# hellovuong/ORB_SLAM3_FAST

Measured on AMD Instinct MI355X. Metric: ORB extract+match frames/sec @1280×720 stereo (both-eye ORBextractor + ComputeStereoMatches), higher is better.
Workload: dtype u8; 1 GPU; C3: synthetic 1280x720 rectified stereo pairs, 1500 features, 8 levels, scale 1.2, FAST 20/7, ComputeStereoMatches (bf=0.12*532.03, b=0.12); handles=4, distinct_streams_per_gpu=32, frames_in_ring=3, stereo_matches_pair0=987, parallelism=independent stereo pairs sharded across GPUs, no data-path collective

## Files before the change

### include/orbx.h

```cpp
#ifndef ORBX_H_
#define ORBX_H_

#include <stddef.h>
#include <stdint.h>

#ifdef __cplusplus
extern "C" {
#endif

#define ORBX_MAX_LEVELS 12

#define ORBX_OK 0
#define ORBX_E_EMPTY (-1)
#define ORBX_E_BADARG (-2)
#define ORBX_E_CAPACITY (-3)
#define ORBX_E_HIP (-4)
#define ORBX_E_NODEVICE (-5)
#define ORBX_E_UNSUPPORTED (-6)
#define ORBX_E_TIMEOUT (-7)

typedef struct orbx_keypoint {
  float x, y, size, angle, response;
  int32_t octave, class_id;
} orbx_keypoint;
// ... 663 lines not shown
int orbx_kfdb_create_sized(int device, int n_vocabulary_words, int scoring, int max_keyframes, int max_words_per_keyframe,
                           orbx_kfdb** out);
void orbx_kfdb_destroy(orbx_kfdb* db);
int orbx_kfdb_size(const orbx_kfdb* db);
int orbx_kfdb_profile(orbx_kfdb* db, int on, float* last_ms);
int orbx_kfdb_add(orbx_kfdb* db, int kf_id, int map_id, const uint32_t* word_ids, const double* word_values, int n_words);
int orbx_kfdb_add_from_batch(orbx_kfdb* db, orbx_extractor* ex, int image, int kf_id, int map_id);
int orbx_kfdb_erase(orbx_kfdb* db, int kf_id);
int orbx_kfdb_clear(orbx_kfdb* db);
int orbx_kfdb_clear_map(orbx_kfdb* db, int map_id);
int orbx_kfdb_set_covisibles(orbx_kfdb* db, int n, const int32_t* kf_ids, const int32_t* best10);
int orbx_kfdb_detect_relocalization_candidates(orbx_kfdb* db, const uint32_t* word_ids, const double* word_values, int n_words,
                                               int map_id, int32_t* candidates, int cap, int32_t* n, const orbx_kfdb_details* details);
int orbx_kfdb_detect_relocalization_candidates_batch(orbx_kfdb* db, orbx_extractor* ex, int first_image, int n_frames,
                                                     const int32_t* map_ids, int32_t* candidates, int cap, int32_t* n,
                                                     const orbx_kfdb_details* details);
int orbx_kfdb_detect_n_best_candidates(orbx_kfdb* db, const uint32_t* word_ids, const double* word_values, int n_words, int map_id,
                                       const int32_t* connected_ids, int n_connected, const int32_t* bad_map_ids, int n_bad_maps,
                                       int n_candidates, int32_t* loop, int32_t* n_loop, int32_t* merge, int32_t* n_merge,
                                       const orbx_kfdb_details* details);



#define ORBX_STAGE_RESIZE 0
#define ORBX_STAGE_DETECT 1
#define ORBX_STAGE_OCTREE 2
#define ORBX_STAGE_BLUR 3
#define ORBX_STAGE_SLOTS 4
#define ORBX_STAGE_DESCRIBE 5
#define ORBX_STAGE_STEREO_MATCH 6
#define ORBX_STAGE_STEREO_FILTER 7
#define ORBX_NUM_STAGES 8
int orbx_profile_enable(orbx_extractor* ex, int on);
int orbx_profile_collect(orbx_extractor* ex, double* ms, int32_t* launches);
const char* orbx_stage_name(int stage);
int orbx_level_stats(orbx_extractor* ex, int image, int32_t* w, int32_t* h, int32_t* n_candidates,
                     int32_t* n_selected);


int orbx_clock_probe_start(int device, int spin_us, void** probe);
int orbx_clock_probe_finish(void* probe, double* ghz);

int orbx_copy_probe(int device, size_t bytes, int iters, double* gbps);

void orbx_debug_introsort(uint64_t* v, int n);
int orbx_debug_introsort_device(int device, uint64_t* v, int n);
#define ORBX_LINALG_RCP64 0
#define ORBX_LINALG_RSQRT64 1
#define ORBX_LINALG_JACOBI_CS 2
#define ORBX_LINALG_SVD3 3
#define ORBX_LINALG_NULL_VECTOR4 4
#define ORBX_LINALG_LDLT6 5
#define ORBX_LINALG_LDLT6_DAMPED 6
#define ORBX_LINALG_LDLT7 7
#define ORBX_LINALG_NULL_VECTOR_SYM9 8
#define ORBX_LINALG_NULL_VECTOR_SYM12 9
#define ORBX_LINALG_SUM16 10
#define ORBX_LINALG_OPS 11
#define ORBX_LINALG_MAX_ITEMS 65536
int orbx_debug_linalg(int device, int op, int n, const void* in, void* out);
#define ORBX_GEOM_CAM_PROJECT 0
#define ORBX_GEOM_CAM_UNPROJECT 1
#define ORBX_GEOM_CAM_UNPROJECT_ROUNDED_TAN 2
#define ORBX_GEOM_KB8_PROJECT_D 3
#define ORBX_GEOM_KB8_PROJECT_JAC 4
#define ORBX_GEOM_SE3_MAP 5
#define ORBX_GEOM_SE3_COMPOSE 6
#define ORBX_GEOM_QMUL 7
#define ORBX_GEOM_QROT 8
#define ORBX_GEOM_NORMALIZE_ROTATION 9
#define ORBX_GEOM_QUAT_FROM_R 10
#define ORBX_GEOM_OPLUS 11
#define ORBX_GEOM_SIM3_EXP 12
#define ORBX_GEOM_SIM3_OPLUS 13
#define ORBX_GEOM_SO_INVERSE 14
#define ORBX_GEOM_RODRIGUES2ROT 15
#define ORBX_GEOM_ROT2RODRIGUES 16
#define ORBX_GEOM_OPS 17
#define ORBX_GEOM_MAX_ITEMS 65536
int orbx_debug_geometry(int device, int op, int n, const void* in, void* out);

void orbx_debug_set_detect_list_cap(int cap);
void orbx_debug_set_octree_global(int on);
void orbx_debug_set_stereo_direct(int max_pairs);
int orbx_debug_upload_results(orbx_extractor* ex, int image, const orbx_keypoint* kps, const uint8_t* desc, int n, int mono_index);
void orbx_debug_set_clahe_cell_kernel(int on);
void orbx_debug_set_remap_lds(int on);
int orbx_debug_remap_footprints(const float* map_x, const float* map_y, ptrdiff_t map_stride, int out_w, int out_h, int src_w,
                                int src_h, int n_maps, int32_t* table, int cap, int32_t* tiles_x, int32_t* tiles_y);
int orbx_debug_front_tables(const orbx_params* p, int width, int height, uint32_t* cells, int cells_cap, uint32_t* tiles,
                            int tiles_cap, int32_t info[4]);
int orbx_debug_preproc_plan(const orbx_preproc* pp, int32_t info[8]);
void orbx_debug_set_resize_tail(int first_level, int max_levels, int band_rows);
int orbx_debug_resize_plan(const orbx_extractor* ex, int32_t* first_level, int32_t* n_levels, int32_t* n_bands, int cap);
int orbx_debug_score_map(orbx_extractor* ex, int enable);
int orbx_debug_score_level(orbx_extractor* ex, int image, int level, uint8_t* dst, ptrdiff_t dst_stride);
int orbx_debug_sincos(int device, const float* angles, int n, int fused, float* sin_out, float* cos_out);

#ifdef __cplusplus
}
#endif
#endif
```

### orb_slam3_fast_amd/__init__.py

```python
import ctypes as C
import os

import numpy as np

_HERE = os.path.dirname(os.path.abspath(__file__))
LIB_PATH = os.path.join(_HERE, os.environ.get("ORBX_LIB_NAME", "liborbx.so"))

KP_DTYPE = np.dtype([("x", "<f4"), ("y", "<f4"), ("size", "<f4"), ("angle", "<f4"), ("response", "<f4"),
                     ("octave", "<i4"), ("class_id", "<i4")])
assert KP_DTYPE.itemsize == 28

OK, E_EMPTY, E_BADARG, E_CAPACITY, E_HIP, E_NODEVICE, E_UNSUPPORTED, E_TIMEOUT = 0, -1, -2, -3, -4, -5, -6, -7
TH_HIGH, TH_LOW, HISTO_LENGTH = 100, 50, 30
NUM_STAGES = 8
MP_DTYPE = np.dtype([("proj_x", "<f4"), ("proj_y", "<f4"), ("proj_xr", "<f4"), ("view_cos", "<f4"), ("track_depth", "<f4"),
                     ("predicted_level", "<i4"), ("in_view", "u1"), ("bad", "u1"), ("has_observations", "u1"),
                     ("pad_", "u1"), ("desc", "u1", (32,))])
assert MP_DTYPE.itemsize == 60
PP_DTYPE = np.dtype([("u", "<f4"), ("v", "<f4"), ("ur", "<f4"), ("radius", "<f4"), ("angle", "<f4"), ("min_level", "<i4"),
                     ("max_level", "<i4"), ("valid", "u1"), ("has_observations", "u1"), ("pad_", "u1", (2,)),
                     ("desc", "u1", (32,))])
assert PP_DTYPE.itemsize == 64
FP_DTYPE = np.dtype([("u", "<f4"), ("v", "<f4"), ("ur", "<f4"), ("radius", "<f4"), ("predicted_level", "<i4"), ("valid", "u1"),
                     ("pad_", "u1", (3,)), ("desc", "u1", (32,))])
# ... 96 lines not shown
        L.orbx_preproc_destroy.restype = None
        L.orbx_preproc_output_size.argtypes = [vp, C.POINTER(i), C.POINTER(i)]
        L.orbx_preproc_run.argtypes = [vp, vp, C.c_ssize_t, i, vp, C.c_ssize_t]
        L.orbx_preproc_run_device.argtypes = [vp, vp, i, C.c_ssize_t, C.c_ssize_t, C.POINTER(vp), C.POINTER(i), C.POINTER(i),
                                              C.POINTER(C.c_ssize_t), C.POINTER(C.c_ssize_t)]
        L.orbx_extract_batch_raw_device.argtypes = [vp, vp, vp, i, C.c_ssize_t, C.c_ssize_t, vp]
        L.orbx_vocabulary_create.argtypes = [i, i, i, i, i, i, vp, vp, vp, vp, C.POINTER(vp)]
        L.orbx_vocabulary_load_text.argtypes = [i, C.c_char_p, C.POINTER(vp)]
        L.orbx_vocabulary_destroy.argtypes = [vp]
        L.orbx_vocabulary_destroy.restype = None
        L.orbx_vocabulary_info.argtypes = [vp, vp]
        L.orbx_bow_transform.argtypes = [vp, vp, i, i, vp, vp, C.POINTER(i), vp, vp, vp, C.POINTER(i)]
        L.orbx_bow_transform_batch.argtypes = [vp, vp, i]
        L.orbx_bow_results_device.argtypes = [vp] + [C.POINTER(vp)] * 6 + [C.POINTER(i)]
        L.orbx_bow_download.argtypes = [vp, i, vp, vp, C.POINTER(i), vp, vp, vp, C.POINTER(i), i]
        L.orbx_kfdb_create.argtypes = [vp, i, i, C.POINTER(vp)]
        L.orbx_kfdb_create_sized.argtypes = [i, i, i, i, i, C.POINTER(vp)]
        L.orbx_kfdb_destroy.argtypes = [vp]
        L.orbx_kfdb_destroy.restype = None
        L.orbx_kfdb_size.argtypes = [vp]
        L.orbx_kfdb_profile.argtypes = [vp, i, C.POINTER(f)]
        L.orbx_kfdb_add.argtypes = [vp, i, i, vp, vp, i]
        L.orbx_kfdb_add_from_batch.argtypes = [vp, vp, i, i, i]
        L.orbx_kfdb_erase.argtypes = [vp, i]
        L.orbx_kfdb_clear.argtypes = [vp]
        L.orbx_kfdb_clear_map.argtypes = [vp, i]
        L.orbx_kfdb_set_covisibles.argtypes = [vp, i, vp, vp]
        L.orbx_kfdb_detect_relocalization_candidates.argtypes = [vp, vp, vp, i, i, vp, i, C.POINTER(i), vp]
        L.orbx_kfdb_detect_relocalization_candidates_batch.argtypes = [vp, vp, i, i, vp, vp, i, vp, vp]
        L.orbx_kfdb_detect_n_best_candidates.argtypes = [vp, vp, vp, i, i, vp, i, vp, i, i, vp, C.POINTER(i), vp, C.POINTER(i), vp]
        L.orbx_search_by_bow.argtypes = [i, vp, vp, vp, i, vp, vp, vp, i, vp, vp, vp, i, vp, vp, i, i, f, i, vp]
        L.orbx_search_by_projection_fisheye_batch.argtypes = [vp, i, i, i, f, f, f, f, vp, vp, vp, i, f, i, f, f, vp, vp, vp, vp, vp, vp]
        L.orbx_search_by_projection_frame_fisheye_batch.argtypes = [vp, i, i, i, f, f, f, f, vp, vp, vp, i, i, vp, vp, vp, vp]
        L.orbx_search_by_bow_batch.argtypes = [vp, i, i, vp, vp, vp, i, vp, vp, vp, vp, vp, i, i, f, i, vp, vp]
        L.orbx_search_by_projection_fisheye.argtypes = [i, vp, vp, i, i, f, f, f, f, vp, i, vp, vp, i, f, i, f, f, vp, vp, vp, vp]
        L.orbx_search_by_projection_frame_fisheye.argtypes = [i, vp, vp, i, i, f, f, f, f, vp, vp, i, i, vp, vp]
        L.orbx_compute_image_bounds.argtypes = [i, i, i, vp, vp, i, vp]
        L.orbx_fisheye_results_device.argtypes = [vp, vp, vp, vp, vp, vp]
        L.orbx_fisheye_download.argtypes = [vp, i, vp, vp, vp, vp, i, i, vp]
        L.orbx_search_for_initialization.argtypes = [i, vp, vp, i, vp, vp, i, f, f, f, f, vp, vp, i, f, i]
        L.orbx_search_for_initialization_batch.argtypes = [vp, i, i, vp, vp, vp, i, f, f, f, f, vp, vp, i, f, i, vp]
        L.orbx_search_by_projection.argtypes = [i, vp, vp, vp, i, f, f, f, f, vp, i, vp, i, f, i, f, f, vp, vp]
        L.orbx_search_by_projection_frame.argtypes = [i, vp, vp, vp, i, f, f, f, f, vp, i, i, vp, vp]
        L.orbx_search_by_projection_frame_batch.argtypes = [vp, i, i, f, f, f, f, vp, vp, i, i, i, vp, vp, vp, vp]
        L.orbx_search_by_projection_batch.argtypes = [vp, i, i, f, f, f, f, vp, vp, i, f, i, f, f, i, vp, vp, vp, vp]
        L.orbx_search_by_projection_keyframe.argtypes = [i, vp, vp, i, f, f, f, f, vp, i, i, i, vp, vp]
        L.orbx_map_upload.argtypes = [vp, i, vp, vp, vp, vp, vp, vp]
        L.orbx_project_map_points_batch.argtypes = [vp, i, vp, f, f, f, f, f, vp, vp]
        L.orbx_last_frames_upload.argtypes = [vp, i, i, vp, vp, vp, vp, vp, vp]
        L.orbx_project_map_points_fisheye_batch.argtypes = [vp, i, vp, vp, f, f, f, f, f, vp, vp, vp]
        L.orbx_project_last_frames_batch.argtypes = [vp, i, vp, f, f, f, f, f, vp]
        L.orbx_search_for_triangulation.argtypes = [i, vp, vp, vp, i, vp, vp, vp, vp, i, vp, vp, vp, i, vp, vp, vp, vp, i, vp, vp, i,
                                                    vp, vp, i, i, i, vp]
        L.orbx_search_for_triangulation_rig.argtypes = [i, vp, vp, vp, i, vp, vp, vp, i, i, vp, vp, vp, i, vp, vp, vp, i, i, vp, vp, i, vp,
                                                        i, i, i, vp]
        L.orbx_search_by_bow_keyframes.argtypes = [i, vp, vp, vp, i, vp, vp, vp, i, vp, vp, vp, i, vp, vp, vp, i, f, i, vp]
        L.orbx_fuse_search.argtypes = [i, vp, vp, vp, i, f, f, f, f, vp, i, vp, i, i, vp, vp]
        L.orbx_features_in_area.argtypes = [i, vp, i, f, f, f, f, vp, i, vp, vp, i, vp, vp]
        L.orbx_comm_unique_id.argtypes = [vp]
        L.orbx_comm_create.argtypes = [vp, i, i, i, C.POINTER(vp)]
        L.orbx_comm_adopt.argtypes = [vp, i, C.POINTER(vp)]
        L.orbx_comm_destroy.argtypes = [vp]
        L.orbx_comm_destroy.restype = None
        L.orbx_comm_size.argtypes = [vp, C.POINTER(i), C.POINTER(i)]
        L.orbx_allgather_descriptors.argtypes = [vp, vp, i, vp, vp]
        L.orbx_comm_wait.argtypes = [vp, i, C.POINTER(C.c_ulonglong)]
        L.orbx_clock_probe_start.argtypes = [i, i, C.POINTER(vp)]
        L.orbx_clock_probe_finish.argtypes = [vp, C.POINTER(C.c_double)]
        L.orbx_copy_probe.argtypes = [i, C.c_size_t, i, C.POINTER(C.c_double)]
        L.orbx_profile_enable.argtypes = [vp, i]
        L.orbx_profile_collect.argtypes = [vp, vp, vp]
        L.orbx_stage_name.restype = C.c_char_p
        L.orbx_stage_name.argtypes = [i]
        L.orbx_level_stats.argtypes = [vp, i, vp, vp, vp, vp]
        L.orbx_debug_introsort.argtypes = [vp, i]
        L.orbx_debug_introsort.restype = None
        L.orbx_debug_introsort_device.argtypes = [i, vp, i]
        L.orbx_debug_linalg.argtypes = [i, i, i, vp, vp]
        L.orbx_debug_geometry.argtypes = [i, i, i, vp, vp]
        L.orbx_debug_set_detect_list_cap.argtypes = [i]
        L.orbx_debug_set_detect_list_cap.restype = None
        L.orbx_debug_set_octree_global.argtypes = [i]
        L.orbx_debug_set_octree_global.restype = None
        L.orbx_debug_set_stereo_direct.argtypes = [i]
        L.orbx_debug_set_stereo_direct.restype = None
        L.orbx_debug_set_clahe_cell_kernel.argtypes = [i]
        L.orbx_debug_set_clahe_cell_kernel.restype = None
        L.orbx_debug_upload_results.argtypes = [vp, i, vp, vp, i, i]
        L.orbx_debug_set_remap_lds.argtypes = [i]
        L.orbx_debug_set_remap_lds.restype = None
        L.orbx_debug_remap_footprints.argtypes = [vp, vp, C.c_ssize_t, i, i, i, i, i, vp, i, C.POINTER(i), C.POINTER(i)]
        L.orbx_debug_preproc_plan.argtypes = [vp, vp]
        if hasattr(L, "orbx_debug_front_tables"):
            L.orbx_debug_front_tables.argtypes = [vp, i, i, vp, i, vp, i, vp]
        L.orbx_debug_set_resize_tail.argtypes = [i, i, i]
        L.orbx_debug_set_resize_tail.restype = None
        L.orbx_debug_resize_plan.argtypes = [vp, vp, vp, vp, i]
        L.orbx_debug_sincos.argtypes = [i, vp, i, i, vp, vp]
        L.orbx_debug_score_map.argtypes = [vp, i]
        L.orbx_set_opencv_compat.argtypes = [vp, i]
        L.orbx_debug_score_level.argtypes = [vp, i, i, vp, C.c_ssize_t]
        _lib = L
    return _lib


def _check(rc):
    if rc < 0:
        raise OrbxError(rc, lib().orbx_last_error().decode())
    return rc


def _p(a):
    return a.ctypes.data_as(C.c_void_p)


def device_count():
    return lib().orbx_device_count()


class ORBextractor:

    def __init__(self, nfeatures, scaleFactor, nlevels, iniThFAST, minThFAST, max_width=1280, max_height=720,
                 max_batch=1, device=0):
        self.nfeatures, self.nlevels = int(nfeatures), int(nlevels)
        self.max_batch = max_batch
        p = _Params(nfeatures, scaleFactor, nlevels, iniThFAST, minThFAST)
        h = C.c_void_p()
        _check(lib().orbx_extractor_create(C.byref(p), max_width, max_height, max_batch, device, C.byref(h)))
        self._h = h
        self.device = device
        L = self.nlevels
        t = [np.zeros(L, np.float32) for _ in range(4)]
        self._nfeat = np.zeros(L, np.int32)
        self._umax = np.zeros(16, np.int32)
        _check(lib().orbx_get_tables(h, _p(t[0]), _p(t[1]), _p(t[2]), _p(t[3]), _p(self._nfeat), _p(self._umax)))
        self._scale, self._inv_scale, self._sigma2, self._inv_sigma2 = t
        cap = C.c_int()
        _check(lib().orbx_batch_results_device(h, None, None, None, None, C.byref(cap)))
        self.capacity = cap.value

    def close(self):
        if getattr(self, "_h", None):
            lib().orbx_extractor_destroy(self._h)
            self._h = None

    def __del__(self):
        try:
            self.close()
        except Exception:
            pass

    def GetLevels(self):
        return self.nlevels

    def GetScaleFactor(self):
        return float(self._scale[1]) if self.nlevels > 1 else 1.0

    def GetScaleFactors(self):
        return self._scale.copy()

    def GetInverseScaleFactors(self):
        return self._inv_scale.copy()

    def GetScaleSigmaSquares(self):
        return self._sigma2.copy()

# ... 1266 lines not shown
    def __init__(self, src_w, src_h, channels=1, rgb=True, maps=None, out_size=None, clahe=None, max_batch=2, device=0):
        prm = _PreprocParams()
        prm.src_w, prm.src_h, prm.channels, prm.rgb_order = src_w, src_h, channels, int(bool(rgb))
        keep = []
        if maps is not None:
            mx = np.ascontiguousarray(maps[0], np.float32)
            my = np.ascontiguousarray(maps[1], np.float32)
            if mx.ndim == 2:
                mx, my = mx[None], my[None]
            prm.n_maps, prm.out_h, prm.out_w = mx.shape
            prm.map_x, prm.map_y, prm.map_stride = mx.ctypes.data, my.ctypes.data, mx.shape[2]
            keep = [mx, my]
        elif out_size is not None:
            prm.out_w, prm.out_h = out_size
        if clahe is not None:
            prm.clahe_clip_limit, (prm.clahe_tiles_x, prm.clahe_tiles_y) = float(clahe[0]), clahe[1]
        h = C.c_void_p()
        _check(lib().orbx_preproc_create(C.byref(prm), max_batch, device, C.byref(h)))
        del keep
        self._h = h
        ow, oh = C.c_int(), C.c_int()
        _check(lib().orbx_preproc_output_size(self._h, C.byref(ow), C.byref(oh)))
        self.out_w, self.out_h, self.channels, self.src_w, self.src_h = ow.value, oh.value, channels, src_w, src_h

    def __del__(self):
        if getattr(self, "_h", None):
            lib().orbx_preproc_destroy(self._h)
            self._h = None

    def run(self, frame, map_index=0):
        frame = np.ascontiguousarray(frame, np.uint8)
        dst = np.zeros((self.out_h, self.out_w), np.uint8)
        _check(lib().orbx_preproc_run(self._h, _p(frame), frame.strides[0], map_index, _p(dst), dst.strides[0]))
        return dst

    def run_device(self, d_frames_ptr, n_frames, row_pitch, image_pitch):
        out, w, h = C.c_void_p(), C.c_int(), C.c_int()
        rp, ip = C.c_ssize_t(), C.c_ssize_t()
        _check(lib().orbx_preproc_run_device(self._h, C.c_void_p(d_frames_ptr), n_frames, row_pitch, image_pitch, C.byref(out),
                                             C.byref(w), C.byref(h), C.byref(rp), C.byref(ip)))
        return out.value, w.value, h.value, rp.value, ip.value

    def plan(self):
        info = np.zeros(8, np.int32)
        _check(lib().orbx_debug_preproc_plan(self._h, _p(info)))
        opt = [None if v < 0 else int(v) for v in info[2:6]]
        return {"lds_table": bool(info[0]), "resize_prepared": bool(info[1]), "remap": opt[0],
                "resize": None if opt[1] is None else ("plain" if opt[1] else "generic"),
                "clahe_vec4": None if opt[2] is None else bool(opt[2]), "gray_segs": opt[3], "frames": int(info[6])}


REMAP_LDS, REMAP_WINDOWS, REMAP_GENERIC = 2, 1, 0


def remap_footprints(map_x, map_y, src_w, src_h):
    mx = np.ascontiguousarray(map_x, np.float32)
    my = np.ascontiguousarray(map_y, np.float32)
    if mx.ndim == 2:
        mx, my = mx[None], my[None]
    if mx.shape != my.shape or mx.ndim != 3:
        raise ValueError("map_x and map_y must be float images of the same size")
    nm, dh, dw = mx.shape
    tx, ty = (dw + 127) // 128, (dh + 7) // 8
    tab = np.zeros((nm, tx, ty, 8), np.int32)
    gx, gy = C.c_int(), C.c_int()
    rc = lib().orbx_debug_remap_footprints(_p(mx), _p(my), dw, dw, dh, src_w, src_h, nm, _p(tab), tab.size, C.byref(gx), C.byref(gy))
    _check(rc)
    if (gx.value, gy.value) != (tx, ty):
        raise OrbxError("unexpected tile grid %d x %d" % (gx.value, gy.value))
    return tab if rc == 1 else None


def front_tables(nfeatures, scaleFactor, nlevels, iniThFAST, minThFAST, width, height):
    prm = _Params(int(nfeatures), float(scaleFactor), int(nlevels), int(iniThFAST), int(minThFAST))
    info = np.zeros(4, np.int32)
    _check(lib().orbx_debug_front_tables(C.byref(prm), width, height, None, 0, None, 0, _p(info)))
    cells = np.zeros((int(info[0]), 16), np.uint32)
    tiles = np.zeros(int(info[1]), np.uint32)
    _check(lib().orbx_debug_front_tables(C.byref(prm), width, height, _p(cells), cells.size, _p(tiles) if tiles.size else None,
                                         tiles.size, _p(info)))
    return cells, tiles, int(info[2]), int(info[3])


class ORBVocabulary:

    def __init__(self, k=None, L=None, parent=None, is_leaf=None, desc=None, weight=None, scoring=0, weighting=0, path=None,
                 device=0):
        h = C.c_void_p()
        if path is not None:
            _check(lib().orbx_vocabulary_load_text(device, path.encode(), C.byref(h)))
        else:
            parent = np.ascontiguousarray(parent, np.int32)
            leaf = np.ascontiguousarray(is_leaf, np.uint8)
            d = np.ascontiguousarray(desc, np.uint8)
            w = np.ascontiguousarray(weight, np.float64)
            _check(lib().orbx_vocabulary_create(device, k, L, scoring, weighting, len(parent), _p(parent), _p(leaf), _p(d), _p(w),
                                                C.byref(h)))
        self._h = h
        info = np.zeros(6, np.int32)
        _check(lib().orbx_vocabulary_info(self._h, _p(info)))
        self.k, self.L, self.n_nodes, self.n_words, self.scoring, self.weighting = (int(x) for x in info)

    def __del__(self):
        if getattr(self, "_h", None):
            lib().orbx_vocabulary_destroy(self._h)
            self._h = None

    def transform(self, desc, levelsup=4):
        d = np.ascontiguousarray(desc, np.uint8).reshape(-1, 32)
        n = len(d)
        words, values = np.zeros(n, np.uint32), np.zeros(n, np.float64)
        nodes, start, feats = np.zeros(n, np.uint32), np.zeros(n + 1, np.int32), np.zeros(n, np.uint32)
        nw, nn = C.c_int(), C.c_int()
        nf = _check(lib().orbx_bow_transform(self._h, _p(d), n, levelsup, _p(words), _p(values), C.byref(nw), _p(nodes), _p(start),
                                             _p(feats), C.byref(nn)))
        return (words[:nw.value].copy(), values[:nw.value].copy()), (nodes[:nn.value].copy(), start[:nn.value + 1].copy(), feats[:nf].copy())

    def transform_batch(self, extractor, levelsup=4):
        _check(lib().orbx_bow_transform_batch(extractor._h, self._h, levelsup))

    @staticmethod
    def download(extractor, image):
        cap = extractor.capacity
        words, values = np.zeros(cap, np.uint32), np.zeros(cap, np.float64)
        nodes, start, feats = np.zeros(cap, np.uint32), np.zeros(cap + 1, np.int32), np.zeros(cap, np.uint32)
        nw, nn = C.c_int(), C.c_int()
        nf = _check(lib().orbx_bow_download(extractor._h, image, _p(words), _p(values), C.byref(nw), _p(nodes), _p(start), _p(feats),
                                            C.byref(nn), cap))
        return (words[:nw.value].copy(), values[:nw.value].copy()), (nodes[:nn.value].copy(), start[:nn.value + 1].copy(), feats[:nf].copy())


class _KfdbDetails(C.Structure):
    _fields_ = [("cap", C.c_int32), ("n_scored", C.c_void_p), ("max_common_words", C.c_void_p), ("kf_id", C.c_void_p),
                ("common_words", C.c_void_p), ("score", C.c_void_p), ("acc_score", C.c_void_p), ("best_kf_id", C.c_void_p)]


KFDB_DETAIL_DTYPE = np.dtype([("kf_id", "<i4"), ("common_words", "<i4"), ("score", "<f4"), ("acc_score", "<f4"), ("best_kf_id", "<i4")])


class KeyFrameDatabase:

    def __init__(self, voc, max_keyframes, max_words):
        self._h = None
        h = C.c_void_p()
        _check(lib().orbx_kfdb_create(voc._h if voc is not None else None, max_keyframes, max_words, C.byref(h)))
        self._h = h
        self.max_keyframes, self.max_words = max_keyframes, max_words

    def close(self):
        if getattr(self, "_h", None):
            lib().orbx_kfdb_destroy(self._h)
            self._h = None

    __del__ = close

    def __len__(self):
        return _check(lib().orbx_kfdb_size(self._h))

    @staticmethod
    def _bow(bow):
        w, v = np.ascontiguousarray(bow[0], np.uint32), np.ascontiguousarray(bow[1], np.float64)
        if w.ndim != 1 or w.shape != v.shape:
            raise ValueError("a BoW vector is (word_ids[n], values[n])")
        return w, v

    def profile(self, on=-1):
# ... 423 lines not shown
```

### orb_slam3_fast_amd/csrc/orbx_api.hip

```cpp
#include "orbx_host.h"
#include "orbx_rgbd.h"

namespace orbx_host {
thread_local std::string g_err;
}

namespace {
struct StageTimer {
  orbx_extractor* ex;
  hipStream_t s;
  int stage;
  size_t i0 = 0;
  bool on;
  StageTimer(orbx_extractor* ex_, hipStream_t s_, int stage_)
      : ex(ex_), s(s_), stage(stage_), on(ex_->profiling && (ex_->profStage < 0 || ex_->profStage == stage_)) {
    if (!on) {
      if (s == ex->stream) ex->lastEvValid = false;
      return;
    }
    if (s == ex->stream && ex->lastEvValid) {
      i0 = ex->lastEv;
    } else {
      hipEvent_t e = ex->next_event();
      i0 = ex->evCursor - 1;
// ... 50 lines not shown
    um[v] = v0;
    ++v0;
  }
  std::memcpy(ex->umax, um, sizeof(um));
}

int build_geom(const orbx_extractor* ex, int w, int h, Geom& g, std::string& why) {
  std::memset(&g, 0, sizeof(g));
  const int L = ex->prm.nlevels;
  g.nlevels = L;
  g.iniTh = ex->prm.ini_th_fast;
  g.minTh = ex->prm.min_th_fast;
  g.cv440 = ex->cv440;
  long long off = 0, candOff = 0, cellOff = 0;
  int cells = 0, sel = 0, xc = 0, yc = 0;
  int maxCW = 0, maxCH = 0;
  for (int l = 0; l < L; l++) {
    LevelDev& v = g.lv[l];
    v.w = cv_round((float)w * ex->inv[l]);
    v.h = cv_round((float)h * ex->inv[l]);
    v.pitch = align_up(v.w, 64);
    v.off = off;
    off += (long long)v.pitch * v.h;
    off = (off + 255) / 256 * 256;
    const int maxBX = v.w - kBorder, maxBY = v.h - kBorder;
    const float width = (float)(maxBX - kBorder), height = (float)(maxBY - kBorder);
    if (width < 35.f || height < 35.f) {
      why = "level " + std::to_string(l) + " is smaller than one 35 px FAST cell (+32 px border)";
      return ORBX_E_UNSUPPORTED;
    }
    v.nCols = (int)(width / 35.f);
    v.nRows = (int)(height / 35.f);
    v.wCell = (int)std::ceil(width / v.nCols);
    v.hCell = (int)std::ceil(height / v.nRows);
    v.cellStart = cells;
    cells += v.nCols * v.nRows;
    v.quota = ex->nfeat[l];
    const int nIni = (int)std::round(width / height);
    if (nIni < 1 || nIni > kMaxIni) {
      why = "unsupported aspect ratio at level " + std::to_string(l);
      return ORBX_E_UNSUPPORTED;
    }
    v.candCap = (((int)width + v.nCols + 1) / 2 + 1) * (((int)height + v.nRows + 1) / 2 + 1);
    v.candOff = candOff;
    candOff += v.candCap;
    v.cellCap = ((v.wCell + 1) / 2) * ((v.hCell + 1) / 2);
    v.cellOff = cellOff;
    cellOff += (long long)v.nCols * v.nRows * v.cellCap;
    v.selOff = sel;
    v.selCap = v.quota + 4 * kMaxIni + 4;
    sel += v.selCap;
    v.xcoef = xc;
    v.ycoef = yc;
    xc += align_up(v.w, 256);
    yc += v.h;
    v.scale = ex->scale[l];
    v.patch = (float)(int)(31 * ex->scale[l]);
    maxCW = std::max(maxCW, v.wCell);
    maxCH = std::max(maxCH, v.hCell);
    if (v.w > 4096 || v.h > 4096) {
      why = "images larger than 4096 px are not supported by the 12-bit key packing";
      return ORBX_E_UNSUPPORTED;
    }
  }
  if (maxCW > 250 || maxCH > 120) {
    why = "FAST cell too large for the packed corner list";
    return ORBX_E_UNSUPPORTED;
  }
  g.totalCells = cells;
  g.tileP = 4 * ((maxCW + 3) / 4 + 2);
  g.tileH = maxCH + 6;
  g.scoreP = 4 * ((maxCW + 3) / 4 + 2);
  g.scoreH = maxCH + 2;
  g.listCap = align_up((long long)maxCW * maxCH, 8);
  g.selImg = sel;
  g.outCap = sel;
  g.pyrImg = off;
  g.candImg = candOff;
  g.cellImg = cellOff;
  if (resize_lds_bytes(g) > 160 * 1024 - 2048) {
    why = "scale factor too large for the LDS-staged resize footprint";
    return ORBX_E_UNSUPPORTED;
  }
  if (octree_lds_bytes(g) > 160 * 1024 - 2048) {
    why = "nfeatures too large for the LDS-resident quadtree";
    return ORBX_E_UNSUPPORTED;
  }
  return ORBX_OK;
}

void build_yrow(const Geom& g, const std::vector<int>& yofs, std::vector<uint32_t>& yrow) {
  yrow.assign(yofs.size(), 0);
  for (int l = 1; l < g.nlevels; l++) {
    const int Sh = g.lv[l - 1].h;
    for (int dy = 0; dy < g.lv[l].h; dy++) {
      const int sy = yofs[g.lv[l].ycoef + dy];
      const int a = std::min(std::max(sy, 0), Sh - 1), b = std::min(std::max(sy + 1, 0), Sh - 1);
      yrow[g.lv[l].ycoef + dy] = (uint32_t)a | ((uint32_t)b << 16);
    }
  }
}

void build_resize_records(const Geom& g, const std::vector<uint4>& xtab, const std::vector<uint32_t>& yrow, const std::vector<short>& yab,
                          std::vector<uint32_t>& tab) {
  int tileOff, rowOff;
  tab.assign((size_t)resize_records_layout(g, g.nlevels, tileOff, rowOff), 0u);
  for (int l = 1; l < g.nlevels; l++) {
    const LevelDev &D = g.lv[l], &S = g.lv[l - 1];
    resize_records_layout(g, l, tileOff, rowOff);
    const int nbx = (D.w + 255) / 256, nby = (D.h + 15) / 16;
    for (int tby = 0; tby < nby; tby++) {
      const int y0 = tby * 16, y1 = std::min(y0 + 16, D.h) - 1;
      const int rb = (int)(yrow[D.ycoef + y0] & 0xFFFFu), re = (int)(yrow[D.ycoef + y1] >> 16);
      const int nrows = re - rb + 1;
      for (int tbx = 0; tbx < nbx; tbx++) {
        const int x0 = tbx * 256, x1 = std::min(x0 + 256, D.w) - 1;
        const int cb = (int)xtab[D.xcoef + x0].y;
        const int ce = std::min((int)xtab[D.xcoef + x1].x + 1, S.w - 1);
        const int ndw = ((ce - cb) >> 2) + 1;
        const bool whole = l > 1 || cb + 4 * ndw <= S.w;
        const bool fast = whole && ndw > 64 && ndw <= 85 && nrows <= 24 && rb + 28 <= S.h;
        uint32_t* t = &tab[(size_t)tileOff + 8 * (size_t)(tby * nbx + tbx)];
        t[0] = (uint32_t)(D.xcoef + x0);
        t[1] = (uint32_t)x0 | ((uint32_t)(y1 - y0 + 1) << 16);
        t[2] = (uint32_t)rb | ((uint32_t)nrows << 16);
        t[3] = (uint32_t)cb | ((uint32_t)ndw << 16);
        t[4] = (fast ? kTileFast : 0u) | (whole ? kTileWhole : 0u);
        t[5] = (uint32_t)((long long)y0 * D.pitch);
        t[6] = (uint32_t)tby;
      }
      for (int w = 0; w < 4; w++)
        for (int k = 0; k < 4; k++) {
          const int dy = std::min(y0 + w + 4 * k, D.h - 1);
          const uint32_t sy = yrow[D.ycoef + dy];
          uint32_t* r = &tab[(size_t)rowOff + 16 * (size_t)(4 * tby + w) + 4 * k];
          r[0] = (uint32_t)(uint16_t)yab[2 * (D.ycoef + dy)] | ((uint32_t)(uint16_t)yab[2 * (D.ycoef + dy) + 1] << 16);
          r[1] = (uint32_t)(((int)(sy & 0xFFFFu) - rb) * 512);
          r[2] = (uint32_t)(((int)(sy >> 16) - rb) * 512);
        }
    }
  }
}

void build_cell_records(const Geom& g, std::vector<CellRec>& recs) {
  recs.assign((size_t)g.totalCells, CellRec{});
  const int TPd = g.tileP >> 2;
  for (int l = 0; l < g.nlevels; l++) {
    const LevelDev& L = g.lv[l];
    const int maxBX = L.w - kBorder, maxBY = L.h - kBorder;
    for (int ci = 0; ci < L.nRows; ci++)
      for (int cj = 0; cj < L.nCols; cj++) {
        const int cell = ci * L.nCols + cj;
        CellRec& r = recs[(size_t)L.cellStart + cell];
        const int iniY = kBorder + ci * L.hCell, iniX = kBorder + cj * L.wCell;
        const int maxY = std::min(iniY + L.hCell + 6, maxBY), maxX = std::min(iniX + L.wCell + 6, maxBX);
        const int rw = maxX - iniX, rh = maxY - iniY;
        const int dw = rw - 6, dh = rh - 6;
        r.flags = ((uint32_t)l << 8) | ((uint32_t)L.w << 16) | (l == 0 ? kCellL0 : 0u);
        if (iniY >= maxBY - 3 || iniX >= maxBX - 6 || dw <= 0 || dh <= 0) {
          r.flags |= kCellReject;
          continue;
        }
        if (iniX + g.tileP <= L.w) r.flags |= kCellWide;
        r.xy = (uint32_t)iniX | ((uint32_t)iniY << 16);
        r.roi = (uint32_t)rw | ((uint32_t)rh << 16);
        r.pitch = (uint32_t)L.pitch;
        r.baseOff = (uint32_t)(L.off + (long long)iniY * L.pitch + iniX);
// ... 152 lines not shown
    bands.insert(bands.end(), nd.begin(), nd.end());
    plans.push_back(tp);
    l += nT;
  }
}

constexpr int kLatLdsMax = 156 * 1024, kLatMaxImages = 2;
static int g_lat_max_images = kLatMaxImages;
static int g_lat_levels = 4, g_lat_rows = 2;
void build_latency_plans(const Geom& g, const std::vector<int>& yofs, std::vector<TailPlan>& plans, std::vector<TailBand>& bands) {
  plans.clear();
  bands.clear();
  static const bool envRead = [] {
    if (const char* e = getenv("ORBX_LAT_TAIL")) {
      int a = -1, b = 0;
      if (sscanf(e, "%d,%d", &a, &b) >= 1) {
        g_lat_levels = a;
        if (b > 0) g_lat_rows = b;
      }
    }
    if (const char* e = getenv("ORBX_LAT_MAX_IMAGES")) g_lat_max_images = atoi(e);
    return true;
  }();
  (void)envRead;
  if (g_lat_levels <= 0) return;
  const int L = g.nlevels;
  int l = 1;
  while (l < L) {
    TailPlan tp;
    std::vector<TailBand> nd;
    int nT = std::min(g_lat_levels, L - l);
    while (nT >= 1 && !build_tail_segment(g, yofs, l, nT, g_lat_rows, tp, nd, 1, 1, (size_t)kLatLdsMax)) nT--;
    if (nT < 1) {
      plans.clear();
      bands.clear();
      return;
    }
    tp.bandOff = (int)bands.size();
    bands.insert(bands.end(), nd.begin(), nd.end());
    plans.push_back(tp);
    l += nT;
  }
}

int configure(orbx_extractor* ex, int w, int h) {
  if (w == ex->curW && h == ex->curH) return ORBX_OK;
  if (w > ex->maxW || h > ex->maxH)
    return fail(ORBX_E_CAPACITY, "image larger than the handle's max_width x max_height");
  Geom g;
  std::string why;
  int rc = build_geom(ex, w, h, g, why);
  if (rc != ORBX_OK) return fail(rc, why);
  const Geom& m = ex->gmax;
  if (g.pyrImg > m.pyrImg || g.candImg > m.candImg || g.selImg > m.selImg || g.cellImg > m.cellImg ||
      g.totalCells > m.totalCells)
    return fail(ORBX_E_CAPACITY, "image within max_width x max_height but its pyramid / cell-grid rounding needs more "
                                 "buffer than the handle's maximum size: create the handle with this size");
  g.outCap = m.outCap;
  g.selImg = m.selImg;
  g.pyrImg = m.pyrImg;
  g.candImg = m.candImg;
  g.cellImg = m.cellImg;
  std::vector<uint4> xtab;
  std::vector<int> yofs;
  std::vector<short> yab;
  build_coefs(g, xtab, yofs, yab);
  HIPC(hipStreamSynchronize(ex->stream));
  HIPC(hipMemcpy(ex->d_xtab.p, xtab.data(), xtab.size() * sizeof(uint4), hipMemcpyHostToDevice));
  HIPC(hipMemcpy(ex->d_yofs.p, yofs.data(), yofs.size() * sizeof(int), hipMemcpyHostToDevice));
  {
    std::vector<uint32_t> yrow, rec;
    build_yrow(g, yofs, yrow);
    HIPC(hipMemcpy(ex->d_yrow.p, yrow.data(), yrow.size() * sizeof(uint32_t), hipMemcpyHostToDevice));
    build_resize_records(g, xtab, yrow, yab, rec);
    if (ex->d_rsRec.n < rec.size()) HIPC(ex->d_rsRec.alloc(rec.size()));
    if (!rec.empty()) HIPC(hipMemcpy(ex->d_rsRec.p, rec.data(), rec.size() * sizeof(uint32_t), hipMemcpyHostToDevice));
  }
  HIPC(hipMemcpy(ex->d_yab.p, yab.data(), yab.size() * sizeof(short), hipMemcpyHostToDevice));
  {
    std::vector<CellRec> recs;
    build_cell_records(g, recs);
    HIPC(hipMemcpy(ex->d_cellRec.p, recs.data(), recs.size() * sizeof(CellRec), hipMemcpyHostToDevice));
  }
  HIPC(prepare_kernels(g));
  std::vector<TailPlan> plans;
  std::vector<TailBand> bands;
  build_tail_plans(g, yofs, plans, bands);
  if (!plans.empty()) {
    if (ex->d_tailBands.n < bands.size()) HIPC(ex->d_tailBands.alloc(bands.size()));
    HIPC(hipMemcpy(ex->d_tailBands.p, bands.data(), bands.size() * sizeof(TailBand), hipMemcpyHostToDevice));
    unsigned lds = 0;
    for (const TailPlan& tp : plans) lds = std::max(lds, tp.ldsBytes);
    HIPC(prepare_resize_tail(lds));
  }
  ex->tails = plans;
  {
    std::vector<TailPlan> lp;
    std::vector<TailBand> lb;
    build_latency_plans(g, yofs, lp, lb);
    if (!lp.empty()) {
      if (ex->d_latBands.n < lb.size()) HIPC(ex->d_latBands.alloc(lb.size()));
      HIPC(hipMemcpy(ex->d_latBands.p, lb.data(), lb.size() * sizeof(TailBand), hipMemcpyHostToDevice));
      unsigned lds = 0;
      for (const TailPlan& tp : lp) lds = std::max(lds, tp.ldsBytes);
      HIPC(prepare_resize_tail(lds));
    }
    ex->latTails = lp;
  }
  ex->g = g;
  ex->curW = w;
  ex->curH = h;
  return ORBX_OK;
}

struct DetectToken {
  std::mutex mu;
  hipEvent_t ev = nullptr;
  bool valid = false;
  const orbx_extractor* last = nullptr;
};
static DetectToken* detect_token(int device) {
  static std::mutex mu;
  static DetectToken* toks[64] = {nullptr};
  if (device < 0 || device >= 64) return nullptr;
  std::lock_guard<std::mutex> lk(mu);
  if (!toks[device]) {
    DetectToken* t = new DetectToken();
    if (hipEventCreateWithFlags(&t->ev, hipEventDisableTiming) != hipSuccess) {
      delete t;
      return nullptr;
    }
    toks[device] = t;
  }
  return toks[device];
}

int record_pipeline(orbx_extractor* ex, int n, bool lapTrivial, bool capturing, bool pyrDone = false);
static void drop_graphs(orbx_extractor* ex) {
  for (auto& e : ex->graphExec) {
    if (e) (void)hipGraphExecDestroy(e);
    e = nullptr;
  }
}

static bool latency_plan_ok(const orbx_extractor* ex, const uint8_t* d_images, int n, int w, ptrdiff_t row_pitch,
                            ptrdiff_t image_pitch) {
  if (ex->latTails.empty() || n > g_lat_max_images) return false;
  if (((uintptr_t)d_images & 15) || (row_pitch & 15) || (image_pitch & 15)) return false;
  return (w & 15) == 0 || d_images == ex->d_stage.p;
}

static int prepare_extract(orbx_extractor* ex, const uint8_t* d_images, int n, int w, int h, ptrdiff_t row_pitch,
                           ptrdiff_t image_pitch, const int32_t* lap, bool& lapTrivial) {
  int rc = configure(ex, w, h);
  if (rc != ORBX_OK) return rc;
  ex->pyr.l0 = d_images;
  ex->pyr.l0Row = row_pitch;
  ex->pyr.l0Img = image_pitch;
  ex->pyr.pyr = ex->d_pyr.p;
  ex->lastN = n;
  ex->lastEvValid = false;
  ex->blurValid = false;
  ex->lastStereoPairs = 0;
  ex->hostPyrImages = 0;
  ex->useLat = latency_plan_ok(ex, d_images, n, w, row_pitch, image_pitch);
  hipStream_t s = ex->stream;
// ... 22 lines not shown
    return ORBX_OK;
  }
  size_t seg = 0;
  for (int l = 1; l < g.nlevels;) {
    StageTimer t(ex, s, ORBX_STAGE_RESIZE);
    if (seg < ex->tails.size() && ex->tails[seg].lA == l) {
      const TailPlan& tp = ex->tails[seg++];
      HIPC(launch_resize_tail(g, ex->pyr, tp, ex->d_tailBands.p + tp.bandOff, 0, n, ex->d_xtab.p, ex->d_yofs.p, ex->d_yab.p, s));
      l += tp.nT;
    } else {
      HIPC(launch_resize(g, ex->pyr, n, l, ex->d_xtab.p, ex->d_yrow.p, ex->d_yab.p, ex->d_rsRec.p, s));
      l++;
    }
  }
  return ORBX_OK;
}

int enqueue_extract(orbx_extractor* ex, const uint8_t* d_images, int n, int w, int h, ptrdiff_t row_pitch,
                    ptrdiff_t image_pitch, const int32_t* lap) {
  bool lapTrivial = true;
  int rc = prepare_extract(ex, d_images, n, w, h, row_pitch, image_pitch, lap, lapTrivial);
  if (rc != ORBX_OK) return rc;
  hipStream_t s = ex->stream;
  static const bool useGraph = getenv("ORBX_GRAPH") && atoi(getenv("ORBX_GRAPH")) != 0;
  if (useGraph && n == 1 && d_images == ex->d_stage.p && !ex->profiling && !ex->graphOff) {
    if (ex->graphW != w || ex->graphH != h) {
      drop_graphs(ex);
      ex->graphW = w;
      ex->graphH = h;
    }
    hipGraphExec_t& exec = ex->graphExec[lapTrivial ? 1 : 0];
    if (!exec) {
      hipGraph_t graph = nullptr;
      bool ok = hipStreamBeginCapture(s, hipStreamCaptureModeThreadLocal) == hipSuccess;
      if (ok) {
        const int rcCap = record_pipeline(ex, n, lapTrivial, true);
        const hipError_t ee = hipStreamEndCapture(s, &graph);
        ok = rcCap == ORBX_OK && ee == hipSuccess && graph != nullptr;
      }
      if (ok) ok = hipGraphInstantiate(&exec, graph, nullptr, nullptr, 0) == hipSuccess;
      if (graph) (void)hipGraphDestroy(graph);
      if (!ok) {
        (void)hipGetLastError();
        exec = nullptr;
        ex->graphOff = true;
      }
    }
    if (exec) {
      HIPC(hipGraphLaunch(exec, s));
      return ORBX_OK;
    }
  }
  return record_pipeline(ex, n, lapTrivial, false);
}

int record_pipeline(orbx_extractor* ex, int n, bool lapTrivial, bool capturing, bool pyrDone) {
  const Geom& g = ex->g;
  hipStream_t s = ex->stream;
  ex->blurValid = false;
  if (!pyrDone) {
    const int rc = enqueue_pyramid(ex, s, 0, n);
    if (rc != ORBX_OK) return rc;
  }
  if (ex->d_dbgScore.p) HIPC(hipMemsetAsync(ex->d_dbgScore.p, 0, ex->d_dbgScore.n, s));
  static const bool noToken = getenv("ORBX_NO_DETECT_TOKEN") && atoi(getenv("ORBX_NO_DETECT_TOKEN")) != 0;
  DetectToken* tok = (!capturing && !noToken && n > g_lat_max_images) ? detect_token(ex->device) : nullptr;
  if (tok) {
    std::lock_guard<std::mutex> lk(tok->mu);
    if (tok->valid && tok->last != ex) HIPC(hipStreamWaitEvent(s, tok->ev, 0));
    ex->lastEvValid = false;
    {
      StageTimer t(ex, s, ORBX_STAGE_DETECT);
      HIPC(launch_detect(g, ex->pyr, ex->d_cellRec.p, n, ex->d_cellCand.p, ex->d_cellCount.p, 0, g.nlevels, ex->d_dbgScore.p, s));
    }
    HIPC(hipEventRecord(tok->ev, s));
    tok->valid = true;
    tok->last = ex;
  } else {
    StageTimer t(ex, s, ORBX_STAGE_DETECT);
    HIPC(launch_detect(g, ex->pyr, ex->d_cellRec.p, n, ex->d_cellCand.p, ex->d_cellCount.p, 0, g.nlevels, ex->d_dbgScore.p, s));
  }
  {
    StageTimer t(ex, s, ORBX_STAGE_OCTREE);
    HIPC(launch_octree(g, n, ex->d_cellCand.p, ex->d_cellCount.p, ex->d_cellPrefix.p, ex->d_cand.p,
                       ex->d_candCount.p, ex->d_knode.p, ex->d_sel.p, ex->d_selCount.p, 0, g.nlevels, s));
  }
  if (!lapTrivial) {
    StageTimer t(ex, s, ORBX_STAGE_SLOTS);
    HIPC(launch_slots(g, n, ex->d_sel.p, ex->d_selCount.p, ex->d_lap.p, ex->d_slot.p, ex->d_nOut.p, ex->d_mono.p, s));
  }
  {
    StageTimer t(ex, s, ORBX_STAGE_DESCRIBE);
    HIPC(launch_describe(g, ex->pyr, n, ex->d_sel.p, ex->d_selCount.p, lapTrivial ? nullptr : ex->d_slot.p, ex->d_kps.p,
                         ex->d_desc.p, ex->d_nOut.p, ex->d_mono.p, s));
  }
  return ORBX_OK;
}

int set_device(int device) {
  int n = 0;
  if (hipGetDeviceCount(&n) != hipSuccess || n <= 0) return fail(ORBX_E_NODEVICE, "no HIP device available");
  if (device < 0 || device >= n) return fail(ORBX_E_BADARG, "device index out of range");
  HIPC(hipSetDevice(device));
  return ORBX_OK;
}

}

extern "C" {

const char* orbx_last_error(void) { return g_err.c_str(); }
int orbx_abi_version(void) { return 1; }
int orbx_device_count(void) {
  int n = 0;
  if (hipGetDeviceCount(&n) != hipSuccess) return 0;
  return n;
}

int orbx_extractor_create(const orbx_params* p, int max_width, int max_height, int max_batch, int device,
                          orbx_extractor** out) {
  if (!p || !out) return fail(ORBX_E_BADARG, "null argument");
  *out = nullptr;
  if (p->nlevels < 1 || p->nlevels > ORBX_MAX_LEVELS || p->nfeatures < 1 || !(p->scale_factor > 1.0f) ||
      p->ini_th_fast < p->min_th_fast || p->min_th_fast < 1 || p->ini_th_fast > 254 || max_batch < 1 ||
      max_width < 1 || max_height < 1)
    return fail(ORBX_E_BADARG, "invalid extractor parameters");
  int rc = set_device(device);
  if (rc != ORBX_OK) return rc;
  orbx_extractor* ex = new orbx_extractor();
  ex->prm = *p;
  ex->device = device;
  ex->maxW = max_width;
  ex->maxH = max_height;
  ex->maxB = max_batch;
  build_tables(ex);
  std::string why;
  rc = build_geom(ex, max_width, max_height, ex->gmax, why);
  if (rc != ORBX_OK) {
    delete ex;
    return fail(rc, why);
  }
  const Geom& m = ex->gmax;
  const size_t B = (size_t)max_batch;
  ex->stagePitch = align_up(max_width, 64);
  int nx = 0, ny = 0;
  for (int l = 0; l < m.nlevels; l++) {
    nx += align_up(m.lv[l].w, 256);
    ny += m.lv[l].h;
  }
  hipError_t e = hipSuccess;
  auto ok = [&](hipError_t r) {
    if (e == hipSuccess) e = r;
  };
  ok(hipStreamCreateWithFlags(&ex->stream, hipStreamNonBlocking));
  ok(hipEventCreateWithFlags(&ex->done, hipEventDisableTiming));
  ok(ex->d_pyr.alloc(B * m.pyrImg + 256));
  ok(ex->d_stage.alloc(B * (size_t)ex->stagePitch * max_height + 256));
  ok(ex->d_cand.alloc(B * m.candImg));
  ok(ex->d_cellCand.alloc(B * m.cellImg));
  ok(ex->d_cellCount.alloc(B * m.totalCells));
  ok(ex->d_cellPrefix.alloc(B * m.totalCells));
  ok(ex->d_knode.alloc(B * m.candImg));
  ok(ex->d_candCount.alloc(B * m.nlevels));
  ok(ex->d_sel.alloc(B * m.selImg));
  ok(ex->d_selCount.alloc(B * m.nlevels + ORBX_MAX_LEVELS));
  ok(ex->d_slot.alloc(B * m.selImg));
  ok(ex->d_kps.alloc(B * m.outCap));
  ok(ex->d_desc.alloc(B * m.outCap * 32));
// ... 612 lines not shown
    HIPC(hipHostMalloc(reinterpret_cast<void**>(&ex->hostPyr), need, hipHostMallocDefault));
    ex->hostPyrBytes = need;
  }
  uint8_t* H = ex->hostPyr;
  const bool want0 = n_levels > 0 && dst[0];
  bool wantRest = false;
  for (int l = 1; l < n_levels; l++) wantRest = wantRest || dst[l];
  if (want0) HIPC(hipMemcpyAsync(H, l0, l0Bytes, hipMemcpyDeviceToHost, ex->stream));
  if (wantRest)
    HIPC(hipMemcpyAsync(H + l0Bytes, ex->pyr.pyr + (long long)image * g.pyrImg + restOff, restBytes, hipMemcpyDeviceToHost, ex->stream));
  HIPC(hipStreamSynchronize(ex->stream));
  for (int l = 0; l < n_levels; l++) {
    if (!dst[l]) continue;
    const LevelDev& L = g.lv[l];
    const uint8_t* src = l == 0 ? H : H + l0Bytes + ((size_t)L.off - restOff);
    const size_t sp = l == 0 ? (size_t)p0 : (size_t)L.pitch;
    if ((size_t)dst_stride[l] == sp && sp == (size_t)L.w) {
      std::memcpy(dst[l], src, sp * L.h);
    } else {
      for (int y = 0; y < L.h; y++) std::memcpy(dst[l] + (size_t)y * dst_stride[l], src + (size_t)y * sp, (size_t)L.w);
    }
  }
  return ORBX_OK;
}

int orbx_debug_candidates(orbx_extractor* ex, int image, int level, int32_t* xys, int cap) {
  if (!ex || image < 0 || image >= ex->lastN || level < 0 || level >= ex->g.nlevels)
    return fail(ORBX_E_BADARG, "bad argument");
  HIPC(hipSetDevice(ex->device));
  HIPC(hipStreamSynchronize(ex->stream));
  const LevelDev& L = ex->g.lv[level];
  const int cells = L.nCols * L.nRows;
  std::vector<int> cnt(cells);
  HIPC(hipMemcpy(cnt.data(), ex->d_cellCount.p + (long long)image * ex->g.totalCells + L.cellStart, (size_t)cells * sizeof(int),
                 hipMemcpyDeviceToHost));
  std::vector<uint32_t> v((size_t)cells * L.cellCap);
  if (!v.empty())
    HIPC(hipMemcpy(v.data(), ex->d_cellCand.p + (long long)image * ex->g.cellImg + L.cellOff, v.size() * 4, hipMemcpyDeviceToHost));
  int n = 0;
  for (int c = 0; c < cells; c++)
    for (int i = 0; i < cnt[c] && n < L.candCap; i++, n++) {
      if (n >= cap) continue;
      const uint32_t k = v[(size_t)c * L.cellCap + i];
      xys[3 * n] = key_x(k);
      xys[3 * n + 1] = key_y(k);
      xys[3 * n + 2] = key_r(k);
    }
  return n;
}

int orbx_debug_front_tables(const orbx_params* p, int width, int height, uint32_t* cells, int cells_cap, uint32_t* tiles,
                            int tiles_cap, int32_t info[4]) {
  if (!p || !info || width < 1 || height < 1 || cells_cap < 0 || tiles_cap < 0 || (cells_cap && !cells) || (tiles_cap && !tiles) ||
      p->nlevels < 1 || p->nlevels > ORBX_MAX_LEVELS || p->nfeatures < 1 || !(p->scale_factor > 1.0f))
    return fail(ORBX_E_BADARG, "bad argument");
  std::unique_ptr<orbx_extractor> ex(new orbx_extractor());
  ex->prm = *p;
  build_tables(ex.get());
  Geom g;
  std::string why;
  const int rc = build_geom(ex.get(), width, height, g, why);
  if (rc != ORBX_OK) return fail(rc, why);
  std::vector<uint4> xtab;
  std::vector<int> yofs;
  std::vector<short> yab;
  std::vector<uint32_t> yrow, rec;
  std::vector<CellRec> cr;
  build_coefs(g, xtab, yofs, yab);
  build_yrow(g, yofs, yrow);
  build_resize_records(g, xtab, yrow, yab, rec);
  build_cell_records(g, cr);
  info[0] = (int32_t)cr.size(); info[1] = (int32_t)rec.size(); info[2] = g.tileP; info[3] = g.tileH;
  if (cells) {
    if (cr.size() * 16 > (size_t)cells_cap) return fail(ORBX_E_CAPACITY, "cell records larger than cells_cap");
    std::memcpy(cells, cr.data(), cr.size() * sizeof(CellRec));
  }
  if (tiles) {
    if (rec.size() > (size_t)tiles_cap) return fail(ORBX_E_CAPACITY, "tile records larger than tiles_cap");
    std::memcpy(tiles, rec.data(), rec.size() * sizeof(uint32_t));
  }
  return ORBX_OK;
}

int orbx_hamming256(const void* a, const void* b) {
  const uint32_t* x = (const uint32_t*)a;
  const uint32_t* y = (const uint32_t*)b;
  int d = 0;
  for (int i = 0; i < 8; i++) d += __builtin_popcount(x[i] ^ y[i]);
  return d;
}

static int enqueue_stereo_match(orbx_extractor* left, int first_left, orbx_extractor* right, int first_right,
                                int n_pairs, float bf, float b, bool withFilter, StereoArgs* argsOut,
                                const ResultPack* packWithBand, bool* packedOut) {
  if (packedOut) *packedOut = false;
  if (!left || !right) return fail(ORBX_E_BADARG, "null handle");
  if (n_pairs <= 0 || first_left < 0 || first_right < 0 || first_left + n_pairs > left->lastN ||
      first_right + n_pairs > right->lastN)
    return fail(ORBX_E_BADARG, "pair range outside the last extraction");
  if (left->device != right->device || left->curW != right->curW || left->curH != right->curH ||
      std::memcmp(&left->prm, &right->prm, sizeof(orbx_params)) != 0)
    return fail(ORBX_E_BADARG, "left and right extractors must share device, image size and parameters");
  if (!(b > 0.f)) return fail(ORBX_E_BADARG, "baseline must be positive");
  HIPC(hipSetDevice(left->device));
  const size_t capL = (size_t)left->gmax.outCap;
  if (left->stereoPairs < n_pairs) {
    HIPC(hipStreamSynchronize(left->stream));
    if (left->uRPairs < n_pairs) {
      HIPC(left->d_uR.alloc((size_t)n_pairs * capL));
      HIPC(left->d_depth.alloc((size_t)n_pairs * capL));
      left->uRPairs = n_pairs;
    }
    HIPC(left->d_sad.alloc((size_t)n_pairs * capL));
    const size_t capS = std::max(capL, (size_t)right->gmax.outCap);
    HIPC(left->d_rowStart.alloc((size_t)n_pairs * 2 * (left->maxH + 2)));
    HIPC(left->d_srec.alloc((size_t)n_pairs * 2 * capS));
    HIPC(left->d_sdesc.alloc((size_t)n_pairs * 2 * capS * 2));
    left->stereoPairs = n_pairs;
  }
  left->lastStereoPairs = n_pairs;
  if (right != left && hipStreamQuery(right->stream) != hipSuccess) {
    HIPC(hipEventRecord(right->done, right->stream));
    HIPC(hipStreamWaitEvent(left->stream, right->done, 0));
  }
  StereoArgs a;
  a.kL = left->d_kps.p;
  a.kR = right->d_kps.p;
  a.dL = left->d_desc.p;
  a.dR = right->d_desc.p;
  a.nL = left->d_nOut.p;
  a.nR = right->d_nOut.p;
  a.capL = (int)capL;
  a.capR = right->gmax.outCap;
  a.firstL = first_left;
  a.firstR = first_right;
  a.bf = bf;
  a.b = b;
  a.uRight = left->d_uR.p;
  a.depth = left->d_depth.p;
  a.sad = left->d_sad.p;
  a.rowStart = left->d_rowStart.p;
  a.srec = left->d_srec.p;
  a.sdesc = left->d_sdesc.p;
  a.cap = (int)std::max(capL, (size_t)right->gmax.outCap);
  a.imgH = left->curH;
  a.band = (int)std::ceil(2.0f * left->scale.back()) + 2;
  const bool direct = stereo_direct_ok(a, n_pairs);
  if (!direct) {
    StageTimer t(left, left->stream, ORBX_STAGE_STEREO_MATCH);
    HIPC(launch_stereo_sort(left->g, a, n_pairs, left->stream));
  }
  {
    StageTimer t(left, left->stream, ORBX_STAGE_STEREO_MATCH);
    const bool pack = direct && packWithBand && n_pairs == 1;
    HIPC(launch_stereo_match(left->g, left->pyr, right->pyr, a, n_pairs, left->stream, direct, pack ? packWithBand : nullptr));
    if (pack && packedOut) *packedOut = true;
  }
  if (withFilter) {
    StageTimer t(left, left->stream, ORBX_STAGE_STEREO_FILTER);
    HIPC(launch_stereo_filter(a, n_pairs, left->stream));
  }
  if (argsOut) *argsOut = a;
  return ORBX_OK;
}

int orbx_stereo_match_batch(orbx_extractor* left, int first_left, orbx_extractor* right, int first_right,
// ... 130 lines not shown
                                const float** d_depth, const float** d_points3d, const int32_t** d_counts) {
  if (!left || left->fisheyePairs == 0) return fail(ORBX_E_BADARG, "no fisheye association has been run on this handle");
  if (d_left_to_right) *d_left_to_right = left->d_fl2r.p;
  if (d_right_to_left) *d_right_to_left = left->d_fr2l.p;
  if (d_depth) *d_depth = left->d_fdepth.p;
  if (d_points3d) *d_points3d = left->d_fp3d.p;
  if (d_counts) *d_counts = left->d_fcnt.p;
  return ORBX_OK;
}

int orbx_fisheye_download(orbx_extractor* left, int pair, int32_t* left_to_right, int32_t* right_to_left, float* depth,
                          float* points3d, int cap_left, int cap_right, int32_t* n_desc_matches) {
  if (!left || pair < 0 || pair >= left->fisheyePairs) return fail(ORBX_E_BADARG, "bad pair index");
  HIPC(hipSetDevice(left->device));
  HIPC(hipStreamSynchronize(left->stream));
  const size_t capL = (size_t)left->gmax.outCap, capR = (size_t)left->fisheyeCapR;
  const size_t nl = std::min(capL, (size_t)std::max(cap_left, 0)), nr = std::min(capR, (size_t)std::max(cap_right, 0));
  if (left_to_right) HIPC(hipMemcpy(left_to_right, left->d_fl2r.p + pair * capL, nl * sizeof(int), hipMemcpyDeviceToHost));
  if (right_to_left) HIPC(hipMemcpy(right_to_left, left->d_fr2l.p + pair * capR, nr * sizeof(int), hipMemcpyDeviceToHost));
  if (depth) HIPC(hipMemcpy(depth, left->d_fdepth.p + pair * capL, nl * sizeof(float), hipMemcpyDeviceToHost));
  if (points3d) HIPC(hipMemcpy(points3d, left->d_fp3d.p + pair * capL * 3, nl * 3 * sizeof(float), hipMemcpyDeviceToHost));
  int cnt[2] = {0, 0};
  HIPC(hipMemcpy(cnt, left->d_fcnt.p + 2 * pair, sizeof(cnt), hipMemcpyDeviceToHost));
  if (n_desc_matches) *n_desc_matches = cnt[1];
  return cnt[0];
}

int orbx_profile_enable(orbx_extractor* ex, int on) {
  if (!ex) return fail(ORBX_E_BADARG, "null handle");
  ex->profiling = on != 0;
  ex->profStage = on >= 2 ? on - 2 : -1;
  ex->lastEvValid = false;
  return ORBX_OK;
}

int orbx_profile_collect(orbx_extractor* ex, double* ms, int32_t* launches) {
  if (!ex || !ms || !launches) return fail(ORBX_E_BADARG, "null argument");
  HIPC(hipSetDevice(ex->device));
  HIPC(hipStreamSynchronize(ex->stream));
  for (int i = 0; i < ORBX_NUM_STAGES; i++) {
    ms[i] = 0;
    launches[i] = 0;
  }
  for (const auto& r : ex->evLog) {
    float t = 0;
    HIPC(hipEventElapsedTime(&t, ex->evPool[r.e0], ex->evPool[r.e1]));
    ms[r.stage] += t;
    launches[r.stage]++;
  }
  ex->evLog.clear();
  ex->evCursor = 0;
  ex->lastEvValid = false;
  return ORBX_OK;
}

const char* orbx_stage_name(int stage) {
  static const char* names[ORBX_NUM_STAGES] = {"k_resize", "k_detect", "k_octree", "k_blur",
                                                "k_slots",  "k_describe", "k_stereo_match", "k_stereo_filter"};
  return stage >= 0 && stage < ORBX_NUM_STAGES ? names[stage] : "?";
}

int orbx_level_stats(orbx_extractor* ex, int image, int32_t* w, int32_t* h, int32_t* n_candidates,
                     int32_t* n_selected) {
  if (!ex || ex->curW == 0 || image < 0 || image >= ex->lastN) return fail(ORBX_E_BADARG, "bad argument");
  HIPC(hipSetDevice(ex->device));
  HIPC(hipStreamSynchronize(ex->stream));
  const int L = ex->g.nlevels;
  for (int l = 0; l < L; l++) {
    if (w) w[l] = ex->g.lv[l].w;
    if (h) h[l] = ex->g.lv[l].h;
  }
  if (n_candidates)
    HIPC(hipMemcpy(n_candidates, ex->d_candCount.p + image * L, L * sizeof(int), hipMemcpyDeviceToHost));
  if (n_selected)
    HIPC(hipMemcpy(n_selected, ex->d_selCount.p + image * L, L * sizeof(int), hipMemcpyDeviceToHost));
  return ORBX_OK;
}

void orbx_debug_introsort(uint64_t* v, int n) { debug_introsort_host(v, n); }
void orbx_debug_set_detect_list_cap(int cap) { debug_set_detect_list_cap(cap); }
void orbx_debug_set_clahe_cell_kernel(int on) { debug_set_clahe_cell_kernel(on); }
void orbx_debug_set_remap_lds(int on) { debug_set_remap_lds(on); }
void orbx_debug_set_octree_global(int on) { debug_set_octree_global(on); }
void orbx_debug_set_stereo_direct(int max_pairs) { debug_set_stereo_direct(max_pairs); }
void orbx_debug_set_resize_tail(int first_level, int max_levels, int band_rows) {
  orbx_host::g_tail_first = first_level;
  orbx_host::g_tail_levels = max_levels > 0 ? max_levels : orbx_host::kTailLevels;
  orbx_host::g_tail_rows = band_rows > 0 ? band_rows : orbx_host::kTailRows;
}
int orbx_debug_resize_plan(const orbx_extractor* ex, int32_t* first_level, int32_t* n_levels, int32_t* n_bands, int cap) {
  if (!ex) return fail(ORBX_E_BADARG, "null handle");
  int n = 0;
  for (const TailPlan& tp : ex->tails) {
    if (n < cap) {
      if (first_level) first_level[n] = tp.lA;
      if (n_levels) n_levels[n] = tp.nT;
      if (n_bands) n_bands[n] = tp.nBands;
    }
    n++;
  }
  return n;
}
int orbx_debug_introsort_device(int device, uint64_t* v, int n) {
  if (!v || n < 0 || n > 4000) return fail(ORBX_E_BADARG, "bad argument");
  if (n == 0) return ORBX_OK;
  int rc = set_device(device);
  if (rc != ORBX_OK) return rc;
  ScratchBuf<uint64_t> d;
  HIPC(d.alloc(n));
  hipError_t e = hipMemcpy(d.p, v, (size_t)n * 8, hipMemcpyHostToDevice);
  if (e == hipSuccess) e = launch_debug_sort(d.p, n, nullptr);
  if (e == hipSuccess) e = hipDeviceSynchronize();
  if (e == hipSuccess) e = hipMemcpy(v, d.p, (size_t)n * 8, hipMemcpyDeviceToHost);
  if (e != hipSuccess) return fail(ORBX_E_HIP, hipGetErrorString(e));
  return ORBX_OK;
}

int orbx_debug_score_map(orbx_extractor* ex, int enable) {
  if (!ex) return fail(ORBX_E_BADARG, "null handle");
  HIPC(hipSetDevice(ex->device));
  HIPC(hipStreamSynchronize(ex->stream));
  drop_graphs(ex);
  if (enable && !ex->d_dbgScore.p) HIPC(ex->d_dbgScore.alloc((size_t)ex->maxB * ex->gmax.pyrImg + 256));
  if (!enable) ex->d_dbgScore.free();
  return ORBX_OK;
}

int orbx_debug_score_level(orbx_extractor* ex, int image, int level, uint8_t* dst, ptrdiff_t dst_stride) {
  if (!ex || !dst || !ex->d_dbgScore.p || ex->curW == 0 || image < 0 || image >= ex->lastN || level < 0 ||
      level >= ex->g.nlevels)
    return fail(ORBX_E_BADARG, "score map not enabled or no such level");
  HIPC(hipSetDevice(ex->device));
  HIPC(hipStreamSynchronize(ex->stream));
  const LevelDev& L = ex->g.lv[level];
  HIPC(hipMemcpy2D(dst, dst_stride, ex->d_dbgScore.p + (long long)image * ex->g.pyrImg + L.off, L.pitch, L.w, L.h,
                   hipMemcpyDeviceToHost));
  return ORBX_OK;
}

int orbx_debug_sincos(int device, const float* angles, int n, int fused, float* sin_out, float* cos_out) {
  if (!angles || !sin_out || !cos_out || n < 0) return fail(ORBX_E_BADARG, "bad argument");
  if (n == 0) return ORBX_OK;
  int rc = set_device(device);
  if (rc != ORBX_OK) return rc;
  ScratchBuf<float> d;
  HIPC(d.alloc((size_t)3 * n));
  hipError_t e = hipMemcpy(d.p, angles, (size_t)n * 4, hipMemcpyHostToDevice);
  if (e == hipSuccess) e = launch_debug_sincos(d.p, n, fused, d.p + n, d.p + 2 * (size_t)n, nullptr);
  if (e == hipSuccess) e = hipDeviceSynchronize();
  if (e == hipSuccess) e = hipMemcpy(sin_out, d.p + n, (size_t)n * 4, hipMemcpyDeviceToHost);
  if (e == hipSuccess) e = hipMemcpy(cos_out, d.p + 2 * (size_t)n, (size_t)n * 4, hipMemcpyDeviceToHost);
  if (e != hipSuccess) return fail(ORBX_E_HIP, hipGetErrorString(e));
  return ORBX_OK;
}

}
```

### orb_slam3_fast_amd/csrc/orbx_host.h

```cpp
#ifndef ORBX_HOST_H
#define ORBX_HOST_H
#if defined(__x86_64__) || defined(__i386__)
#include <immintrin.h>
static inline void cpu_pause() { _mm_pause(); }
#else
static inline void cpu_pause() {}
#endif
#include <memory>
#include <new>
#include <chrono>
#include <climits>
#include <cmath>
#include <cstdio>
#include <cstdlib>
#include <cstring>
#include <string>
#include <mutex>
#include <type_traits>
#include <vector>

#include "orbx_internal.h"

using namespace orbx;

// ... 247 lines not shown
    if (!flag[i]) continue;
    if (kps && (kps[i].octave < 0 || kps[i].octave >= nlevels)) return "keypoint octave outside [0, nlevels)";
    const float* w = worldPos + 3 * (size_t)i;
    if (!finite_all(w, 3)) return "world position not finite";
    idx.push_back(i);
    pos.insert(pos.end(), w, w + 3);
  }
  return nullptr;
}

struct BowSide {
  const uint32_t* ids; const int32_t* start; const uint32_t* feat; int nNodes;
  const orbx_keypoint* kps; const uint8_t* desc; const uint8_t* flags; int n;
  int list() const { return nNodes ? start[nNodes] : 0; }
};
inline int check_nodes(const BowSide& s, const char* what) {
  for (int j = 0; j < s.nNodes; j++)
    if (s.start[j] < 0 || s.start[j] > s.start[j + 1] || (j && s.ids[j] <= s.ids[j - 1]))
      return fail(ORBX_E_BADARG, std::string(what) + ": node ids must ascend and offsets must be monotone");
  return ORBX_OK;
}
inline int check_features(const BowSide& s, const char* what) {
  for (int i = 0; i < s.list(); i++)
    if (s.feat[i] >= (uint32_t)s.n) return fail(ORBX_E_BADARG, std::string(what) + " out of range");
  return ORBX_OK;
}

struct SideAreas { size_t ids, start, feat, desc, flags, kps; };
inline SideAreas add_side(Pack& pk, const BowSide& s) {
  SideAreas o;
  o.ids = pk.add(s.ids, (size_t)s.nNodes * 4);
  o.start = pk.add(s.start, ((size_t)s.nNodes + 1) * 4);
  o.feat = pk.add(s.feat, (size_t)s.list() * 4);
  o.desc = pk.add(s.desc, (size_t)s.n * 32);
  o.flags = pk.add(s.flags, s.n);
  o.kps = pk.add(s.kps, (size_t)s.n * sizeof(orbx_keypoint));
  return o;
}
inline TriArgs tri_args(const Pack& pk, const BowSide& s1, const SideAreas& o1, const BowSide& s2, const SideAreas& o2) {
  TriArgs a{};
  a.nodes1 = pk.ptr<uint32_t>(o1.ids); a.start1 = pk.ptr<int>(o1.start); a.feat1 = pk.ptr<uint32_t>(o1.feat);
  a.nNodes1 = s1.nNodes; a.nList1 = s1.list();
  a.nodes2 = pk.ptr<uint32_t>(o2.ids); a.start2 = pk.ptr<int>(o2.start); a.feat2 = pk.ptr<uint32_t>(o2.feat); a.nNodes2 = s2.nNodes;
  a.k1 = pk.ptr<orbx_keypoint>(o1.kps); a.k2 = pk.ptr<orbx_keypoint>(o2.kps);
  a.d1 = pk.ptr<uint32_t>(o1.desc); a.d2 = pk.ptr<uint32_t>(o2.desc); a.mp1 = pk.ptr<uint8_t>(o1.flags); a.mp2 = pk.ptr<uint8_t>(o2.flags);
  a.n1 = s1.n; a.n2 = s2.n;
  return a;
}

}
using namespace orbx_host;


static inline size_t hr_flag() { return 32; }
static inline size_t hr_kps(size_t) { return 64; }
static inline size_t hr_desc(size_t cap) { return hr_kps(cap) + 2 * cap * sizeof(orbx_keypoint); }
static inline size_t hr_ur(size_t cap) { return hr_desc(cap) + 2 * cap * 32; }
static inline size_t hr_depth(size_t cap) { return hr_ur(cap) + cap * sizeof(float); }
static inline size_t host_results_bytes(size_t cap) { return hr_depth(cap) + cap * sizeof(float) + 64; }

struct orbx_extractor {
  orbx_params prm{};
  int device = 0;
  hipStream_t stream = nullptr;
  hipEvent_t done = nullptr;
  int maxW = 0, maxH = 0, maxB = 0;
  std::vector<float> scale, inv, sig2, invsig2;
  std::vector<int> nfeat;
  int umax[16];
  Geom g{};
  Geom gmax{};
  int curW = 0, curH = 0;
  Pyr pyr{};
  int lastN = 0;
  DevBuf<uint8_t> d_pyr, d_blur, d_stage, d_desc;
  DevBuf<uint8_t> d_dbgScore;
  DevBuf<uint32_t> d_cand, d_cellCand, d_sel;
  DevBuf<uint16_t> d_knode;
  DevBuf<int> d_rowStart, d_cellCount, d_cellPrefix, d_candCount, d_selCount, d_slot, d_nOut, d_mono, d_lap, d_yofs, d_sad;
  DevBuf<short> d_yab;
  DevBuf<uint4> d_xtab;
  DevBuf<uint32_t> d_rsRec;
  DevBuf<orbx::CellRec> d_cellRec;
  DevBuf<int> d_packCtr;
  uint32_t packSeq = 0;
  bool packCtrDirty = false;
  DevBuf<uint32_t> d_yrow;
  DevBuf<uint4> d_srec, d_sdesc;
  std::vector<orbx::TailPlan> tails;
  DevBuf<orbx::TailBand> d_tailBands;
  std::vector<orbx::TailPlan> latTails;
  DevBuf<orbx::TailBand> d_latBands;
  DevBuf<orbx_keypoint> d_kps;
  DevBuf<float> d_uR, d_depth;
  int stagePitch = 0;
  int stereoPairs = 0;
  int lastStereoPairs = 0;
  int uRPairs = 0;
  DevBuf<float> d_mapPos, d_mapNormal, d_mapMinD, d_mapMaxD;
  DevBuf<uint8_t> d_mapDesc, d_mapFlags, d_mapSkip;
  DevBuf<orbx_frame_pose> d_poses;
  DevBuf<orbx_map_point_view> d_views;
  DevBuf<float> d_lfPos, d_lfAngle;
  DevBuf<int> d_lfOct, d_lfN;
  DevBuf<uint8_t> d_lfDesc, d_lfFlags;
  DevBuf<orbx_frame_pose_q> d_posesQ;
  DevBuf<orbx_projected_point> d_pviews;
  DevBuf<float> d_scaleF;
  DevBuf<orbx_frame_pose_kb8> d_posesK;
  DevBuf<orbx_map_point_view> d_fviewsL, d_fviewsR;
  int fviewsFrames = 0, fviewsStride = 0;
  int lfFrames = 0, lfStride = 0, pviewsFrames = 0;
  std::vector<int> lfN;
  int mapN = 0, viewsFrames = 0, viewsStride = 0;
  uint8_t* hostResults = nullptr;
  int hostResImages = 0;
  bool hostResStereo = false;
  uint8_t* hostPyr = nullptr;
  size_t hostPyrBytes = 0;
  bool useLat = false;
  hipStream_t streamPyr = nullptr;
  hipEvent_t evPyr = nullptr;
  bool keepHostPyr = false;
  uint8_t* hostPyrAll = nullptr;
  size_t hostPyrAllBytes = 0;
  int hostPyrImages = 0;
  int hostPyrL0Pitch = 0;
  int32_t* h_lap = nullptr;
  int lapN = 0;
  hipGraphExec_t graphExec[2] = {nullptr, nullptr};
  int graphW = 0, graphH = 0;
  bool graphOff = false;
  DevBuf<int> d_bowWord, d_bowNode, d_bowStart, d_bowCounts;
  DevBuf<double> d_bowWeight, d_bowValues;
  DevBuf<uint32_t> d_bowWords, d_bowNodes, d_bowFeats;
  int bowImages = 0;
  DevBuf<int> d_fl2r, d_fr2l, d_fcnt, d_fcand;
  DevBuf<float> d_fdepth, d_fp3d;
  int fisheyePairs = 0, fisheyeCapR = 0;
  bool profiling = false;
  int profStage = -1;
  std::vector<hipEvent_t> evPool;
  size_t evCursor = 0;
  struct EvRec { int stage; size_t e0, e1; };
  std::vector<EvRec> evLog;
  size_t lastEv = 0;
  bool lastEvValid = false;
  int cv440 = 0;
  bool blurValid = false;
  hipEvent_t next_event() {
    if (evCursor == evPool.size()) {
      hipEvent_t e;
      if (hipEventCreate(&e) != hipSuccess) return nullptr;
      evPool.push_back(e);
    }
    return evPool[evCursor++];
  }
};

struct orbx_vocabulary {
  int device = 0, k = 0, L = 0, scoring = 0, weighting = 0, nNodes = 0, nWords = 0;
  DevBuf<int> childStart, children, wordId;
  DevBuf<uint32_t> desc;
  DevBuf<double> weight;
  BowVoc view() const {
    BowVoc v{};
// ... 25 lines not shown
```

### orb_slam3_fast_amd/csrc/orbx_internal.h

```cpp
#pragma once
#include <hip/hip_runtime.h>
#include <stdint.h>
#include <vector>

#include "../../include/orbx.h"

namespace orbx {

constexpr int kEdge = 19;
constexpr int kHalfPatch = 15;
constexpr int kBorder = 16;
constexpr int kMaxIni = 8;

struct LevelDev {
  int w, h, pitch;
  int nCols, nRows, wCell, hCell;
  int cellStart;
  int quota;
  int candCap;
  int cellCap;
  int selOff, selCap;
  int xcoef, ycoef;
  long long off;
  long long candOff;
// ... 16 lines not shown
  LevelDev lv[ORBX_MAX_LEVELS];
};

constexpr uint32_t kCellReject = 1u;
constexpr uint32_t kCellWide = 2u;
constexpr uint32_t kCellL0 = 4u;
struct alignas(64) CellRec {
  uint32_t xy;
  uint32_t roi;
  uint32_t flags;
  uint32_t pitch;
  uint32_t baseOff;
  uint32_t outOff;
  uint32_t cellCap;
  uint32_t rounds;
  uint32_t nRounds;
  uint32_t nScore16;
  uint32_t actLastLo, actLastHi;
  uint32_t killLastA, killLastB;
  float invQpr;
  uint32_t pad_;
};
static_assert(sizeof(CellRec) == 64, "one scalar load");
struct DetectArgs {
  int totalCells, iniTh, minTh;
  int tileP, tileH, scoreH;
  float invTileP;
  int listCap, cellBegin;
  long long pyrImg, cellImg;
};

struct Pyr {
  const uint8_t* l0;
  long long l0Row, l0Img;
  uint8_t* pyr;
  uint8_t* blur;
};

__host__ __device__ inline const uint8_t* level_ptr(const Geom& g, const Pyr& p, int img, int l, int& pitch) {
  if (l == 0) {
    pitch = (int)p.l0Row;
    return p.l0 + (long long)img * p.l0Img;
  }
  pitch = g.lv[l].pitch;
  return p.pyr + (long long)img * g.pyrImg + g.lv[l].off;
}

__host__ __device__ inline uint32_t pack_key(int x, int y, int r) {
  return (uint32_t)x | ((uint32_t)y << 12) | ((uint32_t)r << 24);
}
__host__ __device__ inline int key_x(uint32_t k) { return k & 0xFFF; }
__host__ __device__ inline int key_y(uint32_t k) { return (k >> 12) & 0xFFF; }
__host__ __device__ inline int key_r(uint32_t k) { return k >> 24; }

struct TailBand {
  int first, last, ownEnd, pad_;
};
struct TailPlan {
  int lA, nT, nBands, bandOff;
  int tileBytes[2];
  int pitch[ORBX_MAX_LEVELS + 1];
  int rtOff[ORBX_MAX_LEVELS];
  int rtTotal;
  unsigned ldsBytes;
};
hipError_t launch_resize_tail(const Geom& g, const Pyr& p, const TailPlan& tp, const TailBand* bands, int img0, int nimg,
                              const uint4* xtab, const int* yofs, const short* yab, hipStream_t s);
hipError_t prepare_resize_tail(unsigned ldsBytes);
hipError_t raise_dynamic_lds(const void* fn, size_t bytes);

size_t resize_plain_lds(int sw, int sh, int dw, int dh);
hipError_t prepare_resize_plain(int sw, int sh, int dw, int dh);
hipError_t launch_resize_plain(const uint8_t* src, int sw, int sh, long long sp, long long sip, uint8_t* dst, int dw, int dh,
                               long long dp, long long dip, const uint4* xtab, const uint32_t* yrow, const short* yab, int nimg,
                               hipStream_t s);
hipError_t launch_resize(const Geom& g, const Pyr& p, int nimg, int level, const uint4* xtab, const uint32_t* yofs ,
                         const short* yab, const uint32_t* records, hipStream_t s);
int resize_records_layout(const Geom& g, int level, int& tileOff, int& rowOff);
constexpr uint32_t kTileFast = 1u, kTileWhole = 2u;
hipError_t launch_detect(const Geom& g, const Pyr& p, const CellRec* cellRec, int nimg, uint32_t* cellCand, int* cellCount,
                         int level0, int level1, uint8_t* dbgScore, hipStream_t s);
hipError_t launch_octree(const Geom& g, int nimg, const uint32_t* cellCand, const int* cellCount, int* cellPrefix,
                         uint32_t* cand, int* candCount, uint16_t* knode, uint32_t* sel, int* selCount, int level0,
                         int level1, hipStream_t s);
hipError_t launch_blur(const Geom& g, const Pyr& p, int nimg, int level0, int level1, hipStream_t s);
hipError_t launch_slots(const Geom& g, int nimg, const uint32_t* sel, const int* selCount, const int* lap,
                        int* slot, int* nOut, int* mono, hipStream_t s);
hipError_t launch_describe(const Geom& g, const Pyr& p, int nimg, const uint32_t* sel, const int* selCount,
                           const int* slot, orbx_keypoint* kps, uint8_t* desc, int* nOut, int* mono, hipStream_t s);
size_t octree_lds_bytes(const Geom& g);
size_t resize_lds_bytes(const Geom& g);

struct StereoArgs {
  const orbx_keypoint *kL, *kR;
  const uint8_t *dL, *dR;
  const int *nL, *nR;
  int capL, capR;
  int firstL, firstR;
  float bf, b;
  float* uRight;
  float* depth;
  int* sad;
  int* rowStart;
  uint4* srec;
  uint4* sdesc;
  int cap;
  int imgH;
  int band;
};
hipError_t launch_stereo_sort(const Geom& g, const StereoArgs& a, int npairs, hipStream_t s);
bool stereo_direct_ok(const StereoArgs& a, int npairs);
void debug_set_stereo_direct(int max_pairs);
struct ResultPack;
hipError_t launch_stereo_match(const Geom& g, const Pyr& pl, const Pyr& pr, const StereoArgs& a, int npairs,
                               hipStream_t s, bool direct = false, const ResultPack* pack = nullptr);
hipError_t launch_stereo_filter(const StereoArgs& a, int npairs, hipStream_t s);
hipError_t launch_bf_knn2(const uint8_t* dQ, int nQ, const uint8_t* dT, int nT, int* idx2, int* dist2,
                          uint8_t* ok, hipStream_t s);

struct FisheyeArgs {
  const orbx_keypoint* kL;
  const orbx_keypoint* kR;
  int nL, nR, monoL, monoR;
  const int* idx2;
  const uint8_t* ratioOk;
  orbx_kb8_rig rig;
  const float* sigma2;
  int nLevels;
  int* leftToRight;
  int* rightToLeft;
  float* depth;
  float* p3D;
  int* counters;
};
hipError_t launch_fisheye_triangulate(const FisheyeArgs& a, hipStream_t s);

struct FisheyeBatchArgs {
  const orbx_keypoint* kL;
  const orbx_keypoint* kR;
  const uint8_t* dL;
  const uint8_t* dR;
  const int* nL;
  const int* nR;
  const int* monoL;
  const int* monoR;
  int capL, capR, firstL, firstR;
  orbx_kb8_rig rig;
  float sigma2[ORBX_MAX_LEVELS];
  int nLevels;
  int* leftToRight;
  int* rightToLeft;
  float* depth;
  float* p3D;
  int* counters;
  uint2* cand;
  int* candCount;
};
hipError_t launch_fisheye_batch(const FisheyeBatchArgs& a, int npairs, hipStream_t s);

struct UndistortArgs {
  const float* in;
  float* out;
  int n, stride;
  float K[4];
  float k[12];
  int hasDist;
};
hipError_t launch_undistort(const UndistortArgs& a, hipStream_t s);

struct RgbdArgs {
  const orbx_keypoint* kps;
  const int* nOut;
  int cap, first;
// ... 213 lines not shown
struct MapProjArgs {
  const float *pos, *normal, *minDist, *maxDist;
  const uint8_t *desc, *flags, *skip;
  const orbx_frame_pose* poses;
  orbx_map_point_view* views;
  int n, nlevels;
  float minX, minY, maxX, maxY, viewCosLimit, logScaleFactor;
};
hipError_t launch_project_map(const MapProjArgs& a, int nFrames, hipStream_t s);
struct MapProjKb8Args {
  const float *pos, *normal, *minDist, *maxDist;
  const uint8_t *desc, *flags, *skip;
  const orbx_frame_pose_kb8 *posesL, *posesR;
  orbx_map_point_view *viewsL, *viewsR;
  int n, nlevels;
  float minX, minY, maxX, maxY, viewCosLimit, logScaleFactor;
};
hipError_t launch_project_map_kb8(const MapProjKb8Args& a, int nFrames, hipStream_t s);
struct LastProjArgs {
  const float* pos;
  const int* octave;
  const float* angle;
  const uint8_t *desc, *flags;
  const int* npts;
  const orbx_frame_pose_q* poses;
  const float* scale;
  orbx_projected_point* views;
  int stride, nlevels;
  float minX, minY, maxX, maxY, th;
};
hipError_t launch_project_last(const LastProjArgs& a, int nFrames, hipStream_t s);
hipError_t launch_proj_batch(const ProjArgs* d_frames, int nFrames, int maxPts, int maxN2, int mode, int checkOri, int rounds,
                             hipStream_t s);

struct FuseArgs {
  InitArgs grid;
  const uint32_t* desc;
  const float* uRight;
  const float* invSigma2;
  const orbx_fuse_point* pts;
  int npts;
  int maxDist;
  int* bestIdx;
  int* bestDist;
  int* result;
};
hipError_t launch_fuse_search(const FuseArgs& a, hipStream_t s);


struct ProjFeArgs {
  const int *offL, *idxL, *distL;
  const int *offR, *idxR, *distR;
  int nLeft, n, nmp, mode, checkOri;
  float nnratio;
  const orbx_map_point_view* mps;
  const orbx_projected_point* pts;
  const orbx_keypoint* kps;
  const int *l2r, *r2l;
  uint8_t* occupied;
  int* match;
  int* result;
  int4* writes[2];
  int* writers[3];
  int* nwriters[3];
  int* flags;
};
hipError_t launch_proj_resolve_fisheye(const ProjFeArgs& a, hipStream_t s);
hipError_t launch_proj_rounds_fisheye(const ProjFeArgs& a, int first_round, int rounds, hipStream_t s);
hipError_t launch_proj_finish_fisheye(const ProjFeArgs& a, int last_round, hipStream_t s);
struct FeConcatArgs {
  const orbx_keypoint* kps; const uint8_t* desc; const int* nOut;
  int firstL, firstR, cap;
  orbx_keypoint* kcat; uint8_t* dcat;
};
hipError_t launch_fe_concat(const FeConcatArgs& a, int nFrames, hipStream_t s);
hipError_t launch_proj_fisheye_batch(const ProjArgs* d_sides, const ProjFeArgs* d_frames, int nFrames, int maxPts, int maxN, int mode,
                                     int checkOri, int rounds, hipStream_t s);
hipError_t prepare_kernels(const Geom& g);
hipError_t prepare_detect(const Geom& g);
void debug_introsort_host(uint64_t* v, int n);
void debug_set_detect_list_cap(int cap);
void debug_set_clahe_cell_kernel(int on);
void debug_set_octree_global(int on);
hipError_t launch_debug_sort(uint64_t* d_v, int n, hipStream_t s);
hipError_t launch_debug_sincos(const float* ang, int n, int fused, float* s, float* c, hipStream_t st);

}
```

### orb_slam3_fast_amd/csrc/orbx_kernels.hip

```cpp
#include <type_traits>
#include <map>
#include <mutex>

#include "orbx_device.h"
#include "orbx_introsort.h"
#include "orbx_sincos.h"
#include "orbx_blur_mfma.h"

namespace orbx {

__constant__ int c_umax[16] = {15, 15, 15, 15, 14, 14, 14, 13, 13, 12, 11, 10, 9, 8, 6, 3};

#define RS_DW 256
#define RS_DR 16
#define RS_HROWS 6
struct ResizeLv {
  struct { int w, h, pitch, xcoef, ycoef; } D;
  struct { int w, h; } S;
  int sp, l;
  int nbx;
  const uint8_t* src; long long srcImg;
  uint8_t* dst; long long dstImg;
  const uint32_t* tiles;
  const uint32_t* rows;
// ... 469 lines not shown
      if (lane == sel) v = vf;
      const bool in = lane > f && lane < l;
      const bool stL = in && !less(v, pivot), stR = in && !less(pivot, v);
      const uint64_t mL = __ballot(stL), mR = __ballot(stR);
      const int nL = __popcll(mL), nR = __popcll(mR), nmin = min(nL, nR);
      const int rankL = __popcll(mL & lanemask_lt()), rankR = __popcll(mR & ~(lanemask_lt() | (1ull << lane)));
      const int LiK = __builtin_amdgcn_ds_permute(4 * (stL ? rankL : 63), lane);
      const int RiK = __builtin_amdgcn_ds_permute(4 * (stR ? rankR : 63), lane);
      const int K = __popcll(__ballot(lane < nmin && LiK < RiK));
      const int INF = 1 << 30;
      const int lk = K < nL ? __builtin_amdgcn_readlane(LiK, K) : INF;
      const int rk = K > 0 ? __builtin_amdgcn_readlane(RiK, K - 1) : INF;
      const int cut = min(lk, rk);
      const int pL = __builtin_amdgcn_ds_bpermute(4 * rankL, RiK), pR = __builtin_amdgcn_ds_bpermute(4 * rankR, LiK);
      const int src = (stL && rankL < K) ? pL : ((stR && rankR < K) ? pR : lane);
      const uint32_t nlo = (uint32_t)__builtin_amdgcn_ds_bpermute(4 * src, (int)(uint32_t)v);
      const uint32_t nhi = (uint32_t)__builtin_amdgcn_ds_bpermute(4 * src, (int)(uint32_t)(v >> 32));
      v = ((uint64_t)nhi << 32) | nlo;
      if (l - cut > 16) {
        const uint32_t e = (uint32_t)cut | ((uint32_t)l << 8) | ((uint32_t)d << 16);
        if (sp == 0) stk[0] = e; else if (sp == 1) stk[1] = e; else stk[2] = e;
        ++sp;
      }
      l = cut;
    }
    if (sp == 0) break;
    --sp;
    const uint32_t e = sp == 0 ? stk[0] : (sp == 1 ? stk[1] : stk[2]);
    f = (int)(e & 0xFF);
    l = (int)((e >> 8) & 0xFF);
    d = (int)(e >> 16);
  }
  if (lane < n) a[first + lane] = v;
}

__device__ int partition_reg2(uint64_t* a, int first, int last, uint64_t* box, int lane) {
  const KeyLess less;
  const int n = last - first;
  uint64_t v0 = a[first + lane], v1 = a[first + min(64 + lane, n - 1)];
  const bool in0 = lane >= 1, in1 = 64 + lane < n;
  auto get = [&](int i) { return i < 64 ? readlane_u64(v0, i) : readlane_u64(v1, i - 64); };
  const int mid = n / 2;
  const uint64_t va = get(1), vb = get(mid), vc = get(n - 1);
  int sel;
  if (less(va, vb)) sel = less(vb, vc) ? mid : (less(va, vc) ? n - 1 : 1);
  else if (less(va, vc)) sel = 1;
  else sel = less(vb, vc) ? n - 1 : mid;
  const uint64_t vf = get(0), pivot = get(sel);
  if (lane == 0) v0 = pivot;
  if (sel < 64) {
    if (lane == sel) v0 = vf;
  } else if (lane == sel - 64) {
    v1 = vf;
  }
  const bool stL0 = in0 && !less(v0, pivot), stL1 = in1 && !less(v1, pivot);
  const bool stR0 = in0 && !less(pivot, v0), stR1 = in1 && !less(pivot, v1);
  const uint64_t mL0 = __ballot(stL0), mL1 = __ballot(stL1), mR0 = __ballot(stR0), mR1 = __ballot(stR1);
  const uint64_t lt = lanemask_lt(), gt = ~(lt | (1ull << lane));
  const int belowL0 = __popcll(mL0 & lt), belowL1 = __popcll(mL0) + __popcll(mL1 & lt);
  const int aboveR0 = __popcll(mR0 & gt) + __popcll(mR1), aboveR1 = __popcll(mR1 & gt);
  const bool swL0 = stL0 && aboveR0 > belowL0, swL1 = stL1 && aboveR1 > belowL1;
  const bool swR0 = stR0 && belowL0 > aboveR0, swR1 = stR1 && belowL1 > aboveR1;
  const uint64_t sL0 = __ballot(swL0), sL1 = __ballot(swL1), sR0 = __ballot(swR0), sR1 = __ballot(swR1);
  const uint64_t nsL0 = mL0 & ~sL0, nsL1 = mL1 & ~sL1;
  const int INF = 1 << 30;
  const int lk = nsL0 ? (int)__builtin_ctzll(nsL0) : (nsL1 ? 64 + (int)__builtin_ctzll(nsL1) : INF);
  const int rk = sR0 ? (int)__builtin_ctzll(sR0) : (sR1 ? 64 + (int)__builtin_ctzll(sR1) : INF);
  const int half = n / 2;
  if (swL0) box[belowL0] = v0;
  if (swL1) box[belowL1] = v1;
  if (swR0) box[half + aboveR0] = v0;
  if (swR1) box[half + aboveR1] = v1;
  wsync();
  if (swL0) v0 = box[half + belowL0];
  if (swL1) v1 = box[half + belowL1];
  if (swR0) v0 = box[aboveR0];
  if (swR1) v1 = box[aboveR1];
  a[first + lane] = v0;
  if (in1) a[first + 64 + lane] = v1;
  wsync();
  return first + min(lk, rk);
}

__device__ __forceinline__ void introsort_block(uint64_t* a, int n, uint64_t* tmp, uint16_t* Li, uint16_t* Ri, uint32_t* segs) {
  const int tid = threadIdx.x, lane = tid & 63, wv = tid >> 6, nw = blockDim.x >> 6, nt = blockDim.x;
  const KeyLess less;
#ifdef OCT_PROF
  long long smk[24]; int nsmk = 0;
#define SMK() do { if (nsmk < 24) smk[nsmk++] = wall_clock64(); } while (0)
#else
#define SMK() do {} while (0)
#endif
  SMK();
  if (n > 16) {
    uint32_t* cnt = segs + 512;
    int lg = 0;
    for (int t = n; t > 1; t >>= 1) lg++;
    if (tid == 0) {
      segs[0] = (uint32_t)n << 13 | (uint32_t)(2 * lg) << 26;
      cnt[0] = 1;
      cnt[1] = 0;
    }
    __syncthreads();
    int cur = 0;
    for (;;) {
      const int ns = (int)cnt[cur];
      if (ns == 0) break;
      for (int k = wv; k < ns; k += nw) {
        const uint32_t sg = segs[cur * 256 + k];
        const int first = (int)(sg & 0x1FFF), last = (int)((sg >> 13) & 0x1FFF), depth = (int)(sg >> 26);
        if (last - first <= 64) {
          introsort_seg_reg(a, first, last, depth, lane);
        } else if (depth == 0) {
          if (lane == 0) is_heapsort<uint64_t, KeyLess>(a, first, last, less);
        } else {
          const int cut = last - first <= 128 ? partition_reg2(a, first, last, tmp + first, lane)
                                              : partition_wave(a, first, last, Li + first, Ri + first, lane);
          if (lane == 0) {
            const uint32_t d = (uint32_t)(depth - 1) << 26;
            if (cut - first > 16) segs[(cur ^ 1) * 256 + atomicAdd(&cnt[cur ^ 1], 1u)] = (uint32_t)first | (uint32_t)cut << 13 | d;
            if (last - cut > 16) segs[(cur ^ 1) * 256 + atomicAdd(&cnt[cur ^ 1], 1u)] = (uint32_t)cut | (uint32_t)last << 13 | d;
          }
        }
      }
      SMK();
      __syncthreads();
      if (tid == 0) cnt[cur] = 0;
      cur ^= 1;
      __syncthreads();
      SMK();
    }
  }
  SMK();
  {
    const int per = (4 * n <= nt) ? 4 : ((2 * n <= nt) ? 2 : 1);
    const int chunk = (33 + per - 1) / per;
    for (int i0 = 0; i0 < n * per; i0 += nt) {
      const int t = i0 + tid, i = min(t / per, n - 1), sub = t % per;
      const uint64_t vi = a[i];
      int c = 0;
      const int jb = i - 16 + sub * chunk, je = min(jb + chunk, i + 17);
      for (int j = jb; j < je; j++) {
        const uint64_t vj = a[min(max(j, 0), n - 1)];
        const bool inw = j >= 0 && j < n;
        c += (inw && (less(vj, vi) || (!less(vi, vj) && j < i))) ? 1 : 0;
      }
      if (per >= 2) c += __shfl_xor(c, 1);
      if (per >= 4) c += __shfl_xor(c, 2);
      if (t < n * per && sub == 0) tmp[max(0, i - 16) + c] = vi;
    }
  }
  SMK();
  __syncthreads();
  for (int i = tid; i < n; i += nt) a[i] = tmp[i];
  __syncthreads();
  SMK();
#if defined(OCT_PROF) && !defined(OCT_NO_SORT_PRINT)
  if (tid == 0 && blockIdx.x == 0 && gridDim.x > 1) {
    printf("sort n=%d:", n);
    for (int i = 1; i < nsmk; i++) printf(" %d", (int)(smk[i] - smk[i - 1]));
    printf("  (x10 ns: init | {work, barriers} per round | - | final rank | copy back)\n");
  }
#endif
#undef SMK
}

__global__ __launch_bounds__(512) void k_debug_sort(uint64_t* v, int n) {
  extern __shared__ __attribute__((aligned(16))) uint8_t smem[];
  uint64_t* a = reinterpret_cast<uint64_t*>(smem);
  uint64_t* tmp = a + n;
  uint32_t* segs = reinterpret_cast<uint32_t*>(tmp + n);
  uint16_t* Li = reinterpret_cast<uint16_t*>(segs + 516);
  uint16_t* Ri = Li + n + 4;
  const int tid = threadIdx.x;
  for (int i = tid; i < n; i += blockDim.x) a[i] = v[i];
  __syncthreads();
  if (blockDim.x == 64) introsort_wave(a, n, tmp, Li, Ri, reinterpret_cast<int*>(segs), tid);
  else introsort_block(a, n, tmp, Li, Ri, segs);
  __syncthreads();
  for (int i = tid; i < n; i += blockDim.x) v[i] = a[i];
}
hipError_t launch_debug_sort(uint64_t* d_v, int n, hipStream_t s) {
  const size_t lds = (size_t)n * 16 + 516 * 4 + (size_t)(2 * n + 16) * 2 + 64;
  hipError_t e = hipFuncSetAttribute(reinterpret_cast<const void*>(k_debug_sort),
                                     hipFuncAttributeMaxDynamicSharedMemorySize, (int)lds);
  if (e != hipSuccess) return e;
  static int flip = 0;
  hipLaunchKernelGGL(k_debug_sort, dim3(1), dim3((flip++ & 1) ? 64 : 512), lds, s, d_v, n);
  return hipGetLastError();
}

struct OctLds {
  int nx0[2], nx1[2], ny0[2], ny1[2], ncnt[2];
  int cnt4, cntr, cpos, scan, e[2], mark, bestk, tsum, cellpre;
  int total;
};
__host__ __device__ inline OctLds oct_layout(int maxn, int maxcells, int rep) {
  OctLds o;
  int off = 0;
  auto take = [&](int bytes) {
    int r = off;
    off += (bytes + 7) & ~7;
    return r;
  };
  for (int b = 0; b < 2; b++) {
    o.nx0[b] = take(maxn * 2);
    o.nx1[b] = take(maxn * 2);
    o.ny0[b] = take(maxn * 2);
    o.ny1[b] = take(maxn * 2);
    o.ncnt[b] = take(maxn * 4);
  }
  o.cnt4 = take(maxn * 16 > 4096 ? maxn * 16 : 4096);
  o.cntr = take(maxn * 16 * rep > 16400 ? maxn * 16 * rep : 16400);
  o.scan = take(maxn * 8);
  o.cpos = take(maxn * 8);
  o.e[0] = take(maxn * 8);
  o.e[1] = take(maxn * 8);
  o.mark = take(maxn * 2);
  o.bestk = take(maxn * 4);
  o.tsum = take(256 * 8 + 64);
  o.cellpre = take((maxcells + 1) * 4);
  o.total = off;
  return o;
}
__host__ __device__ inline int oct_maxn(const Geom& g) {
  int q = 0;
  for (int l = 0; l < g.nlevels; l++) q = g.lv[l].quota > q ? g.lv[l].quota : q;
  return q + 4 * kMaxIni + 8;
}
__host__ __device__ inline int oct_maxcells(const Geom& g) {
  int c = 0;
  for (int l = 0; l < g.nlevels; l++) c = g.lv[l].nCols * g.lv[l].nRows > c ? g.lv[l].nCols * g.lv[l].nRows : c;
  return c;
}
__host__ __device__ inline int oct_rep(const Geom& g) {
  const int maxn = oct_maxn(g), maxcells = oct_maxcells(g);
  if (oct_layout(maxn, maxcells, 2).total <= 78 * 1024) return 2;
  return 1;
}
size_t octree_lds_bytes(const Geom& g) { return (size_t)oct_layout(oct_maxn(g), oct_maxcells(g), oct_rep(g)).total; }

constexpr int OCT_NT = 512;
__device__ __forceinline__ uint64_t wave0_scan_u64(uint64_t* v, int n) {
  const int lane = threadIdx.x;
  const uint64_t s = lane < n ? v[lane] : 0;
  const uint64_t incl = wave_scan_dpp_u64(s);
  if (lane < n) v[lane] = incl - s;
  return readlane_u64(incl, 63);
}
__device__ __forceinline__ uint64_t block_scan_u64(uint64_t* v, int n, uint64_t* tsum) {
  const int tid = threadIdx.x, lane = tid & 63, wv = tid >> 6;
  const int per = (n + OCT_NT - 1) / OCT_NT;
  const int b = min(tid * per, n), e = min(b + per, n);
  uint64_t s = 0;
  for (int i = b; i < e; i++) s += v[i];
  const uint64_t incl = wave_scan_dpp_u64(s);
  if (lane == 63) tsum[wv] = incl;
  __syncthreads();
  uint64_t wbase = 0, total = 0;
#pragma unroll
  for (int w = 0; w < OCT_NT / 64; w++) {
    const uint64_t t = tsum[w];
    if (w < wv) wbase += t;
    total += t;
  }
  uint64_t run = wbase + incl - s;
  for (int i = b; i < e; i++) {
    const uint64_t t = v[i];
    v[i] = run;
    run += t;
  }
  __syncthreads();
  return total;
}

__device__ __forceinline__ int quadrant(int x, int y, int x0, int x1, int y0, int y1) {
  const int hx = (x1 - x0 + 1) >> 1, hy = (y1 - y0 + 1) >> 1;
  return (x < x0 + hx ? 0 : 1) | (y < y0 + hy ? 0 : 2);
}

constexpr int OCT_KMAX = 32;
constexpr int OCT_GROUP = 4;
template <bool REG>
struct OctCands {
  uint32_t rk[REG ? OCT_KMAX : 1];
  uint32_t rn2[REG ? OCT_KMAX / 2 : 1];
  uint32_t* keys;
  uint16_t* kn;
  int n;
  static constexpr uint32_t kNoCand = 0xFFFFu;
  template <class F>
  __device__ __forceinline__ void sweep(F f) {
    if constexpr (REG) {
#pragma unroll
      for (int j0 = 0; j0 < OCT_KMAX; j0 += OCT_GROUP) {
        if (j0 * OCT_NT >= n) continue;
#pragma unroll
        for (int j = j0; j < j0 + OCT_GROUP; j++)
        {
          uint32_t key = rk[j], nd = (rn2[j >> 1] >> (16 * (j & 1))) & 0xFFFFu;
          asm volatile("" : "+v"(key), "+v"(nd));
          if (nd != kNoCand) {
            f(0, key, nd);
            rn2[j >> 1] = (j & 1) ? (rn2[j >> 1] & 0xFFFFu) | (nd << 16) : (rn2[j >> 1] & 0xFFFF0000u) | nd;
          }
        }
        __builtin_amdgcn_sched_barrier(0);
      }
    } else {
      for (int k = threadIdx.x; k < n; k += OCT_NT) {
        uint32_t nd = kn[k];
        const uint32_t nd0 = nd;
        f(k, keys[k], nd);
        if (nd != nd0) kn[k] = (uint16_t)nd;
      }
    }
  }
  template <class F>
  __device__ __forceinline__ void fill(F f) {
    if constexpr (REG) {
#pragma unroll
      for (int j = 0; j < OCT_KMAX; j++) {
        const int k = (int)threadIdx.x + j * OCT_NT;
        rk[j] = 0;
        if (k < n) rk[j] = f(k);
      }
#pragma unroll
      for (int j = 0; j < OCT_KMAX; j++) {
        const int k = (int)threadIdx.x + j * OCT_NT;
        const uint32_t nd = k < n ? 0u : kNoCand;
        rn2[j >> 1] = (j & 1) ? rn2[j >> 1] | (nd << 16) : nd;
      }
    } else {
      for (int k = threadIdx.x; k < n; k += OCT_NT) {
        keys[k] = f(k);
        kn[k] = 0;
      }
    }
  }
};

struct OctCtx {
  int16_t *nx0, *nx1, *ny0, *ny1;
  uint32_t* ncnt;
  int nodeStride;
  uint32_t* cnt4;
  int nrep;
  uint32_t* cntr;
  uint16_t* cpos;
  uint64_t* scan;
  uint64_t* ebuf;
  uint16_t* mark;
  uint32_t* nmid;
  uint64_t* tsum;
  int* cellpre;
  int* s_i;
  int maxn;
  uint16_t* owner;
  int ownerBytes;
  uint8_t* tab;
  int tabBytes;
};

template <class CD>
__device__ __forceinline__ void octree_gather(CD& cd, const OctCtx& c, const LevelDev& L, int n, int cells,
                                              const uint32_t* __restrict__ sparse) {
  if (2 * n <= c.ownerBytes) {
    for (int cell = threadIdx.x; cell < cells; cell += OCT_NT) {
      const int b = c.cellpre[cell], e = min(c.cellpre[cell + 1], n);
      for (int i = b; i < e; i++) c.owner[i] = (uint16_t)cell;
    }
    __syncthreads();
    cd.fill([&](int k) {
      const int cell = c.owner[k];
      return sparse[(long long)cell * L.cellCap + (k - c.cellpre[cell])];
    });
    __syncthreads();
  } else {
    cd.fill([&](int k) {
      int lo = 0, hi = cells;
      while (hi - lo > 1) {
        const int mid = (lo + hi) >> 1;
        if (c.cellpre[mid] <= k) lo = mid; else hi = mid;
      }
      return sparse[(long long)lo * L.cellCap + (k - c.cellpre[lo])];
    });
  }
}

template <bool REG>
__device__ __forceinline__ void octree_body(const Geom& g, const LevelDev& L, const OctCtx& c, int n, int cells,
                                            const uint32_t* __restrict__ sparse, uint32_t* __restrict__ keys,
                                            uint16_t* __restrict__ kn, uint32_t* __restrict__ out,
                                            int* __restrict__ outCount, int profLevel) {
  const int tid = threadIdx.x;
#ifdef OCT_PROF
  long long tmk[96]; int nmk = 0;
#define MK() do { if (nmk < 96) tmk[nmk++] = wall_clock64(); } while (0)
#else
#define MK() do {} while (0)
#endif
  MK();
  OctCands<REG> cd;
  cd.keys = keys;
  cd.kn = kn;
  cd.n = n;
  octree_gather(cd, c, L, n, cells, sparse);
  MK();
  const int N = L.quota;
  struct Buf {
    char* base;
    int stride;
    __device__ __forceinline__ int16_t* operator[](int b) const { return reinterpret_cast<int16_t*>(base + b * stride); }
  };
  struct BufU {
    char* base;
    int stride;
    __device__ __forceinline__ uint32_t* operator[](int b) const { return reinterpret_cast<uint32_t*>(base + b * stride); }
  };
  const Buf nx0{(char*)c.nx0, c.nodeStride}, nx1{(char*)c.nx1, c.nodeStride}, ny0{(char*)c.ny0, c.nodeStride},
      ny1{(char*)c.ny1, c.nodeStride};
  const BufU ncnt{(char*)c.ncnt, c.nodeStride};
  uint32_t* cnt4 = c.cnt4;
  uint32_t* cntr = c.cntr;
  const int nrep = c.nrep, rep = tid & (nrep - 1);
  auto zero_counters = [&](int nslots) {
    for (int i = tid; i < nslots * nrep; i += OCT_NT) cntr[i] = 0;
  };
  auto reduce_counters = [&](int nslots) {
    for (int i = tid; i < nslots; i += OCT_NT) {
      uint32_t v = 0;
      for (int r = 0; r < nrep; r++) v += cntr[i * nrep + r];
      cnt4[i] = v;
    }
  };
  uint16_t* cpos = c.cpos;
  uint64_t* scan = c.scan;
  uint16_t* mark = c.mark;
  uint32_t* nmid = c.nmid;
  uint64_t* tsum = c.tsum;
  auto pack_mid = [&](int b, int i) {
    const int x0 = nx0[b][i], x1 = nx1[b][i], y0 = ny0[b][i], y1 = ny1[b][i];
    return (uint32_t)(x0 + ((x1 - x0 + 1) >> 1)) | ((uint32_t)(y0 + ((y1 - y0 + 1) >> 1)) << 12) |
           (ncnt[b][i] > 1 ? 0x80000000u : 0u);
  };
  auto classify = [&](uint32_t key, uint32_t mid) {
    return (key_x(key) >= (int)(mid & 0xFFF) ? 1 : 0) | (key_y(key) >= (int)((mid >> 12) & 0xFFF) ? 2 : 0);
  };
  int* s_i = c.s_i;

  const int W = L.w - 2 * kBorder, H = L.h - 2 * kBorder;
  const int nIni = (int)roundf((float)W / (float)H);
  const float hX = (float)W / (float)nIni;

  zero_counters(kMaxIni);
  __syncthreads();
  cd.sweep([&](int, uint32_t key, uint32_t& nd) {
    const int r = (int)((float)key_x(key) / hX);
    nd = (uint32_t)r;
    atomicAdd(&cntr[r * nrep + rep], 1u);
  });
  __syncthreads();
  reduce_counters(kMaxIni);
  __syncthreads();
  if (tid == 0) {
    int na = 0;
    for (int i = 0; i < nIni; i++) {
      if (cnt4[i] == 0) {
        cpos[i] = 0xFFFF;
        continue;
      }
      nx0[0][na] = (int16_t)(int)(hX * (float)i);
      nx1[0][na] = (int16_t)(int)(hX * (float)(i + 1));
      ny0[0][na] = 0;
      ny1[0][na] = (int16_t)H;
      ncnt[0][na] = cnt4[i];
      cpos[i] = (uint16_t)na;
      na++;
    }
    s_i[0] = na;
    for (int i = 0; i < na; i++) nmid[i] = pack_mid(0, i);
  }
  __syncthreads();
  cd.sweep([&](int, uint32_t, uint32_t& nd) { nd = cpos[nd]; });
  int nA = s_i[0];
  int cur = 0;
  __syncthreads();

  MK();
  bool finish = false;
  int nE = 0, ecur = 0;
  while (!finish) {
    const int prevSize = nA;
    zero_counters(nA * 4);
    __syncthreads();
    MK();
    cd.sweep([&](int, uint32_t key, uint32_t& nd) {
      const uint32_t mid = nmid[nd];
      if (mid >> 31) {
        const int q = classify(key, mid);
        atomicAdd(&cntr[(nd * 4 + q) * nrep + rep], 1u);
        nd |= (uint32_t)q << 14;
      }
    });
    __syncthreads();
    reduce_counters(nA * 4);
    __syncthreads();
    MK();
    for (int i = tid; i < nA; i += OCT_NT) {
      uint64_t cc = 0, nm = 1, ce = 0;
      if (ncnt[cur][i] > 1) {
        nm = 0;
        for (int q = 0; q < 4; q++) {
          cc += cnt4[i * 4 + q] > 0;
          ce += cnt4[i * 4 + q] > 1;
        }
      }
      scan[i] = cc | (nm << 21) | (ce << 42);
    }
    __syncthreads();
    const uint64_t tot = block_scan_u64(scan, nA, tsum);
    MK();
    const int tc = (int)(tot & 0x1FFFFF), tnm = (int)((tot >> 21) & 0x1FFFFF), tce = (int)(tot >> 42);
    const int nxt = cur ^ 1;
    for (int i = tid; i < nA; i += OCT_NT) {
      const uint64_t pre = scan[i];
      const int pc = (int)(pre & 0x1FFFFF), pnm = (int)((pre >> 21) & 0x1FFFFF), pce = (int)(pre >> 42);
      if (ncnt[cur][i] > 1) {
        const int x0 = nx0[cur][i], x1 = nx1[cur][i], y0 = ny0[cur][i], y1 = ny1[cur][i];
        const int hx = (x1 - x0 + 1) >> 1, hy = (y1 - y0 + 1) >> 1;
        int cc = 0;
        for (int q = 0; q < 4; q++) cc += cnt4[i * 4 + q] > 0;
        const int base = tc - (pc + cc);
        int after = 0, eb = pce;
        for (int q = 0; q < 4; q++) {
          const uint32_t cq = cnt4[i * 4 + q];
          if (cq > 1) {
            int rank_after = 0;
            for (int q2 = q + 1; q2 < 4; q2++) rank_after += cnt4[i * 4 + q2] > 0;
            const int cx0 = (q & 1) ? x0 + hx : x0;
            (c.ebuf + ecur * c.maxn)[eb++] = ((uint64_t)cq << 28) | ((uint64_t)(uint32_t)cx0 << 16) | (uint64_t)(base + rank_after);
          }
        }
        for (int q = 3; q >= 0; q--) {
          const uint32_t cq = cnt4[i * 4 + q];
          if (cq == 0) continue;
          const int pos = base + after++;
          nx0[nxt][pos] = (int16_t)((q & 1) ? x0 + hx : x0);
          nx1[nxt][pos] = (int16_t)((q & 1) ? x1 : x0 + hx);
          ny0[nxt][pos] = (int16_t)((q & 2) ? y0 + hy : y0);
          ny1[nxt][pos] = (int16_t)((q & 2) ? y1 : y0 + hy);
          ncnt[nxt][pos] = cq;
          cpos[i * 4 + q] = (uint16_t)pos;
        }
      } else {
        const int pos = tc + pnm;
        nx0[nxt][pos] = nx0[cur][i];
        nx1[nxt][pos] = nx1[cur][i];
        ny0[nxt][pos] = ny0[cur][i];
        ny1[nxt][pos] = ny1[cur][i];
        ncnt[nxt][pos] = ncnt[cur][i];
        cpos[i * 4] = (uint16_t)pos;
      }
    }
    __syncthreads();
    MK();
    cd.sweep([&](int, uint32_t, uint32_t& v) { v = cpos[(v & 0x3FFF) * 4 + (v >> 14)]; });
    for (int i = tid; i < tc + tnm; i += OCT_NT) nmid[i] = pack_mid(nxt, i);
    __syncthreads();
    MK();
    cur = nxt;
    nA = tc + tnm;
    nE = tce;
    if (nA >= N || nA == prevSize) {
      finish = true;
    } else if (nA + 3 * nE > N) {
      break;
    }
  }

  MK();
  while (!finish) {
    const int prevSize = nA;
    uint64_t* E = c.ebuf + ecur * c.maxn;
    uint64_t* E2 = c.ebuf + (ecur ^ 1) * c.maxn;
    introsort_block(E, nE, E2, reinterpret_cast<uint16_t*>(scan), reinterpret_cast<uint16_t*>(scan) + c.maxn + 4,
                    reinterpret_cast<uint32_t*>(tsum));
    MK();
    if (tid == 0) {
      s_i[1] = nE;
      s_i[2] = 0;
    }
    zero_counters(nA * 4);
    for (int i = tid; i < nA; i += OCT_NT) {
      mark[i] = 0;
      nmid[i] &= 0x7FFFFFFFu;
    }
    __syncthreads();
    for (int m = tid; m < nE; m += OCT_NT) {
      const int nd = (int)(E[nE - 1 - m] & 0xFFFF);
      mark[nd] = (uint16_t)(m + 1);
      nmid[nd] |= 0x80000000u;
    }
    __syncthreads();
    cd.sweep([&](int, uint32_t key, uint32_t& nd) {
      const uint32_t mid = nmid[nd];
      if (mid >> 31) {
        const int q = classify(key, mid);
        atomicAdd(&cntr[(nd * 4 + q) * nrep + rep], 1u);
        nd |= (uint32_t)q << 14;
      }
    });
    __syncthreads();
    reduce_counters(nA * 4);
    __syncthreads();
    for (int m = tid; m < nE; m += OCT_NT) {
      const int nd = (int)(E[nE - 1 - m] & 0xFFFF);
      uint64_t cc = 0, ce = 0;
      for (int q = 0; q < 4; q++) {
        cc += cnt4[nd * 4 + q] > 0;
        ce += cnt4[nd * 4 + q] > 1;
      }
      scan[m] = cc | (ce << 21);
    }
    __syncthreads();
    block_scan_u64(scan, nE, tsum);
    for (int m = tid; m < nE; m += OCT_NT) {
      const int nd = (int)(E[nE - 1 - m] & 0xFFFF);
      int cc = 0;
      for (int q = 0; q < 4; q++) cc += cnt4[nd * 4 + q] > 0;
      const int cincl = (int)(scan[m] & 0x1FFFFF) + cc;
      if (nA + cincl - (m + 1) >= N) {
        atomicMin(&s_i[1], m + 1);
        s_i[2] = 1;
      }
    }
    __syncthreads();
    const int nP = s_i[1];
    const bool broke = s_i[2] != 0;
    int tc, tce;
    if (nP < nE) {
      tc = (int)(scan[nP] & 0x1FFFFF);
      tce = (int)(scan[nP] >> 21);
    } else {
      const int nd = (int)(E[0] & 0xFFFF);
      int cc = 0, ce = 0;
      for (int q = 0; q < 4; q++) {
        cc += cnt4[nd * 4 + q] > 0;
        ce += cnt4[nd * 4 + q] > 1;
      }
      tc = nE ? (int)(scan[nE - 1] & 0x1FFFFF) + cc : 0;
      tce = nE ? (int)(scan[nE - 1] >> 21) + ce : 0;
    }
    const int nxt = cur ^ 1;
    for (int m = tid; m < nP; m += OCT_NT) {
      const int nd = (int)(E[nE - 1 - m] & 0xFFFF);
      const int x0 = nx0[cur][nd], x1 = nx1[cur][nd], y0 = ny0[cur][nd], y1 = ny1[cur][nd];
      const int hx = (x1 - x0 + 1) >> 1, hy = (y1 - y0 + 1) >> 1;
      int cc = 0;
      for (int q = 0; q < 4; q++) cc += cnt4[nd * 4 + q] > 0;
      const int pc = (int)(scan[m] & 0x1FFFFF);
      int eb = (int)(scan[m] >> 21);
      const int base = tc - (pc + cc);
      for (int q = 0; q < 4; q++) {
        const uint32_t cq = cnt4[nd * 4 + q];
        if (cq > 1) {
          int rank_after = 0;
          for (int q2 = q + 1; q2 < 4; q2++) rank_after += cnt4[nd * 4 + q2] > 0;
          const int cx0 = (q & 1) ? x0 + hx : x0;
          E2[eb++] = ((uint64_t)cq << 28) | ((uint64_t)(uint32_t)cx0 << 16) | (uint64_t)(base + rank_after);
        }
      }
      int after = 0;
      for (int q = 3; q >= 0; q--) {
        const uint32_t cq = cnt4[nd * 4 + q];
        if (cq == 0) continue;
        const int pos = base + after++;
        nx0[nxt][pos] = (int16_t)((q & 1) ? x0 + hx : x0);
        nx1[nxt][pos] = (int16_t)((q & 1) ? x1 : x0 + hx);
        ny0[nxt][pos] = (int16_t)((q & 2) ? y0 + hy : y0);
        ny1[nxt][pos] = (int16_t)((q & 2) ? y1 : y0 + hy);
        ncnt[nxt][pos] = cq;
        cpos[nd * 4 + q] = (uint16_t)pos;
      }
    }
    __syncthreads();
    for (int i = tid; i < nA; i += OCT_NT) scan[i] = (mark[i] == 0 || mark[i] > nP) ? 1 : 0;
    __syncthreads();
    const int nKeep = (int)block_scan_u64(scan, nA, tsum);
    for (int i = tid; i < nA; i += OCT_NT) {
      if (mark[i] == 0 || mark[i] > nP) {
        const int pos = tc + (int)scan[i];
        nx0[nxt][pos] = nx0[cur][i];
        nx1[nxt][pos] = nx1[cur][i];
        ny0[nxt][pos] = ny0[cur][i];
        ny1[nxt][pos] = ny1[cur][i];
        ncnt[nxt][pos] = ncnt[cur][i];
        cpos[i * 4] = cpos[i * 4 + 1] = cpos[i * 4 + 2] = cpos[i * 4 + 3] = (uint16_t)pos;
      }
    }
    __syncthreads();
    cd.sweep([&](int, uint32_t, uint32_t& v) { v = cpos[(v & 0x3FFF) * 4 + (v >> 14)]; });
    for (int i = tid; i < tc + nKeep; i += OCT_NT) nmid[i] = pack_mid(nxt, i);
    __syncthreads();
    cur = nxt;
    nA = tc + nKeep;
    nE = tce;
    ecur ^= 1;
    MK();
    if (broke || nA == prevSize) finish = true;
  }

  MK();
  uint64_t* best = scan;
  uint64_t* bestr = reinterpret_cast<uint64_t*>(cntr);
  const int nrepB = nrep >= 2 ? nrep * 2 : 1, repB = tid & (nrepB - 1);
  if (nrepB > 1)
    for (int i = tid; i < nA * nrepB; i += OCT_NT) bestr[i] = 0;
  else
    for (int i = tid; i < nA; i += OCT_NT) best[i] = 0;
  __syncthreads();
  const float invH = 1.0f / (float)L.hCell, invW = 1.0f / (float)L.wCell;
  auto rank_key = [&](uint32_t key) {
    const int xr = key_x(key) - 3, yr = key_y(key) - 3;
    const int cy = (int)(((float)yr + 0.5f) * invH), cx = (int)(((float)xr + 0.5f) * invW);
    const uint32_t rank = (uint32_t)(((cy * L.nCols + cx) * L.hCell + (yr - cy * L.hCell)) * L.wCell + (xr - cx * L.wCell));
    return ((unsigned long long)key_r(key) << 32) | (0xFFFFFFFFu - rank);
  };
  if (nrepB > 1) {
    cd.sweep([&](int, uint32_t key, uint32_t& nd) {
      atomicMax((unsigned long long*)&bestr[nd * nrepB + repB], rank_key(key));
    });
    __syncthreads();
    for (int i = tid; i < nA; i += OCT_NT) {
      uint64_t v = 0;
      for (int r = 0; r < nrepB; r++) v = bestr[i * nrepB + r] > v ? bestr[i * nrepB + r] : v;
      best[i] = v;
    }
  } else {
    cd.sweep([&](int, uint32_t key, uint32_t& nd) { atomicMax((unsigned long long*)&best[nd], rank_key(key)); });
  }
  __syncthreads();
  const int nOut = min(nA, L.selCap);
  cd.sweep([&](int, uint32_t key, uint32_t& nd) {
    if ((int)nd < nOut && best[nd] == rank_key(key)) out[nd] = pack_key(key_x(key) + kBorder, key_y(key) + kBorder, key_r(key));
  });
  if (tid == 0) *outCount = nOut;
  MK();
#ifdef OCT_PROF
  if (tid == 0 && profLevel) {
    printf("n=%d nA=%d :", n, nA);
    for (int i = 1; i < nmk; i++) printf(" %d", (int)(tmk[i] - tmk[i - 1]));
    printf("\n");
  }
#endif
#undef MK
}

constexpr int OCT_HD = 5;
__host__ __device__ inline int oct_hbase(int nIni, int d) { return nIni * (((1 << (2 * d)) - 1) / 3); }
__host__ __device__ inline bool oct_hist_fits(int nIni) {
  return nIni <= 2 && oct_hbase(nIni, OCT_HD + 1) * 6 <= 16400 && nIni * (1 << (2 * OCT_HD)) * 2 <= 4096;
}

__device__ __forceinline__ bool octree_hist_body(const Geom& g, const LevelDev& L, const OctCtx& c, int n, int cells,
                                                 const uint32_t* __restrict__ sparse, uint32_t* __restrict__ keys,
                                                 uint32_t* __restrict__ out, int* __restrict__ outCount, int prof) {
  const int tid = threadIdx.x;
#ifdef OCT_PROF
  long long hmk[48]; int nhmk = 0;
#define HMK() do { if (nhmk < 48) hmk[nhmk++] = wall_clock64(); } while (0)
#else
#define HMK() do {} while (0)
#endif
  HMK();
  OctCands<true> cd;
  cd.keys = keys;
  cd.kn = nullptr;
  cd.n = n;
  octree_gather(cd, c, L, n, cells, sparse);
  HMK();
  const int N = L.quota;
  struct Buf {
    char* base;
    int stride;
    __device__ __forceinline__ int16_t* operator[](int b) const { return reinterpret_cast<int16_t*>(base + b * stride); }
  };
  struct BufU {
    char* base;
    int stride;
    __device__ __forceinline__ uint32_t* operator[](int b) const { return reinterpret_cast<uint32_t*>(base + b * stride); }
  };
  const Buf nx0{(char*)c.nx0, c.nodeStride}, nx1{(char*)c.nx1, c.nodeStride}, ny0{(char*)c.ny0, c.nodeStride},
      ny1{(char*)c.ny1, c.nodeStride};
  const BufU ncnt{(char*)c.ncnt, c.nodeStride};
  const int W = L.w - 2 * kBorder, H = L.h - 2 * kBorder;
  const int nIni = (int)roundf((float)W / (float)H);
  const float hX = (float)W / (float)nIni;
  uint32_t* hist = c.cntr;
  uint16_t* leafAt = reinterpret_cast<uint16_t*>(hist + oct_hbase(nIni, OCT_HD + 1));
  uint16_t* t5 = reinterpret_cast<uint16_t*>(c.cnt4);
  uint16_t* ndcBuf = c.cpos;
  auto ndc = [&](int b) { return ndcBuf + b * c.maxn; };
  uint64_t* scan = c.scan;
  uint16_t* mark = c.mark;
  uint64_t* tsum = c.tsum;
  int* s_i = c.s_i;
  const int nH = oct_hbase(nIni, OCT_HD + 1);
  for (int i = tid; i < nH; i += OCT_NT) hist[i] = 0;
  if (tid == 0) s_i[3] = 0;
  const bool pathTab = 2 * (W + H) + 8 <= c.tabBytes;
  uint16_t* px = reinterpret_cast<uint16_t*>(c.tab);
  uint16_t* py = px + ((W + 3) & ~3);
  auto x_path = [&](int x) {
    const int r = (int)((float)x / hX);
    int x0 = (int)(hX * (float)r), x1 = (int)(hX * (float)(r + 1));
    uint32_t code = (uint32_t)r;
#pragma unroll
    for (int d = 0; d < OCT_HD; d++) {
      const int mx = x0 + ((x1 - x0 + 1) >> 1);
      const int qx = x >= mx;
      x0 = qx ? mx : x0;
      x1 = qx ? x1 : mx;
      code = code * 4 + (uint32_t)qx;
    }
    return code;
  };
  auto y_path = [&](int y) {
    int y0 = 0, y1 = H;
    uint32_t code = 0;
#pragma unroll
    for (int d = 0; d < OCT_HD; d++) {
      const int my = y0 + ((y1 - y0 + 1) >> 1);
      const int qy = y >= my;
      y0 = qy ? my : y0;
      y1 = qy ? y1 : my;
      code = code * 4 + (uint32_t)(qy << 1);
    }
    return code;
  };
  if (pathTab) {
    for (int i = tid; i < W + H; i += OCT_NT) {
      if (i < W) px[i] = (uint16_t)x_path(i);
      else py[i - W] = (uint16_t)y_path(i - W);
    }
  }
  __syncthreads();
  {
    uint32_t* h5 = hist + oct_hbase(nIni, OCT_HD);
    if (pathTab) {
      cd.sweep([&](int, uint32_t key, uint32_t& nd) {
        const uint32_t code = (uint32_t)px[key_x(key)] + (uint32_t)py[key_y(key)];
        nd = code;
        atomicAdd(&h5[code], 1u);
      });
    } else {
      cd.sweep([&](int, uint32_t key, uint32_t& nd) {
        const uint32_t code = x_path(key_x(key)) + y_path(key_y(key));
        nd = code;
        atomicAdd(&h5[code], 1u);
      });
    }
  }
  __syncthreads();
  HMK();
  for (int d = OCT_HD - 1; d >= 0; d--) {
    const uint32_t* ch = hist + oct_hbase(nIni, d + 1);
    uint32_t* pa = hist + oct_hbase(nIni, d);
    for (int i = tid; i < (nIni << (2 * d)); i += OCT_NT) pa[i] = ch[4 * i] + ch[4 * i + 1] + ch[4 * i + 2] + ch[4 * i + 3];
    __syncthreads();
  }
  auto child_count = [&](uint32_t dc, int q) {
    const int d = (int)(dc >> 13);
    return hist[oct_hbase(nIni, d + 1) + (int)(dc & 0x1FFF) * 4 + q];
  };
  if (tid == 0) {
    int na = 0;
    for (int i = 0; i < nIni; i++) {
      if (hist[i] == 0) continue;
      nx0[0][na] = (int16_t)(int)(hX * (float)i);
      nx1[0][na] = (int16_t)(int)(hX * (float)(i + 1));
      ny0[0][na] = 0;
      ny1[0][na] = (int16_t)H;
      ncnt[0][na] = hist[i];
      ndc(0)[na] = (uint16_t)i;
      na++;
    }
    s_i[0] = na;
  }
  __syncthreads();
  int nA = s_i[0];
  int cur = 0;
  bool finish = false;
  int nE = 0, ecur = 0;
  HMK();
  auto pass = [&](auto waveTag) -> int {
    constexpr bool kWave = decltype(waveTag)::value;
    auto sync = [&]() {
      if (kWave) {
        __builtin_amdgcn_fence(__ATOMIC_ACQ_REL, "workgroup");
        __builtin_amdgcn_wave_barrier();
      } else {
        __syncthreads();
      }
    };
    const int prevSize = nA;
      for (int i = tid; i < nA; i += OCT_NT) {
        uint64_t cc = 0, nm = 1, ce = 0;
        if (ncnt[cur][i] > 1) {
          nm = 0;
          const uint32_t dc = ndc(cur)[i];
          if ((dc >> 13) >= (uint32_t)OCT_HD) {
            s_i[3] = 1;
          } else {
            for (int q = 0; q < 4; q++) {
              const uint32_t cq = child_count(dc, q);
              cc += cq > 0;
              ce += cq > 1;
            }
          }
        }
        scan[i] = cc | (nm << 21) | (ce << 42);
      }
      sync();
      if (s_i[3]) return 3;
      const uint64_t tot = kWave ? wave0_scan_u64(scan, nA) : block_scan_u64(scan, nA, tsum);
      const int tc = (int)(tot & 0x1FFFFF), tnm = (int)((tot >> 21) & 0x1FFFFF), tce = (int)(tot >> 42);
      const int nxt = cur ^ 1;
      for (int i = tid; i < nA; i += OCT_NT) {
        const uint64_t pre = scan[i];
        const int pc = (int)(pre & 0x1FFFFF), pnm = (int)((pre >> 21) & 0x1FFFFF), pce = (int)(pre >> 42);
        if (ncnt[cur][i] > 1) {
          const uint32_t dc = ndc(cur)[i];
          const uint32_t cdc = (((dc >> 13) + 1) << 13) | ((dc & 0x1FFF) * 4);
          const int x0 = nx0[cur][i], x1 = nx1[cur][i], y0 = ny0[cur][i], y1 = ny1[cur][i];
          const int hx = (x1 - x0 + 1) >> 1, hy = (y1 - y0 + 1) >> 1;
          uint32_t cq4[4];
          int cc = 0;
          for (int q = 0; q < 4; q++) {
            cq4[q] = child_count(dc, q);
            cc += cq4[q] > 0;
          }
          const int base = tc - (pc + cc);
          int after = 0, eb = pce;
          for (int q = 0; q < 4; q++) {
            if (cq4[q] > 1) {
              int rank_after = 0;
              for (int q2 = q + 1; q2 < 4; q2++) rank_after += cq4[q2] > 0;
              const int cx0 = (q & 1) ? x0 + hx : x0;
              (c.ebuf + ecur * c.maxn)[eb++] = ((uint64_t)cq4[q] << 28) | ((uint64_t)(uint32_t)cx0 << 16) | (uint64_t)(base + rank_after);
            }
          }
          for (int q = 3; q >= 0; q--) {
            if (cq4[q] == 0) continue;
            const int pos = base + after++;
            nx0[nxt][pos] = (int16_t)((q & 1) ? x0 + hx : x0);
            nx1[nxt][pos] = (int16_t)((q & 1) ? x1 : x0 + hx);
            ny0[nxt][pos] = (int16_t)((q & 2) ? y0 + hy : y0);
            ny1[nxt][pos] = (int16_t)((q & 2) ? y1 : y0 + hy);
            ncnt[nxt][pos] = cq4[q];
            ndc(nxt)[pos] = (uint16_t)(cdc + q);
          }
        } else {
          const int pos = tc + pnm;
          nx0[nxt][pos] = nx0[cur][i];
          nx1[nxt][pos] = nx1[cur][i];
          ny0[nxt][pos] = ny0[cur][i];
          ny1[nxt][pos] = ny1[cur][i];
          ncnt[nxt][pos] = ncnt[cur][i];
          ndc(nxt)[pos] = ndc(cur)[i];
        }
      }
    sync();
    cur = nxt;
    nA = tc + tnm;
    nE = tce;
    if (nA >= N || nA == prevSize) return 1;
    if (nA + 3 * nE > N) return 2;
    return 0;
  };
  int state = 0;
  if (nA <= 64) {
    if (tid < 64) {
      while (state == 0 && nA <= 64) state = pass(std::true_type{});
      if (tid == 0) {
        s_i[4] = state;
        s_i[5] = nA;
        s_i[6] = nE;
        s_i[7] = cur;
      }
    }
    __syncthreads();
    state = s_i[4];
    nA = s_i[5];
    nE = s_i[6];
    cur = s_i[7];
  }
  while (state == 0) state = pass(std::false_type{});
  if (state == 3) return false;
  finish = state == 1;
  HMK();
  while (!finish) {
    const int prevSize = nA;
    uint64_t* E = c.ebuf + ecur * c.maxn;
    uint64_t* E2 = c.ebuf + (ecur ^ 1) * c.maxn;
    introsort_block(E, nE, E2, reinterpret_cast<uint16_t*>(scan), reinterpret_cast<uint16_t*>(scan) + c.maxn + 4,
                    reinterpret_cast<uint32_t*>(tsum));
    HMK();
    if (tid == 0) {
      s_i[1] = nE;
      s_i[2] = 0;
    }
    for (int i = tid; i < nA; i += OCT_NT) mark[i] = 0;
    __syncthreads();
    for (int m = tid; m < nE; m += OCT_NT) {
      const int nd = (int)(E[nE - 1 - m] & 0xFFFF);
      mark[nd] = (uint16_t)(m + 1);
      const uint32_t dc = ndc(cur)[nd];
      uint64_t cc = 0, ce = 0;
      if ((dc >> 13) >= (uint32_t)OCT_HD) {
        s_i[3] = 1;
      } else {
        for (int q = 0; q < 4; q++) {
          const uint32_t cq = child_count(dc, q);
          cc += cq > 0;
          ce += cq > 1;
        }
      }
      scan[m] = cc | (ce << 21);
    }
    __syncthreads();
    if (s_i[3]) return false;
    block_scan_u64(scan, nE, tsum);
    for (int m = tid; m < nE; m += OCT_NT) {
      const int nd = (int)(E[nE - 1 - m] & 0xFFFF);
      const uint32_t dc = ndc(cur)[nd];
      int cc = 0;
      for (int q = 0; q < 4; q++) cc += child_count(dc, q) > 0;
      const int cincl = (int)(scan[m] & 0x1FFFFF) + cc;
      if (nA + cincl - (m + 1) >= N) {
        atomicMin(&s_i[1], m + 1);
        s_i[2] = 1;
      }
    }
    __syncthreads();
    const int nP = s_i[1];
    const bool broke = s_i[2] != 0;
    int tc, tce;
    if (nP < nE) {
      tc = (int)(scan[nP] & 0x1FFFFF);
      tce = (int)(scan[nP] >> 21);
    } else {
      int cc = 0, ce = 0;
      if (nE) {
        const uint32_t dc = ndc(cur)[(int)(E[0] & 0xFFFF)];
        for (int q = 0; q < 4; q++) {
          const uint32_t cq = child_count(dc, q);
          cc += cq > 0;
          ce += cq > 1;
        }
      }
      tc = nE ? (int)(scan[nE - 1] & 0x1FFFFF) + cc : 0;
      tce = nE ? (int)(scan[nE - 1] >> 21) + ce : 0;
    }
    const int nxt = cur ^ 1;
    for (int m = tid; m < nP; m += OCT_NT) {
      const int nd = (int)(E[nE - 1 - m] & 0xFFFF);
      const uint32_t dc = ndc(cur)[nd];
      const uint32_t cdc = (((dc >> 13) + 1) << 13) | ((dc & 0x1FFF) * 4);
      const int x0 = nx0[cur][nd], x1 = nx1[cur][nd], y0 = ny0[cur][nd], y1 = ny1[cur][nd];
      const int hx = (x1 - x0 + 1) >> 1, hy = (y1 - y0 + 1) >> 1;
      uint32_t cq4[4];
      int cc = 0;
      for (int q = 0; q < 4; q++) {
        cq4[q] = child_count(dc, q);
        cc += cq4[q] > 0;
      }
      const int pc = (int)(scan[m] & 0x1FFFFF);
      int eb = (int)(scan[m] >> 21);
      const int base = tc - (pc + cc);
      for (int q = 0; q < 4; q++) {
        if (cq4[q] > 1) {
          int rank_after = 0;
          for (int q2 = q + 1; q2 < 4; q2++) rank_after += cq4[q2] > 0;
          const int cx0 = (q & 1) ? x0 + hx : x0;
          E2[eb++] = ((uint64_t)cq4[q] << 28) | ((uint64_t)(uint32_t)cx0 << 16) | (uint64_t)(base + rank_after);
        }
      }
      int after = 0;
      for (int q = 3; q >= 0; q--) {
        if (cq4[q] == 0) continue;
        const int pos = base + after++;
        nx0[nxt][pos] = (int16_t)((q & 1) ? x0 + hx : x0);
        nx1[nxt][pos] = (int16_t)((q & 1) ? x1 : x0 + hx);
        ny0[nxt][pos] = (int16_t)((q & 2) ? y0 + hy : y0);
        ny1[nxt][pos] = (int16_t)((q & 2) ? y1 : y0 + hy);
        ncnt[nxt][pos] = cq4[q];
        ndc(nxt)[pos] = (uint16_t)(cdc + q);
      }
    }
    __syncthreads();
    for (int i = tid; i < nA; i += OCT_NT) scan[i] = (mark[i] == 0 || mark[i] > nP) ? 1 : 0;
    __syncthreads();
    const int nKeep = (int)block_scan_u64(scan, nA, tsum);
    for (int i = tid; i < nA; i += OCT_NT) {
      if (mark[i] == 0 || mark[i] > nP) {
        const int pos = tc + (int)scan[i];
        nx0[nxt][pos] = nx0[cur][i];
        nx1[nxt][pos] = nx1[cur][i];
        ny0[nxt][pos] = ny0[cur][i];
        ny1[nxt][pos] = ny1[cur][i];
        ncnt[nxt][pos] = ncnt[cur][i];
        ndc(nxt)[pos] = ndc(cur)[i];
      }
    }
    __syncthreads();
    cur = nxt;
    nA = tc + nKeep;
    nE = tce;
    ecur ^= 1;
    if (broke || nA == prevSize) finish = true;
    HMK();
  }
  for (int i = tid; i < nH; i += OCT_NT) leafAt[i] = 0xFFFF;
  __syncthreads();
  for (int i = tid; i < nA; i += OCT_NT) {
    const uint32_t dc = ndc(cur)[i];
    leafAt[oct_hbase(nIni, (int)(dc >> 13)) + (int)(dc & 0x1FFF)] = (uint16_t)i;
  }
  __syncthreads();
  for (int c5 = tid; c5 < (nIni << (2 * OCT_HD)); c5 += OCT_NT) {
    uint16_t v = 0xFFFF;
#pragma unroll
    for (int d = OCT_HD; d >= 0; d--) {
      const uint16_t w = leafAt[oct_hbase(nIni, d) + (c5 >> (2 * (OCT_HD - d)))];
      v = v == 0xFFFF ? w : v;
    }
    t5[c5] = v;
  }
  __syncthreads();
  HMK();
  uint64_t* best = scan;
  uint64_t* bestr = reinterpret_cast<uint64_t*>(c.cntr);
  const int nrepB = c.nrep >= 2 ? c.nrep * 2 : 1, repB = tid & (nrepB - 1);
  if (nrepB > 1)
    for (int i = tid; i < nA * nrepB; i += OCT_NT) bestr[i] = 0;
  else
    for (int i = tid; i < nA; i += OCT_NT) best[i] = 0;
  __syncthreads();
  const float invH = 1.0f / (float)L.hCell, invW = 1.0f / (float)L.wCell;
  auto rank_key = [&](uint32_t key) {
    const int xr = key_x(key) - 3, yr = key_y(key) - 3;
    const int cy = (int)(((float)yr + 0.5f) * invH), cx = (int)(((float)xr + 0.5f) * invW);
    const uint32_t rank = (uint32_t)(((cy * L.nCols + cx) * L.hCell + (yr - cy * L.hCell)) * L.wCell + (xr - cx * L.wCell));
    return ((unsigned long long)key_r(key) << 32) | (0xFFFFFFFFu - rank);
  };
  cd.sweep([&](int, uint32_t key, uint32_t& nd) {
    const uint32_t fn = t5[nd];
    if (nrepB > 1) atomicMax((unsigned long long*)&bestr[fn * nrepB + repB], rank_key(key));
    else atomicMax((unsigned long long*)&best[fn], rank_key(key));
  });
  __syncthreads();
  const int nOut = min(nA, L.selCap);
  for (int i = tid; i < nOut; i += OCT_NT) {
    uint64_t v = nrepB > 1 ? 0 : best[i];
    if (nrepB > 1)
      for (int r = 0; r < nrepB; r++) v = bestr[i * nrepB + r] > v ? bestr[i * nrepB + r] : v;
    const uint32_t rank = 0xFFFFFFFFu - (uint32_t)v, resp = (uint32_t)(v >> 32);
    const uint32_t xloc = rank % (uint32_t)L.wCell, t1 = rank / (uint32_t)L.wCell;
    const uint32_t yloc = t1 % (uint32_t)L.hCell, t2 = t1 / (uint32_t)L.hCell;
    const uint32_t cx = t2 % (uint32_t)L.nCols, cy = t2 / (uint32_t)L.nCols;
    out[i] = pack_key((int)(cx * L.wCell + xloc) + 3 + kBorder, (int)(cy * L.hCell + yloc) + 3 + kBorder, (int)resp);
  }
  if (tid == 0) *outCount = nOut;
  HMK();
#ifdef OCT_PROF
  if (tid == 0 && prof) {
    printf("hist n=%d nA=%d :", n, nA);
    for (int i = 1; i < nhmk; i++) printf(" %d", (int)(hmk[i] - hmk[i - 1]));
    printf("  (x10 ns: gather | sweep1 | sums+roots | phase 1 | {sort, rest} per phase-2 round | leaf table | best sweeps)\n");
  }
#endif
#undef HMK
  return true;
}

__global__ __launch_bounds__(OCT_NT, 4) void k_octree(Geom g, const uint32_t* __restrict__ cellCand,
                                                const int* __restrict__ cellCount, int* __restrict__ cellPrefix,
                                                uint32_t* __restrict__ cand, int* __restrict__ candCount,
                                                uint16_t* __restrict__ knode, uint32_t* __restrict__ sel,
                                                int* __restrict__ selCount, int profLevel, int forceGlobal, int level0,
                                                int nlv) {
  extern __shared__ __attribute__((aligned(16))) uint8_t smem[];
  __shared__ int s_i[8];
  const int tid = threadIdx.x;
#ifdef OCT_WG_PROF
  struct WgPrint {
    long long t0;
    int l, img, on;
    __device__ ~WgPrint() {
      if (on) printf("octwg level %d img %d start %lld end %lld\n", l, img, t0 % 100000000, wall_clock64() % 100000000);
    }
  } wgPrint{wall_clock64(), 0, 0, (int)(threadIdx.x == 0)};
#endif
  const int nimg_ = gridDim.x / nlv;
  const int l = level0 + blockIdx.x / nimg_, img = blockIdx.x % nimg_;
#ifdef OCT_WG_PROF
  wgPrint.l = l;
  wgPrint.img = img;
#endif
  const LevelDev L = g.lv[l];
  const int maxn = oct_maxn(g);
  const int nrep = oct_rep(g);
  const OctLds o = oct_layout(maxn, oct_maxcells(g), nrep);
  OctCtx c;
  c.nx0 = (int16_t*)(smem + o.nx0[0]);
  c.nx1 = (int16_t*)(smem + o.nx1[0]);
  c.ny0 = (int16_t*)(smem + o.ny0[0]);
  c.ny1 = (int16_t*)(smem + o.ny1[0]);
  c.ncnt = (uint32_t*)(smem + o.ncnt[0]);
  c.nodeStride = o.nx0[1] - o.nx0[0];
  c.ebuf = (uint64_t*)(smem + o.e[0]);
  c.cnt4 = (uint32_t*)(smem + o.cnt4);
  c.cntr = (uint32_t*)(smem + o.cntr);
  c.nrep = nrep;
  c.cpos = (uint16_t*)(smem + o.cpos);
  c.scan = (uint64_t*)(smem + o.scan);
  c.mark = (uint16_t*)(smem + o.mark);
  c.nmid = (uint32_t*)(smem + o.bestk);
  c.tsum = (uint64_t*)(smem + o.tsum);
  c.cellpre = (int*)(smem + o.cellpre);
  c.s_i = s_i;
  c.maxn = maxn;
  c.owner = (uint16_t*)smem;
  c.ownerBytes = o.tsum;
  c.tab = smem + o.cpos;
  c.tabBytes = o.tsum - o.cpos;

  const int cells = L.nCols * L.nRows;
  int n;
  {
    const int* cc = cellCount + (long long)img * g.totalCells + L.cellStart;
    const int per = (cells + OCT_NT - 1) / OCT_NT;
    const int cb = min(tid * per, cells), ce = min(cb + per, cells);
    int sum = 0;
    for (int ci = cb; ci < ce; ci++) sum += cc[ci];
    const int incl = wave_scan_dpp(sum);
    if ((tid & 63) == 63) c.tsum[tid >> 6] = (uint64_t)incl;
    __syncthreads();
    int wbase = 0, total = 0;
#pragma unroll
    for (int w = 0; w < OCT_NT / 64; w++) {
      const int t = (int)c.tsum[w];
      if (w < (tid >> 6)) wbase += t;
      total += t;
    }
    n = min(total, L.candCap);
    int run = wbase + incl - sum;
    for (int ci = cb; ci < ce; ci++) {
      c.cellpre[ci] = run;
      run += cc[ci];
    }
    if (tid == 0) {
      c.cellpre[cells] = total;
      candCount[img * g.nlevels + l] = n;
    }
    __syncthreads();
  }
  const uint32_t* sparse = cellCand + (long long)img * g.cellImg + L.cellOff;
  uint32_t* keys = cand + (long long)img * g.candImg + L.candOff;
  uint16_t* kn = knode + (long long)img * g.candImg + L.candOff;
  uint32_t* out = sel + (long long)img * g.selImg + L.selOff;
  int* outCount = selCount + img * g.nlevels + l;
  if (n <= OCT_KMAX * OCT_NT && forceGlobal != 1) {
    const int W = L.w - 2 * kBorder, H = L.h - 2 * kBorder;
    const int nIni = (int)roundf((float)W / (float)H);
    bool done = false;
    if (forceGlobal == 0 && oct_hist_fits(nIni)) {
      done = octree_hist_body(g, L, c, n, cells, sparse, keys, out, outCount, profLevel == l && img == 0);
      __syncthreads();
    }
    if (!done) octree_body<true>(g, L, c, n, cells, sparse, keys, kn, out, outCount, profLevel == l && img == 0);
  } else {
    octree_body<false>(g, L, c, n, cells, sparse, keys, kn, out, outCount, profLevel == l && img == 0);
  }
}

static int g_octree_force_global_host = 0;
void debug_set_octree_global(int on) { g_octree_force_global_host = on < 0 ? 0 : (on > 2 ? 2 : on); }

hipError_t launch_octree(const Geom& g, int nimg, const uint32_t* cellCand, const int* cellCount, int* cellPrefix,
                         uint32_t* cand, int* candCount, uint16_t* knode, uint32_t* sel, int* selCount, int level0,
                         int level1, hipStream_t s) {
  if (level1 <= level0) return hipSuccess;
  dim3 grid((level1 - level0) * nimg);
#ifdef OCT_PROF
  static const int profLevel = getenv("ORBX_OCTREE_PROF_LEVEL") ? atoi(getenv("ORBX_OCTREE_PROF_LEVEL")) : 0;
#else
  const int profLevel = -1;
#endif
  hipLaunchKernelGGL(k_octree, grid, dim3(OCT_NT), octree_lds_bytes(g), s, g, cellCand, cellCount, cellPrefix, cand,
                     candCount, knode, sel, selCount, profLevel, g_octree_force_global_host, level0, level1 - level0);
  return hipGetLastError();
}

__device__ __forceinline__ int reflect101(int p, int n) {
  if (p < 0) p = -p;
  if (p >= n) p = 2 * n - 2 - p;
  return p;
}

#define BL_TW 128
#define BL_TH 32
template <bool T440>
__global__ __launch_bounds__(256) void k_blur(Geom g, Pyr p, int level0, int level1, int xcdRun) {
  constexpr uint32_t kT2 = T440 ? 49u : 48u, kT3 = T440 ? 55u : 56u;
  __shared__ uint32_t in[BL_TH + 6][BL_TW / 4 + 2 + 1];
  __shared__ uint32_t hp[(BL_TH + 6) / 2][BL_TW + 1];
  const int tid = threadIdx.x;
  const int img = blockIdx.z;
  int tile = xcd_run_remap_rt(blockIdx.x, gridDim.x, blockIdx.z, xcdRun);
  int l = level0;
  for (;; l++) {
    const int tx = (g.lv[l].w + BL_TW - 1) / BL_TW, ty = (g.lv[l].h + BL_TH - 1) / BL_TH;
    if (tile < tx * ty || l + 1 == level1) break;
    tile -= tx * ty;
  }
  const LevelDev L = g.lv[l];
  const int tx = (L.w + BL_TW - 1) / BL_TW;
  if (tile >= tx * ((L.h + BL_TH - 1) / BL_TH)) return;
  const int x0 = (tile % tx) * BL_TW, y0 = (tile / tx) * BL_TH;
  const int bodyEnd = T440 && g.cv440 > 1 ? (L.w & ~(g.cv440 - 1)) : 0;
  int pitch;
  const uint8_t* im = level_ptr(g, p, img, l, pitch);
  constexpr int IW = BL_TW / 4 + 2;
  if (x0 >= 4 && y0 >= 3 && x0 + BL_TW + 4 <= L.w && y0 + BL_TH + 3 <= L.h) {
    const int c = tid % IW, r0 = tid / IW;
    if (r0 < 7) {
      const uint8_t* src = im + (long long)(y0 - 3 + r0) * pitch + (x0 - 4) + 4 * c;
#pragma unroll
      for (int k = 0; k < 6; k++) {
        const int r = r0 + 7 * k;
        if (r < BL_TH + 6) in[r][c] = *reinterpret_cast<const uint32_t*>(src + (long long)(7 * k) * pitch);
      }
    }
  } else {
    for (int i = tid; i < (BL_TH + 6) * IW; i += 256) {
      const int r = i / IW, c = i - r * IW;
      const int y = y0 + r - 3, x = x0 - 4 + 4 * c;
      uint32_t v;
      if (y >= 0 && y < L.h && x >= 0 && x + 4 <= L.w) {
        v = *reinterpret_cast<const uint32_t*>(im + (long long)y * pitch + x);
      } else {
        const int yy = reflect101(min(max(y, -3), L.h + 2), L.h);
        v = 0;
#pragma unroll
        for (int k = 0; k < 4; k++) {
          const int xx = reflect101(min(max(x + k, -3), L.w + 2), L.w);
          v |= (uint32_t)im[(long long)yy * pitch + xx] << (8 * k);
        }
      }
      in[r][c] = v;
    }
  }
  __syncthreads();
  for (int i = tid; i < ((BL_TH + 6) / 2) * (BL_TW / 4); i += 256) {
    const int j = i / (BL_TW / 4), c = i - j * (BL_TW / 4);
    uint32_t h[2][4];
#pragma unroll
    for (int rr = 0; rr < 2; rr++) {
      const uint32_t Lw = in[2 * j + rr][c], C = in[2 * j + rr][c + 1], R = in[2 * j + rr][c + 2];
      const uint32_t wA = 18u | (34u << 8) | (kT2 << 16) | (kT3 << 24), wB = kT2 | (34u << 8) | (18u << 16);
      h[rr][0] = __builtin_amdgcn_udot4(__builtin_amdgcn_alignbyte(C, Lw, 1), wA,
                                        __builtin_amdgcn_udot4(__builtin_amdgcn_alignbyte(R, C, 1), wB, 0, false), false);
      h[rr][1] = __builtin_amdgcn_udot4(__builtin_amdgcn_alignbyte(C, Lw, 2), wA,
                                        __builtin_amdgcn_udot4(__builtin_amdgcn_alignbyte(R, C, 2), wB, 0, false), false);
      h[rr][2] = __builtin_amdgcn_udot4(__builtin_amdgcn_alignbyte(C, Lw, 3), wA,
                                        __builtin_amdgcn_udot4(__builtin_amdgcn_alignbyte(R, C, 3), wB, 0, false), false);
      h[rr][3] = __builtin_amdgcn_udot4(C, wA, __builtin_amdgcn_udot4(R, wB, 0, false), false);
    }
#pragma unroll
    for (int k = 0; k < 4; k++) hp[j][32 * k + c] = h[0][k] | (h[1][k] << 16);
  }
  __syncthreads();
  {
    const int bc = tid & 31, br = tid >> 5;
// ... 482 lines not shown
      uint32_t v = __builtin_bit_cast(uint32_t, kx);
      v = lane == 1 ? __builtin_bit_cast(uint32_t, ky) : v;
      v = lane == 2 ? __builtin_bit_cast(uint32_t, L.patch) : v;
      v = lane == 3 ? __builtin_bit_cast(uint32_t, angle) : v;
      v = lane == 4 ? __builtin_bit_cast(uint32_t, (float)key_r(keyk)) : v;
      v = lane == 5 ? (uint32_t)l : v;
      v = lane == 6 ? 0xFFFFFFFFu : v;
      pendKp = v;
      pendSlot = n_out_slot;
    }
  }
  store_pending();
}

static DescPlan make_desc_plan(const Geom& g, int nimg) {
  DescPlan dp{};
  dp.nk = (int)std::min<long long>(8, std::max<long long>(1, (long long)nimg * g.selImg / 12288));
  int tks = 0;
  for (int l = 0; l < ORBX_MAX_LEVELS; l++) {
    dp.taskOff[l] = l < g.nlevels ? tks : 0x7fffffff;
    if (l < g.nlevels) tks += (g.lv[l].selCap + dp.nk - 1) / dp.nk;
  }
  dp.tasks = tks;
  const uint64_t d = (uint64_t)tks, m = (1ull << 32) / d + 1, e = m * d - (1ull << 32), jmax = (uint64_t)nimg * d;
  dp.magic = (d > 1 && m < (1ull << 32) && jmax * e < (1ull << 32)) ? (unsigned)m : 0u;
  return dp;
}

hipError_t launch_describe(const Geom& g, const Pyr& p, int nimg, const uint32_t* sel, const int* selCount,
                           const int* slot, orbx_keypoint* kps, uint8_t* desc, int* nOut, int* mono, hipStream_t s) {
  const DescPlan dp = make_desc_plan(g, nimg);
  const dim3 grid(dp.tasks, nimg), block(64);
  if (g.cv440) hipLaunchKernelGGL(k_describe<true>, grid, block, 0, s, g, p, dp, sel, selCount, slot, kps, desc, nOut, mono, nimg >= 8 ? 1 : 0);
  else hipLaunchKernelGGL(k_describe<false>, grid, block, 0, s, g, p, dp, sel, selCount, slot, kps, desc, nOut, mono, nimg >= 8 ? 1 : 0);
  return hipGetLastError();
}

__global__ __launch_bounds__(256) void k_result_pack(ResultPack a) {
  const int sec = blockIdx.y;
  if (!((a.mask >> sec) & 1)) return;
  if (sec == 6) {
    if (blockIdx.x == 0 && threadIdx.x < 2) {
      const int t = threadIdx.x;
      a.hCnt[t] = t < a.nimg ? (uint32_t)a.nOut[t] : 0u;
      a.hCnt[2 + t] = t < a.nimg ? (uint32_t)a.mono[t] : 0u;
    }
    return;
  }
  const int img = sec < 4 ? (sec & 1) : 0;
  if (img >= a.nimg || (sec >= 4 && !a.stereo)) return;
  const int n = (sec >= 4 && a.fixedN >= 0) ? min(a.fixedN, a.cap) : min(a.nOut[img], a.cap);
  const uint32_t* src;
  uint32_t* dst;
  int len;
  if (sec < 2) {
    src = a.kps + (size_t)img * a.cap * 7; dst = a.hKps + (size_t)img * a.cap * 7; len = n * 7;
  } else if (sec < 4) {
    src = a.desc + (size_t)img * a.cap * 8; dst = a.hDesc + (size_t)img * a.cap * 8; len = n * 8;
  } else {
    src = sec == 4 ? a.uR : a.depth; dst = sec == 4 ? a.hUr : a.hDepth; len = n;
  }
  for (int i = blockIdx.x * 256 + threadIdx.x; i < len; i += gridDim.x * 256) dst[i] = src[i];
}
hipError_t launch_result_pack(const ResultPack& a, hipStream_t s) {
  hipLaunchKernelGGL(k_result_pack, dim3(12, 7), dim3(256), 0, s, a);
  return hipGetLastError();
}

hipError_t raise_dynamic_lds(const void* fn, size_t bytes) {
  static std::mutex mu;
  static std::map<std::pair<int, const void*>, size_t> high;
  int dev = 0;
  hipError_t e = hipGetDevice(&dev);
  if (e != hipSuccess) return e;
  std::lock_guard<std::mutex> lk(mu);
  size_t& h = high[{dev, fn}];
  if (bytes <= h) return hipSuccess;
  e = hipFuncSetAttribute(fn, hipFuncAttributeMaxDynamicSharedMemorySize, (int)bytes);
  if (e == hipSuccess) h = bytes;
  return e;
}

hipError_t prepare_kernels(const Geom& g) {
  hipError_t e = raise_dynamic_lds(reinterpret_cast<const void*>(k_octree), octree_lds_bytes(g));
  if (e != hipSuccess) return e;
  if (g.nlevels > 1) {
    e = raise_dynamic_lds(reinterpret_cast<const void*>(k_resize<0, true>), std::max<size_t>(resize_lds_bytes(g), 1024));
    if (e != hipSuccess) return e;
    e = raise_dynamic_lds(reinterpret_cast<const void*>(k_resize<kResizeNdw, true>), std::max<size_t>(resize_lds_bytes(g), 1024));
    if (e != hipSuccess) return e;
  }
  return prepare_detect(g);
}

__global__ void k_debug_sincos(const float* __restrict__ ang, int n, int fused, float* __restrict__ s, float* __restrict__ c) {
  const int i = blockIdx.x * blockDim.x + threadIdx.x;
  if (i >= n) return;
  float sv, cv;
  if (fused) glibc_sincosf<true>(ang[i], sv, cv);
  else glibc_sincosf<false>(ang[i], sv, cv);
  s[i] = sv;
  c[i] = cv;
}
hipError_t launch_debug_sincos(const float* ang, int n, int fused, float* s, float* c, hipStream_t st) {
  hipLaunchKernelGGL(k_debug_sincos, dim3((n + 255) / 256), dim3(256), 0, st, ang, n, fused, s, c);
  return hipGetLastError();
}

void debug_introsort_host(uint64_t* v, int n) { introsort<uint64_t, KeyLess>(v, n, KeyLess()); }

}
```

Before: 83710 stereo frames/s.

## Size octree block threads per pyramid level with a mixed-class launch

Templates the octree distribution kernel on its thread count and adds a mixed kernel that launches 512 threads per block but lets each level use only 128, 256 or 512 of them, chosen from that level's area. Small pyramid levels then run their scans, sorts and sweeps with fewer threads, cutting idle-thread and barrier cost. Threads beyond the chosen count exit early, yet the block still holds full-size LDS and launch resources. The mixed path is taken only when the image count exceeds the latency threshold; otherwise the 512-thread kernel runs as before.

```diff
diff --git a/include/orbx.h b/include/orbx.h
--- a/include/orbx.h
+++ b/include/orbx.h
@@ -769,6 +769,8 @@
 
 void orbx_debug_set_detect_list_cap(int cap);
 void orbx_debug_set_octree_global(int on);
+void orbx_debug_set_octree_class(int nt);
+int orbx_debug_octree_plan(const orbx_params* p, int width, int height, int32_t* nt_per_level, int32_t* lds_bytes_per_level);
 void orbx_debug_set_stereo_direct(int max_pairs);
 int orbx_debug_upload_results(orbx_extractor* ex, int image, const orbx_keypoint* kps, const uint8_t* desc, int n, int mono_index);
 void orbx_debug_set_clahe_cell_kernel(int on);
diff --git a/orb_slam3_fast_amd/__init__.py b/orb_slam3_fast_amd/__init__.py
--- a/orb_slam3_fast_amd/__init__.py
+++ b/orb_slam3_fast_amd/__init__.py
@@ -202,6 +202,10 @@
         L.orbx_debug_set_detect_list_cap.restype = None
         L.orbx_debug_set_octree_global.argtypes = [i]
         L.orbx_debug_set_octree_global.restype = None
+        if hasattr(L, "orbx_debug_set_octree_class"):
+            L.orbx_debug_set_octree_class.argtypes = [i]
+            L.orbx_debug_set_octree_class.restype = None
+            L.orbx_debug_octree_plan.argtypes = [vp, i, i, vp, vp]
         L.orbx_debug_set_stereo_direct.argtypes = [i]
         L.orbx_debug_set_stereo_direct.restype = None
         L.orbx_debug_set_clahe_cell_kernel.argtypes = [i]
@@ -1634,6 +1638,13 @@
     return cells, tiles, int(info[2]), int(info[3])
 
 
+def octree_plan(nfeatures, scaleFactor, nlevels, iniThFAST, minThFAST, width, height):
+    prm = _Params(int(nfeatures), float(scaleFactor), int(nlevels), int(iniThFAST), int(minThFAST))
+    nt, lds = np.zeros(int(nlevels), np.int32), np.zeros(int(nlevels), np.int32)
+    _check(lib().orbx_debug_octree_plan(C.byref(prm), width, height, _p(nt), _p(lds)))
+    return nt, lds
+
+
 class ORBVocabulary:
 
     def __init__(self, k=None, L=None, parent=None, is_leaf=None, desc=None, weight=None, scoring=0, weighting=0, path=None,
diff --git a/orb_slam3_fast_amd/csrc/orbx_api.hip b/orb_slam3_fast_amd/csrc/orbx_api.hip
--- a/orb_slam3_fast_amd/csrc/orbx_api.hip
+++ b/orb_slam3_fast_amd/csrc/orbx_api.hip
@@ -156,7 +156,7 @@
     why = "scale factor too large for the LDS-staged resize footprint";
     return ORBX_E_UNSUPPORTED;
   }
-  if (octree_lds_bytes(g) > 160 * 1024 - 2048) {
+  if (octree_lds_bytes(g, 0, g.nlevels) > 160 * 1024 - 2048) {
     why = "nfeatures too large for the LDS-resident quadtree";
     return ORBX_E_UNSUPPORTED;
   }
@@ -475,6 +475,7 @@
     build_cell_records(g, recs);
     HIPC(hipMemcpy(ex->d_cellRec.p, recs.data(), recs.size() * sizeof(CellRec), hipMemcpyHostToDevice));
   }
+  build_octree_plan(g, ex->octPlan);
   HIPC(prepare_kernels(g));
   std::vector<TailPlan> plans;
   std::vector<TailBand> bands;
@@ -663,8 +664,14 @@
   }
   {
     StageTimer t(ex, s, ORBX_STAGE_OCTREE);
-    HIPC(launch_octree(g, n, ex->d_cellCand.p, ex->d_cellCount.p, ex->d_cellPrefix.p, ex->d_cand.p,
-                       ex->d_candCount.p, ex->d_knode.p, ex->d_sel.p, ex->d_selCount.p, 0, g.nlevels, s));
+    const int forced = debug_octree_class();
+    if (!forced && n > g_lat_max_images) {
+      HIPC(launch_octree_mixed(g, ex->octPlan, n, ex->d_cellCand.p, ex->d_cellCount.p, ex->d_cand.p, ex->d_candCount.p,
+                               ex->d_knode.p, ex->d_sel.p, ex->d_selCount.p, s));
+    } else {
+      HIPC(launch_octree(g, n, ex->d_cellCand.p, ex->d_cellCount.p, ex->d_cellPrefix.p, ex->d_cand.p, ex->d_candCount.p,
+                         ex->d_knode.p, ex->d_sel.p, ex->d_selCount.p, 0, g.nlevels, forced ? forced : 512, s));
+    }
   }
   if (!lapTrivial) {
     StageTimer t(ex, s, ORBX_STAGE_SLOTS);
@@ -1443,6 +1450,26 @@
   return ORBX_OK;
 }
 
+int orbx_debug_octree_plan(const orbx_params* p, int width, int height, int32_t* nt_per_level, int32_t* lds_bytes_per_level) {
+  if (!p || !nt_per_level || !lds_bytes_per_level || width < 1 || height < 1 || p->nlevels < 1 || p->nlevels > ORBX_MAX_LEVELS ||
+      p->nfeatures < 1 || !(p->scale_factor > 1.0f))
+    return fail(ORBX_E_BADARG, "bad argument");
+  std::unique_ptr<orbx_extractor> ex(new orbx_extractor());
+  ex->prm = *p;
+  build_tables(ex.get());
+  Geom g;
+  std::string why;
+  const int rc = build_geom(ex.get(), width, height, g, why);
+  if (rc != ORBX_OK) return fail(rc, why);
+  OctPlan op;
+  build_octree_plan(g, op);
+  for (int l = 0; l < g.nlevels; l++) {
+    nt_per_level[l] = op.nt[l];
+    lds_bytes_per_level[l] = op.lds[l];
+  }
+  return ORBX_OK;
+}
+
 int orbx_hamming256(const void* a, const void* b) {
   const uint32_t* x = (const uint32_t*)a;
   const uint32_t* y = (const uint32_t*)b;
@@ -1739,6 +1766,7 @@
 void orbx_debug_set_clahe_cell_kernel(int on) { debug_set_clahe_cell_kernel(on); }
 void orbx_debug_set_remap_lds(int on) { debug_set_remap_lds(on); }
 void orbx_debug_set_octree_global(int on) { debug_set_octree_global(on); }
+void orbx_debug_set_octree_class(int nt) { debug_set_octree_class(nt); }
 void orbx_debug_set_stereo_direct(int max_pairs) { debug_set_stereo_direct(max_pairs); }
 void orbx_debug_set_resize_tail(int first_level, int max_levels, int band_rows) {
   orbx_host::g_tail_first = first_level;
diff --git a/orb_slam3_fast_amd/csrc/orbx_host.h b/orb_slam3_fast_amd/csrc/orbx_host.h
--- a/orb_slam3_fast_amd/csrc/orbx_host.h
+++ b/orb_slam3_fast_amd/csrc/orbx_host.h
@@ -353,6 +353,7 @@
   DevBuf<uint4> d_xtab;
   DevBuf<uint32_t> d_rsRec;
   DevBuf<orbx::CellRec> d_cellRec;
+  orbx::OctPlan octPlan{};
   DevBuf<int> d_packCtr;
   uint32_t packSeq = 0;
   bool packCtrDirty = false;
diff --git a/orb_slam3_fast_amd/csrc/orbx_internal.h b/orb_slam3_fast_amd/csrc/orbx_internal.h
--- a/orb_slam3_fast_amd/csrc/orbx_internal.h
+++ b/orb_slam3_fast_amd/csrc/orbx_internal.h
@@ -122,13 +122,19 @@
                          int level0, int level1, uint8_t* dbgScore, hipStream_t s);
 hipError_t launch_octree(const Geom& g, int nimg, const uint32_t* cellCand, const int* cellCount, int* cellPrefix,
                          uint32_t* cand, int* candCount, uint16_t* knode, uint32_t* sel, int* selCount, int level0,
-                         int level1, hipStream_t s);
+                         int level1, int nt, hipStream_t s);
+struct OctPlan {
+  int nt[ORBX_MAX_LEVELS], lds[ORBX_MAX_LEVELS];
+};
+void build_octree_plan(const Geom& g, OctPlan& p);
+hipError_t launch_octree_mixed(const Geom& g, const OctPlan& plan, int nimg, const uint32_t* cellCand, const int* cellCount,
+                               uint32_t* cand, int* candCount, uint16_t* knode, uint32_t* sel, int* selCount, hipStream_t s);
 hipError_t launch_blur(const Geom& g, const Pyr& p, int nimg, int level0, int level1, hipStream_t s);
 hipError_t launch_slots(const Geom& g, int nimg, const uint32_t* sel, const int* selCount, const int* lap,
                         int* slot, int* nOut, int* mono, hipStream_t s);
 hipError_t launch_describe(const Geom& g, const Pyr& p, int nimg, const uint32_t* sel, const int* selCount,
                            const int* slot, orbx_keypoint* kps, uint8_t* desc, int* nOut, int* mono, hipStream_t s);
-size_t octree_lds_bytes(const Geom& g);
+size_t octree_lds_bytes(const Geom& g, int level0, int level1);
 size_t resize_lds_bytes(const Geom& g);
 
 struct StereoArgs {
@@ -508,6 +514,8 @@
 void debug_set_detect_list_cap(int cap);
 void debug_set_clahe_cell_kernel(int on);
 void debug_set_octree_global(int on);
+void debug_set_octree_class(int nt);
+int debug_octree_class();
 hipError_t launch_debug_sort(uint64_t* d_v, int n, hipStream_t s);
 hipError_t launch_debug_sincos(const float* ang, int n, int fused, float* s, float* c, hipStream_t st);
 
diff --git a/orb_slam3_fast_amd/csrc/orbx_kernels.hip b/orb_slam3_fast_amd/csrc/orbx_kernels.hip
--- a/orb_slam3_fast_amd/csrc/orbx_kernels.hip
+++ b/orb_slam3_fast_amd/csrc/orbx_kernels.hip
@@ -575,8 +575,8 @@
   return first + min(lk, rk);
 }
 
-__device__ __forceinline__ void introsort_block(uint64_t* a, int n, uint64_t* tmp, uint16_t* Li, uint16_t* Ri, uint32_t* segs) {
-  const int tid = threadIdx.x, lane = tid & 63, wv = tid >> 6, nw = blockDim.x >> 6, nt = blockDim.x;
+__device__ __forceinline__ void introsort_block(uint64_t* a, int n, uint64_t* tmp, uint16_t* Li, uint16_t* Ri, uint32_t* segs, int nt) {
+  const int tid = threadIdx.x, lane = tid & 63, wv = tid >> 6, nw = nt >> 6;
   const KeyLess less;
 #ifdef OCT_PROF
   long long smk[24]; int nsmk = 0;
@@ -669,7 +669,7 @@
   for (int i = tid; i < n; i += blockDim.x) a[i] = v[i];
   __syncthreads();
   if (blockDim.x == 64) introsort_wave(a, n, tmp, Li, Ri, reinterpret_cast<int*>(segs), tid);
-  else introsort_block(a, n, tmp, Li, Ri, segs);
+  else introsort_block(a, n, tmp, Li, Ri, segs, (int)blockDim.x);
   __syncthreads();
   for (int i = tid; i < n; i += blockDim.x) v[i] = a[i];
 }
@@ -716,24 +716,25 @@
   o.total = off;
   return o;
 }
-__host__ __device__ inline int oct_maxn(const Geom& g) {
+__host__ __device__ inline int oct_maxn(const Geom& g, int l0, int l1) {
   int q = 0;
-  for (int l = 0; l < g.nlevels; l++) q = g.lv[l].quota > q ? g.lv[l].quota : q;
+  for (int l = l0; l < l1; l++) q = g.lv[l].quota > q ? g.lv[l].quota : q;
   return q + 4 * kMaxIni + 8;
 }
-__host__ __device__ inline int oct_maxcells(const Geom& g) {
+__host__ __device__ inline int oct_maxcells(const Geom& g, int l0, int l1) {
   int c = 0;
-  for (int l = 0; l < g.nlevels; l++) c = g.lv[l].nCols * g.lv[l].nRows > c ? g.lv[l].nCols * g.lv[l].nRows : c;
+  for (int l = l0; l < l1; l++) c = g.lv[l].nCols * g.lv[l].nRows > c ? g.lv[l].nCols * g.lv[l].nRows : c;
   return c;
 }
-__host__ __device__ inline int oct_rep(const Geom& g) {
-  const int maxn = oct_maxn(g), maxcells = oct_maxcells(g);
+__host__ __device__ inline int oct_rep(const Geom& g, int l0, int l1) {
+  const int maxn = oct_maxn(g, l0, l1), maxcells = oct_maxcells(g, l0, l1);
   if (oct_layout(maxn, maxcells, 2).total <= 78 * 1024) return 2;
   return 1;
 }
-size_t octree_lds_bytes(const Geom& g) { return (size_t)oct_layout(oct_maxn(g), oct_maxcells(g), oct_rep(g)).total; }
-
-constexpr int OCT_NT = 512;
+size_t octree_lds_bytes(const Geom& g, int l0, int l1) {
+  return (size_t)oct_layout(oct_maxn(g, l0, l1), oct_maxcells(g, l0, l1), oct_rep(g, l0, l1)).total;
+}
+
 __device__ __forceinline__ uint64_t wave0_scan_u64(uint64_t* v, int n) {
   const int lane = threadIdx.x;
   const uint64_t s = lane < n ? v[lane] : 0;
@@ -741,9 +742,10 @@
   if (lane < n) v[lane] = incl - s;
   return readlane_u64(incl, 63);
 }
+template <int NT>
 __device__ __forceinline__ uint64_t block_scan_u64(uint64_t* v, int n, uint64_t* tsum) {
   const int tid = threadIdx.x, lane = tid & 63, wv = tid >> 6;
-  const int per = (n + OCT_NT - 1) / OCT_NT;
+  const int per = (n + NT - 1) / NT;
   const int b = min(tid * per, n), e = min(b + per, n);
   uint64_t s = 0;
   for (int i = b; i < e; i++) s += v[i];
@@ -752,7 +754,7 @@
   __syncthreads();
   uint64_t wbase = 0, total = 0;
 #pragma unroll
-  for (int w = 0; w < OCT_NT / 64; w++) {
+  for (int w = 0; w < NT / 64; w++) {
     const uint64_t t = tsum[w];
     if (w < wv) wbase += t;
     total += t;
@@ -774,7 +776,7 @@
 
 constexpr int OCT_KMAX = 32;
 constexpr int OCT_GROUP = 4;
-template <bool REG>
+template <bool REG, int NT>
 struct OctCands {
   uint32_t rk[REG ? OCT_KMAX : 1];
   uint32_t rn2[REG ? OCT_KMAX / 2 : 1];
@@ -787,7 +789,7 @@
     if constexpr (REG) {
 #pragma unroll
       for (int j0 = 0; j0 < OCT_KMAX; j0 += OCT_GROUP) {
-        if (j0 * OCT_NT >= n) continue;
+        if (j0 * NT >= n) continue;
 #pragma unroll
         for (int j = j0; j < j0 + OCT_GROUP; j++)
         {
@@ -801,7 +803,7 @@
         __builtin_amdgcn_sched_barrier(0);
       }
     } else {
-      for (int k = threadIdx.x; k < n; k += OCT_NT) {
+      for (int k = threadIdx.x; k < n; k += NT) {
         uint32_t nd = kn[k];
         const uint32_t nd0 = nd;
         f(k, keys[k], nd);
@@ -814,18 +816,18 @@
     if constexpr (REG) {
 #pragma unroll
       for (int j = 0; j < OCT_KMAX; j++) {
-        const int k = (int)threadIdx.x + j * OCT_NT;
+        const int k = (int)threadIdx.x + j * NT;
         rk[j] = 0;
         if (k < n) rk[j] = f(k);
       }
 #pragma unroll
       for (int j = 0; j < OCT_KMAX; j++) {
-        const int k = (int)threadIdx.x + j * OCT_NT;
+        const int k = (int)threadIdx.x + j * NT;
         const uint32_t nd = k < n ? 0u : kNoCand;
         rn2[j >> 1] = (j & 1) ? rn2[j >> 1] | (nd << 16) : nd;
       }
     } else {
-      for (int k = threadIdx.x; k < n; k += OCT_NT) {
+      for (int k = threadIdx.x; k < n; k += NT) {
         keys[k] = f(k);
         kn[k] = 0;
       }
@@ -855,11 +857,11 @@
   int tabBytes;
 };
 
-template <class CD>
+template <int NT, class CD>
 __device__ __forceinline__ void octree_gather(CD& cd, const OctCtx& c, const LevelDev& L, int n, int cells,
                                               const uint32_t* __restrict__ sparse) {
   if (2 * n <= c.ownerBytes) {
-    for (int cell = threadIdx.x; cell < cells; cell += OCT_NT) {
+    for (int cell = threadIdx.x; cell < cells; cell += NT) {
       const int b = c.cellpre[cell], e = min(c.cellpre[cell + 1], n);
       for (int i = b; i < e; i++) c.owner[i] = (uint16_t)cell;
     }
@@ -881,7 +883,7 @@
   }
 }
 
-template <bool REG>
+template <bool REG, int NT>
 __device__ __forceinline__ void octree_body(const Geom& g, const LevelDev& L, const OctCtx& c, int n, int cells,
                                             const uint32_t* __restrict__ sparse, uint32_t* __restrict__ keys,
                                             uint16_t* __restrict__ kn, uint32_t* __restrict__ out,
@@ -894,11 +896,11 @@
 #define MK() do {} while (0)
 #endif
   MK();
-  OctCands<REG> cd;
+  OctCands<REG, NT> cd;
   cd.keys = keys;
   cd.kn = kn;
   cd.n = n;
-  octree_gather(cd, c, L, n, cells, sparse);
+  octree_gather<NT>(cd, c, L, n, cells, sparse);
   MK();
   const int N = L.quota;
   struct Buf {
@@ -918,10 +920,10 @@
   uint32_t* cntr = c.cntr;
   const int nrep = c.nrep, rep = tid & (nrep - 1);
   auto zero_counters = [&](int nslots) {
-    for (int i = tid; i < nslots * nrep; i += OCT_NT) cntr[i] = 0;
+    for (int i = tid; i < nslots * nrep; i += NT) cntr[i] = 0;
   };
   auto reduce_counters = [&](int nslots) {
-    for (int i = tid; i < nslots; i += OCT_NT) {
+    for (int i = tid; i < nslots; i += NT) {
       uint32_t v = 0;
       for (int r = 0; r < nrep; r++) v += cntr[i * nrep + r];
       cnt4[i] = v;
@@ -1000,7 +1002,7 @@
     reduce_counters(nA * 4);
     __syncthreads();
     MK();
-    for (int i = tid; i < nA; i += OCT_NT) {
+    for (int i = tid; i < nA; i += NT) {
       uint64_t cc = 0, nm = 1, ce = 0;
       if (ncnt[cur][i] > 1) {
         nm = 0;
@@ -1012,11 +1014,11 @@
       scan[i] = cc | (nm << 21) | (ce << 42);
     }
     __syncthreads();
-    const uint64_t tot = block_scan_u64(scan, nA, tsum);
+    const uint64_t tot = block_scan_u64<NT>(scan, nA, tsum);
     MK();
     const int tc = (int)(tot & 0x1FFFFF), tnm = (int)((tot >> 21) & 0x1FFFFF), tce = (int)(tot >> 42);
     const int nxt = cur ^ 1;
-    for (int i = tid; i < nA; i += OCT_NT) {
+    for (int i = tid; i < nA; i += NT) {
       const uint64_t pre = scan[i];
       const int pc = (int)(pre & 0x1FFFFF), pnm = (int)((pre >> 21) & 0x1FFFFF), pce = (int)(pre >> 42);
       if (ncnt[cur][i] > 1) {
@@ -1059,7 +1061,7 @@
     __syncthreads();
     MK();
     cd.sweep([&](int, uint32_t, uint32_t& v) { v = cpos[(v & 0x3FFF) * 4 + (v >> 14)]; });
-    for (int i = tid; i < tc + tnm; i += OCT_NT) nmid[i] = pack_mid(nxt, i);
+    for (int i = tid; i < tc + tnm; i += NT) nmid[i] = pack_mid(nxt, i);
     __syncthreads();
     MK();
     cur = nxt;
@@ -1078,19 +1080,19 @@
     uint64_t* E = c.ebuf + ecur * c.maxn;
     uint64_t* E2 = c.ebuf + (ecur ^ 1) * c.maxn;
     introsort_block(E, nE, E2, reinterpret_cast<uint16_t*>(scan), reinterpret_cast<uint16_t*>(scan) + c.maxn + 4,
-                    reinterpret_cast<uint32_t*>(tsum));
+                    reinterpret_cast<uint32_t*>(tsum), NT);
     MK();
     if (tid == 0) {
       s_i[1] = nE;
       s_i[2] = 0;
     }
     zero_counters(nA * 4);
-    for (int i = tid; i < nA; i += OCT_NT) {
+    for (int i = tid; i < nA; i += NT) {
       mark[i] = 0;
       nmid[i] &= 0x7FFFFFFFu;
     }
     __syncthreads();
-    for (int m = tid; m < nE; m += OCT_NT) {
+    for (int m = tid; m < nE; m += NT) {
       const int nd = (int)(E[nE - 1 - m] & 0xFFFF);
       mark[nd] = (uint16_t)(m + 1);
       nmid[nd] |= 0x80000000u;
@@ -1107,7 +1109,7 @@
     __syncthreads();
     reduce_counters(nA * 4);
     __syncthreads();
-    for (int m = tid; m < nE; m += OCT_NT) {
+    for (int m = tid; m < nE; m += NT) {
       const int nd = (int)(E[nE - 1 - m] & 0xFFFF);
       uint64_t cc = 0, ce = 0;
       for (int q = 0; q < 4; q++) {
@@ -1117,8 +1119,8 @@
       scan[m] = cc | (ce << 21);
     }
     __syncthreads();
-    block_scan_u64(scan, nE, tsum);
-    for (int m = tid; m < nE; m += OCT_NT) {
+    block_scan_u64<NT>(scan, nE, tsum);
+    for (int m = tid; m < nE; m += NT) {
       const int nd = (int)(E[nE - 1 - m] & 0xFFFF);
       int cc = 0;
       for (int q = 0; q < 4; q++) cc += cnt4[nd * 4 + q] > 0;
@@ -1146,7 +1148,7 @@
       tce = nE ? (int)(scan[nE - 1] >> 21) + ce : 0;
     }
     const int nxt = cur ^ 1;
-    for (int m = tid; m < nP; m += OCT_NT) {
+    for (int m = tid; m < nP; m += NT) {
       const int nd = (int)(E[nE - 1 - m] & 0xFFFF);
       const int x0 = nx0[cur][nd], x1 = nx1[cur][nd], y0 = ny0[cur][nd], y1 = ny1[cur][nd];
       const int hx = (x1 - x0 + 1) >> 1, hy = (y1 - y0 + 1) >> 1;
@@ -1178,10 +1180,10 @@
       }
     }
     __syncthreads();
-    for (int i = tid; i < nA; i += OCT_NT) scan[i] = (mark[i] == 0 || mark[i] > nP) ? 1 : 0;
-    __syncthreads();
-    const int nKeep = (int)block_scan_u64(scan, nA, tsum);
-    for (int i = tid; i < nA; i += OCT_NT) {
+    for (int i = tid; i < nA; i += NT) scan[i] = (mark[i] == 0 || mark[i] > nP) ? 1 : 0;
+    __syncthreads();
+    const int nKeep = (int)block_scan_u64<NT>(scan, nA, tsum);
+    for (int i = tid; i < nA; i += NT) {
       if (mark[i] == 0 || mark[i] > nP) {
         const int pos = tc + (int)scan[i];
         nx0[nxt][pos] = nx0[cur][i];
@@ -1194,7 +1196,7 @@
     }
     __syncthreads();
     cd.sweep([&](int, uint32_t, uint32_t& v) { v = cpos[(v & 0x3FFF) * 4 + (v >> 14)]; });
-    for (int i = tid; i < tc + nKeep; i += OCT_NT) nmid[i] = pack_mid(nxt, i);
+    for (int i = tid; i < tc + nKeep; i += NT) nmid[i] = pack_mid(nxt, i);
     __syncthreads();
     cur = nxt;
     nA = tc + nKeep;
@@ -1209,9 +1211,9 @@
   uint64_t* bestr = reinterpret_cast<uint64_t*>(cntr);
   const int nrepB = nrep >= 2 ? nrep * 2 : 1, repB = tid & (nrepB - 1);
   if (nrepB > 1)
-    for (int i = tid; i < nA * nrepB; i += OCT_NT) bestr[i] = 0;
+    for (int i = tid; i < nA * nrepB; i += NT) bestr[i] = 0;
   else
-    for (int i = tid; i < nA; i += OCT_NT) best[i] = 0;
+    for (int i = tid; i < nA; i += NT) best[i] = 0;
   __syncthreads();
   const float invH = 1.0f / (float)L.hCell, invW = 1.0f / (float)L.wCell;
   auto rank_key = [&](uint32_t key) {
@@ -1225,7 +1227,7 @@
       atomicMax((unsigned long long*)&bestr[nd * nrepB + repB], rank_key(key));
     });
     __syncthreads();
-    for (int i = tid; i < nA; i += OCT_NT) {
+    for (int i = tid; i < nA; i += NT) {
       uint64_t v = 0;
       for (int r = 0; r < nrepB; r++) v = bestr[i * nrepB + r] > v ? bestr[i * nrepB + r] : v;
       best[i] = v;
@@ -1256,6 +1258,7 @@
   return nIni <= 2 && oct_hbase(nIni, OCT_HD + 1) * 6 <= 16400 && nIni * (1 << (2 * OCT_HD)) * 2 <= 4096;
 }
 
+template <int NT>
 __device__ __forceinline__ bool octree_hist_body(const Geom& g, const LevelDev& L, const OctCtx& c, int n, int cells,
                                                  const uint32_t* __restrict__ sparse, uint32_t* __restrict__ keys,
                                                  uint32_t* __restrict__ out, int* __restrict__ outCount, int prof) {
@@ -1267,11 +1270,11 @@
 #define HMK() do {} while (0)
 #endif
   HMK();
-  OctCands<true> cd;
+  OctCands<true, NT> cd;
   cd.keys = keys;
   cd.kn = nullptr;
   cd.n = n;
-  octree_gather(cd, c, L, n, cells, sparse);
+  octree_gather<NT>(cd, c, L, n, cells, sparse);
   HMK();
   const int N = L.quota;
   struct Buf {
@@ -1300,7 +1303,7 @@
   uint64_t* tsum = c.tsum;
   int* s_i = c.s_i;
   const int nH = oct_hbase(nIni, OCT_HD + 1);
-  for (int i = tid; i < nH; i += OCT_NT) hist[i] = 0;
+  for (int i = tid; i < nH; i += NT) hist[i] = 0;
   if (tid == 0) s_i[3] = 0;
   const bool pathTab = 2 * (W + H) + 8 <= c.tabBytes;
   uint16_t* px = reinterpret_cast<uint16_t*>(c.tab);
@@ -1333,7 +1336,7 @@
     return code;
   };
   if (pathTab) {
-    for (int i = tid; i < W + H; i += OCT_NT) {
+    for (int i = tid; i < W + H; i += NT) {
       if (i < W) px[i] = (uint16_t)x_path(i);
       else py[i - W] = (uint16_t)y_path(i - W);
     }
@@ -1360,7 +1363,7 @@
   for (int d = OCT_HD - 1; d >= 0; d--) {
     const uint32_t* ch = hist + oct_hbase(nIni, d + 1);
     uint32_t* pa = hist + oct_hbase(nIni, d);
-    for (int i = tid; i < (nIni << (2 * d)); i += OCT_NT) pa[i] = ch[4 * i] + ch[4 * i + 1] + ch[4 * i + 2] + ch[4 * i + 3];
+    for (int i = tid; i < (nIni << (2 * d)); i += NT) pa[i] = ch[4 * i] + ch[4 * i + 1] + ch[4 * i + 2] + ch[4 * i + 3];
     __syncthreads();
   }
   auto child_count = [&](uint32_t dc, int q) {
@@ -1398,7 +1401,7 @@
       }
     };
     const int prevSize = nA;
-      for (int i = tid; i < nA; i += OCT_NT) {
+      for (int i = tid; i < nA; i += NT) {
         uint64_t cc = 0, nm = 1, ce = 0;
         if (ncnt[cur][i] > 1) {
           nm = 0;
@@ -1417,10 +1420,10 @@
       }
       sync();
       if (s_i[3]) return 3;
-      const uint64_t tot = kWave ? wave0_scan_u64(scan, nA) : block_scan_u64(scan, nA, tsum);
+      const uint64_t tot = kWave ? wave0_scan_u64(scan, nA) : block_scan_u64<NT>(scan, nA, tsum);
       const int tc = (int)(tot & 0x1FFFFF), tnm = (int)((tot >> 21) & 0x1FFFFF), tce = (int)(tot >> 42);
       const int nxt = cur ^ 1;
-      for (int i = tid; i < nA; i += OCT_NT) {
+      for (int i = tid; i < nA; i += NT) {
         const uint64_t pre = scan[i];
         const int pc = (int)(pre & 0x1FFFFF), pnm = (int)((pre >> 21) & 0x1FFFFF), pce = (int)(pre >> 42);
         if (ncnt[cur][i] > 1) {
@@ -1498,15 +1501,15 @@
     uint64_t* E = c.ebuf + ecur * c.maxn;
     uint64_t* E2 = c.ebuf + (ecur ^ 1) * c.maxn;
     introsort_block(E, nE, E2, reinterpret_cast<uint16_t*>(scan), reinterpret_cast<uint16_t*>(scan) + c.maxn + 4,
-                    reinterpret_cast<uint32_t*>(tsum));
+                    reinterpret_cast<uint32_t*>(tsum), NT);
     HMK();
     if (tid == 0) {
       s_i[1] = nE;
       s_i[2] = 0;
     }
-    for (int i = tid; i < nA; i += OCT_NT) mark[i] = 0;
-    __syncthreads();
-    for (int m = tid; m < nE; m += OCT_NT) {
+    for (int i = tid; i < nA; i += NT) mark[i] = 0;
+    __syncthreads();
+    for (int m = tid; m < nE; m += NT) {
       const int nd = (int)(E[nE - 1 - m] & 0xFFFF);
       mark[nd] = (uint16_t)(m + 1);
       const uint32_t dc = ndc(cur)[nd];
@@ -1524,8 +1527,8 @@
     }
     __syncthreads();
     if (s_i[3]) return false;
-    block_scan_u64(scan, nE, tsum);
-    for (int m = tid; m < nE; m += OCT_NT) {
+    block_scan_u64<NT>(scan, nE, tsum);
+    for (int m = tid; m < nE; m += NT) {
       const int nd = (int)(E[nE - 1 - m] & 0xFFFF);
       const uint32_t dc = ndc(cur)[nd];
       int cc = 0;
@@ -1557,7 +1560,7 @@
       tce = nE ? (int)(scan[nE - 1] >> 21) + ce : 0;
     }
     const int nxt = cur ^ 1;
-    for (int m = tid; m < nP; m += OCT_NT) {
+    for (int m = tid; m < nP; m += NT) {
       const int nd = (int)(E[nE - 1 - m] & 0xFFFF);
       const uint32_t dc = ndc(cur)[nd];
       const uint32_t cdc = (((dc >> 13) + 1) << 13) | ((dc & 0x1FFF) * 4);
@@ -1593,10 +1596,10 @@
       }
     }
     __syncthreads();
-    for (int i = tid; i < nA; i += OCT_NT) scan[i] = (mark[i] == 0 || mark[i] > nP) ? 1 : 0;
-    __syncthreads();
-    const int nKeep = (int)block_scan_u64(scan, nA, tsum);
-    for (int i = tid; i < nA; i += OCT_NT) {
+    for (int i = tid; i < nA; i += NT) scan[i] = (mark[i] == 0 || mark[i] > nP) ? 1 : 0;
+    __syncthreads();
+    const int nKeep = (int)block_scan_u64<NT>(scan, nA, tsum);
+    for (int i = tid; i < nA; i += NT) {
       if (mark[i] == 0 || mark[i] > nP) {
         const int pos = tc + (int)scan[i];
         nx0[nxt][pos] = nx0[cur][i];
@@ -1615,14 +1618,14 @@
     if (broke || nA == prevSize) finish = true;
     HMK();
   }
-  for (int i = tid; i < nH; i += OCT_NT) leafAt[i] = 0xFFFF;
-  __syncthreads();
-  for (int i = tid; i < nA; i += OCT_NT) {
+  for (int i = tid; i < nH; i += NT) leafAt[i] = 0xFFFF;
+  __syncthreads();
+  for (int i = tid; i < nA; i += NT) {
     const uint32_t dc = ndc(cur)[i];
     leafAt[oct_hbase(nIni, (int)(dc >> 13)) + (int)(dc & 0x1FFF)] = (uint16_t)i;
   }
   __syncthreads();
-  for (int c5 = tid; c5 < (nIni << (2 * OCT_HD)); c5 += OCT_NT) {
+  for (int c5 = tid; c5 < (nIni << (2 * OCT_HD)); c5 += NT) {
     uint16_t v = 0xFFFF;
 #pragma unroll
     for (int d = OCT_HD; d >= 0; d--) {
@@ -1637,9 +1640,9 @@
   uint64_t* bestr = reinterpret_cast<uint64_t*>(c.cntr);
   const int nrepB = c.nrep >= 2 ? c.nrep * 2 : 1, repB = tid & (nrepB - 1);
   if (nrepB > 1)
-    for (int i = tid; i < nA * nrepB; i += OCT_NT) bestr[i] = 0;
+    for (int i = tid; i < nA * nrepB; i += NT) bestr[i] = 0;
   else
-    for (int i = tid; i < nA; i += OCT_NT) best[i] = 0;
+    for (int i = tid; i < nA; i += NT) best[i] = 0;
   __syncthreads();
   const float invH = 1.0f / (float)L.hCell, invW = 1.0f / (float)L.wCell;
   auto rank_key = [&](uint32_t key) {
@@ -1655,7 +1658,7 @@
   });
   __syncthreads();
   const int nOut = min(nA, L.selCap);
-  for (int i = tid; i < nOut; i += OCT_NT) {
+  for (int i = tid; i < nOut; i += NT) {
     uint64_t v = nrepB > 1 ? 0 : best[i];
     if (nrepB > 1)
       for (int r = 0; r < nrepB; r++) v = bestr[i * nrepB + r] > v ? bestr[i * nrepB + r] : v;
@@ -1678,14 +1681,12 @@
   return true;
 }
 
-__global__ __launch_bounds__(OCT_NT, 4) void k_octree(Geom g, const uint32_t* __restrict__ cellCand,
-                                                const int* __restrict__ cellCount, int* __restrict__ cellPrefix,
-                                                uint32_t* __restrict__ cand, int* __restrict__ candCount,
-                                                uint16_t* __restrict__ knode, uint32_t* __restrict__ sel,
-                                                int* __restrict__ selCount, int profLevel, int forceGlobal, int level0,
-                                                int nlv) {
-  extern __shared__ __attribute__((aligned(16))) uint8_t smem[];
-  __shared__ int s_i[8];
+template <int NT>
+__device__ __forceinline__ void octree_block(const Geom& g, const uint32_t* __restrict__ cellCand,
+                                             const int* __restrict__ cellCount, uint32_t* __restrict__ cand,
+                                             int* __restrict__ candCount, uint16_t* __restrict__ knode,
+                                             uint32_t* __restrict__ sel, int* __restrict__ selCount, int profLevel,
+                                             int forceGlobal, int level0, int nlv, uint8_t* smem, int* s_i) {
   const int tid = threadIdx.x;
 #ifdef OCT_WG_PROF
   struct WgPrint {
@@ -1703,9 +1704,9 @@
   wgPrint.img = img;
 #endif
   const LevelDev L = g.lv[l];
-  const int maxn = oct_maxn(g);
-  const int nrep = oct_rep(g);
-  const OctLds o = oct_layout(maxn, oct_maxcells(g), nrep);
+  const int maxn = oct_maxn(g, level0, level0 + nlv);
+  const int nrep = oct_rep(g, level0, level0 + nlv);
+  const OctLds o = oct_layout(maxn, oct_maxcells(g, level0, level0 + nlv), nrep);
   OctCtx c;
   c.nx0 = (int16_t*)(smem + o.nx0[0]);
   c.nx1 = (int16_t*)(smem + o.nx1[0]);
@@ -1734,7 +1735,7 @@
   int n;
   {
     const int* cc = cellCount + (long long)img * g.totalCells + L.cellStart;
-    const int per = (cells + OCT_NT - 1) / OCT_NT;
+    const int per = (cells + NT - 1) / NT;
     const int cb = min(tid * per, cells), ce = min(cb + per, cells);
     int sum = 0;
     for (int ci = cb; ci < ce; ci++) sum += cc[ci];
@@ -1743,7 +1744,7 @@
     __syncthreads();
     int wbase = 0, total = 0;
 #pragma unroll
-    for (int w = 0; w < OCT_NT / 64; w++) {
+    for (int w = 0; w < NT / 64; w++) {
       const int t = (int)c.tsum[w];
       if (w < (tid >> 6)) wbase += t;
       total += t;
@@ -1765,36 +1766,110 @@
   uint16_t* kn = knode + (long long)img * g.candImg + L.candOff;
   uint32_t* out = sel + (long long)img * g.selImg + L.selOff;
   int* outCount = selCount + img * g.nlevels + l;
-  if (n <= OCT_KMAX * OCT_NT && forceGlobal != 1) {
+  if (n <= OCT_KMAX * NT && forceGlobal != 1) {
     const int W = L.w - 2 * kBorder, H = L.h - 2 * kBorder;
     const int nIni = (int)roundf((float)W / (float)H);
     bool done = false;
     if (forceGlobal == 0 && oct_hist_fits(nIni)) {
-      done = octree_hist_body(g, L, c, n, cells, sparse, keys, out, outCount, profLevel == l && img == 0);
+      done = octree_hist_body<NT>(g, L, c, n, cells, sparse, keys, out, outCount, profLevel == l && img == 0);
       __syncthreads();
     }
-    if (!done) octree_body<true>(g, L, c, n, cells, sparse, keys, kn, out, outCount, profLevel == l && img == 0);
+    if (!done) octree_body<true, NT>(g, L, c, n, cells, sparse, keys, kn, out, outCount, profLevel == l && img == 0);
   } else {
-    octree_body<false>(g, L, c, n, cells, sparse, keys, kn, out, outCount, profLevel == l && img == 0);
-  }
+    octree_body<false, NT>(g, L, c, n, cells, sparse, keys, kn, out, outCount, profLevel == l && img == 0);
+  }
+}
+
+template <int NT>
+__global__ __launch_bounds__(NT, 4) void k_octree(Geom g, const uint32_t* __restrict__ cellCand,
+                                                const int* __restrict__ cellCount, int* __restrict__ cellPrefix,
+                                                uint32_t* __restrict__ cand, int* __restrict__ candCount,
+                                                uint16_t* __restrict__ knode, uint32_t* __restrict__ sel,
+                                                int* __restrict__ selCount, int profLevel, int forceGlobal, int level0,
+                                                int nlv) {
+  extern __shared__ __attribute__((aligned(16))) uint8_t smem[];
+  __shared__ int s_i[8];
+  octree_block<NT>(g, cellCand, cellCount, cand, candCount, knode, sel, selCount, profLevel, forceGlobal, level0, nlv, smem, s_i);
+}
+
+__global__ __launch_bounds__(512, 4) void k_octree_mixed(Geom g, const uint32_t* __restrict__ cellCand,
+                                                         const int* __restrict__ cellCount, uint32_t* __restrict__ cand,
+                                                         int* __restrict__ candCount, uint16_t* __restrict__ knode,
+                                                         uint32_t* __restrict__ sel, int* __restrict__ selCount,
+                                                         int profLevel, int forceGlobal, uint32_t classes) {
+  extern __shared__ __attribute__((aligned(16))) uint8_t smem[];
+  __shared__ int s_i[8];
+  const int l = blockIdx.x / (gridDim.x / g.nlevels);
+  const int nt = 128 << ((classes >> (2 * l)) & 3u);
+  if ((int)threadIdx.x >= nt) return;
+  if (nt == 512)
+    octree_block<512>(g, cellCand, cellCount, cand, candCount, knode, sel, selCount, profLevel, forceGlobal, 0, g.nlevels, smem, s_i);
+  else if (nt == 256)
+    octree_block<256>(g, cellCand, cellCount, cand, candCount, knode, sel, selCount, profLevel, forceGlobal, 0, g.nlevels, smem, s_i);
+  else
+    octree_block<128>(g, cellCand, cellCount, cand, candCount, knode, sel, selCount, profLevel, forceGlobal, 0, g.nlevels, smem, s_i);
 }
 
 static int g_octree_force_global_host = 0;
 void debug_set_octree_global(int on) { g_octree_force_global_host = on < 0 ? 0 : (on > 2 ? 2 : on); }
-
-hipError_t launch_octree(const Geom& g, int nimg, const uint32_t* cellCand, const int* cellCount, int* cellPrefix,
-                         uint32_t* cand, int* candCount, uint16_t* knode, uint32_t* sel, int* selCount, int level0,
-                         int level1, hipStream_t s) {
-  if (level1 <= level0) return hipSuccess;
+static int g_octree_class_host = 0;
+void debug_set_octree_class(int nt) { g_octree_class_host = (nt == 128 || nt == 256 || nt == 512) ? nt : 0; }
+int debug_octree_class() { return g_octree_class_host; }
+
+constexpr int kOctArea256 = 300000, kOctArea128 = 70000;
+void build_octree_plan(const Geom& g, OctPlan& p) {
+  int prev = 512;
+  for (int l = 0; l < g.nlevels; l++) {
+    const long long area = (long long)(g.lv[l].w - 2 * kBorder) * (g.lv[l].h - 2 * kBorder);
+    const int nt = area > kOctArea256 ? 512 : (area > kOctArea128 ? 256 : 128);
+    prev = p.nt[l] = nt < prev ? nt : prev;
+    p.lds[l] = (int)octree_lds_bytes(g, 0, g.nlevels);
+  }
+}
+
+template <int NT>
+static hipError_t launch_octree_nt(const Geom& g, int nimg, const uint32_t* cellCand, const int* cellCount, int* cellPrefix,
+                                   uint32_t* cand, int* candCount, uint16_t* knode, uint32_t* sel, int* selCount, int level0,
+                                   int level1, hipStream_t s) {
   dim3 grid((level1 - level0) * nimg);
 #ifdef OCT_PROF
   static const int profLevel = getenv("ORBX_OCTREE_PROF_LEVEL") ? atoi(getenv("ORBX_OCTREE_PROF_LEVEL")) : 0;
 #else
   const int profLevel = -1;
 #endif
-  hipLaunchKernelGGL(k_octree, grid, dim3(OCT_NT), octree_lds_bytes(g), s, g, cellCand, cellCount, cellPrefix, cand,
-                     candCount, knode, sel, selCount, profLevel, g_octree_force_global_host, level0, level1 - level0);
+  const size_t lds = octree_lds_bytes(g, level0, level1);
+  if (g_octree_class_host) {
+    const hipError_t e = raise_dynamic_lds(reinterpret_cast<const void*>(k_octree<NT>), lds);
+    if (e != hipSuccess) return e;
+  }
+  hipLaunchKernelGGL(k_octree<NT>, grid, dim3(NT), lds, s, g, cellCand, cellCount, cellPrefix, cand, candCount, knode, sel,
+                     selCount, profLevel, g_octree_force_global_host, level0, level1 - level0);
   return hipGetLastError();
+}
+hipError_t launch_octree_mixed(const Geom& g, const OctPlan& plan, int nimg, const uint32_t* cellCand, const int* cellCount,
+                               uint32_t* cand, int* candCount, uint16_t* knode, uint32_t* sel, int* selCount, hipStream_t s) {
+  uint32_t classes = 0;
+  for (int l = 0; l < g.nlevels; l++) classes |= (plan.nt[l] == 512 ? 2u : (plan.nt[l] == 256 ? 1u : 0u)) << (2 * l);
+#ifdef OCT_PROF
+  static const int profLevel = getenv("ORBX_OCTREE_PROF_LEVEL") ? atoi(getenv("ORBX_OCTREE_PROF_LEVEL")) : 0;
+#else
+  const int profLevel = -1;
+#endif
+  hipLaunchKernelGGL(k_octree_mixed, dim3(g.nlevels * nimg), dim3(512), octree_lds_bytes(g, 0, g.nlevels), s, g, cellCand,
+                     cellCount, cand, candCount, knode, sel, selCount, profLevel, g_octree_force_global_host, classes);
+  return hipGetLastError();
+}
+hipError_t launch_octree(const Geom& g, int nimg, const uint32_t* cellCand, const int* cellCount, int* cellPrefix,
+                         uint32_t* cand, int* candCount, uint16_t* knode, uint32_t* sel, int* selCount, int level0,
+                         int level1, int nt, hipStream_t s) {
+  if (level1 <= level0) return hipSuccess;
+  if (nt == 128)
+    return launch_octree_nt<128>(g, nimg, cellCand, cellCount, cellPrefix, cand, candCount, knode, sel, selCount, level0, level1, s);
+  if (nt == 256)
+    return launch_octree_nt<256>(g, nimg, cellCand, cellCount, cellPrefix, cand, candCount, knode, sel, selCount, level0, level1, s);
+  if (nt == 512)
+    return launch_octree_nt<512>(g, nimg, cellCand, cellCount, cellPrefix, cand, candCount, knode, sel, selCount, level0, level1, s);
+  return hipErrorInvalidValue;
 }
 
 __device__ __forceinline__ int reflect101(int p, int n) {
@@ -2443,7 +2518,9 @@
 }
 
 hipError_t prepare_kernels(const Geom& g) {
-  hipError_t e = raise_dynamic_lds(reinterpret_cast<const void*>(k_octree), octree_lds_bytes(g));
+  const size_t octLds = octree_lds_bytes(g, 0, g.nlevels);
+  hipError_t e = raise_dynamic_lds(reinterpret_cast<const void*>(k_octree<512>), octLds);
+  if (e == hipSuccess) e = raise_dynamic_lds(reinterpret_cast<const void*>(k_octree_mixed), octLds);
   if (e != hipSuccess) return e;
   if (g.nlevels > 1) {
     e = raise_dynamic_lds(reinterpret_cast<const void*>(k_resize<0, true>), std::max<size_t>(resize_lds_bytes(g), 1024));
```

Result: faster. 84800 stereo frames/s (median of 6 runs) (+1.3%).
